# facebookresearch/pytorch3d

Hardware: AMD Instinct MI355X
Metric: rasterized Mpix/s (fwd+bwd) at 512^2 faces_per_pixel=8 (higher is better)
Workload: dtype f32

## Files before the change

include/p3d_amd.h:

```cpp
#ifndef P3D_AMD_H_
#define P3D_AMD_H_

#include <stddef.h>
#include <stdint.h>

#ifdef __cplusplus
extern "C" {
#endif

#define P3D_ABI_VERSION 3

#define P3D_OK 0
#define P3D_ERR_INVALID_ARG (-1)
#define P3D_ERR_K_TOO_LARGE (-2)
#define P3D_ERR_TOO_MANY_BINS (-3)
#define P3D_ERR_WORKSPACE (-4)
#define P3D_ERR_LAUNCH (-5)
#define P3D_ERR_UNSUPPORTED (-6)

#define P3D_MAX_K 150
#define P3D_MAX_BINS_PER_SIDE 21

typedef void* p3d_stream_t;

int p3d_abi_version(void);
const char* p3d_error_string(int code);


size_t p3d_rasterize_meshes_workspace_bytes(int64_t F, int N, int H, int W, int bin_size, int max_faces_per_bin);

size_t p3d_rasterize_meshes_short_workspace_bytes(int64_t F, int N, int H, int W, int bin_size, int max_faces_per_bin,
                                                  int64_t list_entries);
size_t p3d_rasterize_meshes_workspace_need_offset(int64_t F, int N, int H, int W, int bin_size, int max_faces_per_bin);

int p3d_rasterize_meshes(const float* face_verts, const int64_t* mesh_to_face_first_idx,
                         const int64_t* num_faces_per_mesh, const int64_t* clipped_faces_neighbor_idx, int64_t F, int N,
                         int H, int W, float blur_radius, int faces_per_pixel, int bin_size, int max_faces_per_bin,
                         int perspective_correct, int clip_barycentric_coords, int cull_backfaces, int64_t* pix_to_face,
                         float* zbuf, float* bary, float* dists, void* workspace, size_t workspace_bytes,
                         p3d_stream_t stream);

int p3d_rasterize_meshes_naive(const float* face_verts, const int64_t* mesh_to_face_first_idx,
                               const int64_t* num_faces_per_mesh, const int64_t* clipped_faces_neighbor_idx, int64_t F,
                               int N, int H, int W, float blur_radius, int faces_per_pixel, int perspective_correct,
                               int clip_barycentric_coords, int cull_backfaces, int64_t* pix_to_face, float* zbuf,
                               float* bary, float* dists, p3d_stream_t stream);

int p3d_rasterize_meshes_coarse(const float* face_verts, const int64_t* mesh_to_face_first_idx,
                                const int64_t* num_faces_per_mesh, int64_t F, int N, int H, int W, float blur_radius,
                                int bin_size, int max_faces_per_bin, int32_t* bin_faces, void* workspace,
                                size_t workspace_bytes, p3d_stream_t stream);

size_t p3d_rasterize_fine_workspace_bytes(int N, int BH, int BW, int M);

int p3d_rasterize_meshes_fine(const float* face_verts, const int32_t* bin_faces,
                              const int64_t* clipped_faces_neighbor_idx, int64_t F, int N, int BH, int BW, int M, int H,
                              int W, float blur_radius, int bin_size, int faces_per_pixel, int perspective_correct,
                              int clip_barycentric_coords, int cull_backfaces, int64_t* pix_to_face, float* zbuf,
                              float* bary, float* dists, void* workspace, size_t workspace_bytes, p3d_stream_t stream);

int p3d_rasterize_meshes_backward(const float* face_verts, const int64_t* pix_to_face, const float* grad_zbuf,
                                  const float* grad_bary, const float* grad_dists, int64_t F, int N, int H, int W, int K,
                                  int perspective_correct, int clip_barycentric_coords, float* grad_face_verts,
                                  p3d_stream_t stream);

size_t p3d_rasterize_meshes_cover_bytes(int N, int H, int W);

int p3d_rasterize_meshes_cover_check(const int64_t* pix_to_face, const int32_t* cover, int N, int H, int W, int K, int32_t* stale,
                                     p3d_stream_t stream);

size_t p3d_rasterize_meshes_cover_list_bytes(int N, int H, int W);

#define P3D_RASTER_COVER_LIST 1u
#define P3D_RASTER_CUDA_TIE_ORDER 2u


int p3d_rasterize_meshes_ex(const float* face_verts, const int64_t* mesh_to_face_first_idx, const int64_t* num_faces_per_mesh,
                            const int64_t* clipped_faces_neighbor_idx, int64_t F, int N, int H, int W, float blur_radius,
                            int faces_per_pixel, int bin_size, int max_faces_per_bin, int perspective_correct,
                            int clip_barycentric_coords, int cull_backfaces, int64_t* pix_to_face, float* zbuf, float* bary,
                            float* dists, int32_t* cover, unsigned flags, void* workspace, size_t workspace_bytes,
                            p3d_stream_t stream);

int p3d_gather_face_verts_pre(const float* verts, const int64_t* faces, int64_t V, int64_t F, float* face_verts, float* face_pre,
                              p3d_stream_t stream);

size_t p3d_rasterize_meshes_backward_workspace_bytes(int N, int H, int W);

#define P3D_BWD_COVER_HAS_LIST 1u
#define P3D_BWD_MAKE_FACE_PRE 2u

int p3d_rasterize_meshes_backward_ex(const float* face_verts, const int64_t* faces, float* face_pre,
                                     const int64_t* pix_to_face, const float* grad_zbuf, const float* grad_bary,
                                     const float* grad_dists, const int32_t* cover, int64_t F, int64_t V, int N, int H, int W,
                                     int K, int perspective_correct, int clip_barycentric_coords, unsigned flags,
                                     float* grad_out, void* workspace, size_t workspace_bytes, p3d_stream_t stream);


int p3d_gather_face_verts(const float* verts, const int64_t* faces, int64_t V, int64_t F, float* face_verts,
                          p3d_stream_t stream);
int p3d_scatter_face_grads(const float* grad_face_verts, const int64_t* faces, int64_t V, int64_t F, float* grad_verts,
                           p3d_stream_t stream);


int p3d_face_areas_normals_forward(const float* verts, const int64_t* faces, int64_t V, int64_t F, float* areas, float* normals,
                                   p3d_stream_t stream);
int p3d_face_areas_normals_backward(const float* grad_areas, const float* grad_normals, const float* verts, const int64_t* faces,
                                    int64_t V, int64_t F, float* grad_face_verts, p3d_stream_t stream);

size_t p3d_verts_normals_forward_workspace_bytes(int64_t F);
size_t p3d_verts_normals_backward_workspace_bytes(int64_t F);
int p3d_verts_normals_forward(const float* verts, const int64_t* faces, const int32_t* offsets, const int32_t* corners, int64_t V,
                              int64_t F, float* face_raw, float* sums, float* normals, p3d_stream_t stream);
int p3d_verts_normals_backward(const float* grad_normals, const float* verts, const int64_t* faces, const float* sums,
                               const int32_t* offsets, const int32_t* corners, int64_t V, int64_t F, float* face_rows,
                               float* grad_verts, p3d_stream_t stream);

size_t p3d_mesh_edge_loss_forward_workspace_bytes(int64_t E);
size_t p3d_mesh_laplacian_forward_workspace_bytes(int64_t V);
size_t p3d_mesh_normal_consistency_forward_workspace_bytes(int64_t P);
size_t p3d_mesh_normal_consistency_backward_workspace_bytes(int64_t P);
int p3d_mesh_edge_loss_forward(const float* verts, const int32_t* edges, const int32_t* edge_mesh, const int32_t* num_edges, int64_t V,
                               int64_t E, int N, float target_length, void* workspace, size_t workspace_bytes, float* loss,
                               p3d_stream_t stream);
int p3d_mesh_edge_loss_backward(const float* grad_loss, const float* verts, const int32_t* adj_offsets, const int32_t* adj,
                                const int32_t* vert_mesh, const int32_t* num_edges, int64_t V, int64_t E, int N, float target_length,
                                float* grad_verts, p3d_stream_t stream);
int p3d_mesh_laplacian_forward(const float* verts, const int32_t* adj_offsets, const int32_t* adj, const int32_t* vert_mesh,
                               const int32_t* num_verts, int64_t V, int64_t E, int N, float* q, void* workspace, size_t workspace_bytes,
                               float* loss, p3d_stream_t stream);
int p3d_mesh_laplacian_backward(const float* grad_loss, const float* q, const int32_t* adj_offsets, const int32_t* adj, int64_t V, int64_t E,
                                int N, float* grad_verts, p3d_stream_t stream);
int p3d_mesh_normal_consistency_forward(const float* verts, const int32_t* pairs, const int32_t* pair_mesh, const int32_t* num_pairs,
                                        int64_t V, int64_t P, int N, void* workspace, size_t workspace_bytes, float* loss,
                                        p3d_stream_t stream);
int p3d_mesh_normal_consistency_backward(const float* grad_loss, const float* verts, const int32_t* pairs, const int32_t* pair_mesh,
                                         const int32_t* num_pairs, const int32_t* offsets, const int32_t* slots, int64_t V, int64_t P,
                                         int N, void* workspace, size_t workspace_bytes, float* grad_verts, p3d_stream_t stream);


int p3d_transform_gather_face_verts(const float* verts_world, const int64_t* faces, const int64_t* mesh_to_face_first_idx,
                                    const float* matrices, int64_t V, int64_t F, int N, int num_matrices, float* face_verts,
                                    p3d_stream_t stream);
int p3d_transform_verts_forward(const float* verts_world, const int64_t* mesh_to_vert_first_idx, const float* matrices,
                                int64_t V, int N, int num_matrices, float* verts_ndc, p3d_stream_t stream);
int p3d_transform_verts_backward(const float* verts_world, const int64_t* mesh_to_vert_first_idx, const float* matrices,
                                 const float* grad_verts_ndc, int64_t V, int N, int num_matrices, float* grad_verts_world,
                                 p3d_stream_t stream);
size_t p3d_transform_backward_workspace_bytes(int64_t V, int N, int num_matrices);
int p3d_transform_backward_cameras(const float* verts_world, const int64_t* mesh_to_vert_first_idx, const float* matrices,
                                   const float* grad_verts_ndc, int64_t V, int N, int num_matrices, float* grad_verts_world,
                                   float* grad_matrices, void* workspace, size_t workspace_bytes, p3d_stream_t stream);


size_t p3d_rasterize_points_workspace_bytes(int64_t P, int N, int H, int W, int bin_size, int max_points_per_bin);
size_t p3d_rasterize_points_short_workspace_bytes(int64_t P, int N, int H, int W, int bin_size, int max_points_per_bin,
                                                  int64_t list_entries);
size_t p3d_rasterize_points_workspace_need_offset(int64_t P, int N, int H, int W, int bin_size, int max_points_per_bin);

int p3d_rasterize_points_ex(const float* points, const int64_t* cloud_to_packed_first_idx, const int64_t* num_points_per_cloud,
                            const float* radius, int64_t P, int N, int H, int W, int points_per_pixel, int bin_size,
                            int max_points_per_bin, int32_t* idxs, float* zbuf, float* dists, int composite_mode,
                            const float* features, int C, float inv_r2, float* images, unsigned flags, void* workspace,
                            size_t workspace_bytes, p3d_stream_t stream);

int p3d_rasterize_points(const float* points, const int64_t* cloud_to_packed_first_idx,
                         const int64_t* num_points_per_cloud, const float* radius, int64_t P, int N, int H, int W,
                         int points_per_pixel, int bin_size, int max_points_per_bin, int32_t* idxs, float* zbuf,
                         float* dists, void* workspace, size_t workspace_bytes, p3d_stream_t stream);

int p3d_rasterize_points_naive(const float* points, const int64_t* cloud_to_packed_first_idx,
                               const int64_t* num_points_per_cloud, const float* radius, int64_t P, int N, int H, int W,
                               int points_per_pixel, int32_t* idxs, float* zbuf, float* dists, p3d_stream_t stream);
// ... 297 lines not shown
```

pytorch3d_amd/_C.py:

```python
import ctypes
import os

import torch

from . import _lib

EPS = 1e-6
MAX_FLOAT = 3.4e38
MAX_INT = 2147483647
MAX_UINT = 4294967295
MAX_USHORT = 65535
PULSAR_MAX_GRAD_SPHERES = 128

kMaxPointsPerPixel = 150
kMaxItemsPerBin = 22


def _ptr(t):
    return ctypes.c_void_p(t.data_ptr() if t is not None and t.numel() > 0 else None)


def _stream(device):
    return ctypes.c_void_p(torch.cuda.current_stream(device).cuda_stream)

# ... 103 lines not shown
        self.pinned = None
        self.event = None

    def collect(self):
        if self.event is not None and self.event.query():
            self.last = int(self.pinned[0])
            self.entries = self.last if self.entries is None or self.last >= self.entries else self.entries - (self.entries - self.last) // 8
            self.event = None

    def tight(self):
        return self.last is not None and self.capacity is not None and self.last * 5 > self.capacity * 4

    def report_later(self, ws, offset, capacity=None):
        self.calls += 1
        if self.event is not None or (torch.cuda.is_available() and torch.cuda.is_current_stream_capturing()):
            return
        if not (self.calls <= 4 or self.calls % 8 == 0 or self.tight()):
            return
        if self.pinned is None:
            self.pinned = torch.empty((1,), dtype=torch.int64, pin_memory=True)
        self.pinned.copy_(ws[offset:offset + 8].view(torch.int64), non_blocking=True)
        self.event = torch.cuda.Event()
        self.event.record()
        if capacity is not None:
            self.capacity = int(capacity)


def _mesh_workspace(lib, F, N, H, W, bin_size, M, dev, what="meshes", extra=0):
    worst_fn = getattr(lib, f"p3d_rasterize_{what}_workspace_bytes")
    short_fn = getattr(lib, f"p3d_rasterize_{what}_short_workspace_bytes")
    at_fn = getattr(lib, f"p3d_rasterize_{what}_workspace_need_offset")
    worst = worst_fn(F, N, H, W, bin_size, M)
    if SHORT_WORKSPACE == "never" or (SHORT_WORKSPACE != "always" and worst <= SHORT_WORKSPACE_ABOVE):
        WORKSPACE_STATS["last_bytes"], WORKSPACE_STATS["last_entries"] = worst, None
        return _workspace(worst, dev), None, 0, None
    key = (what, dev.index, F, N, H, W, bin_size, M)
    need = _NEEDS.get(key)
    if need is None:
        if len(_NEEDS) >= 64:
            _NEEDS.pop(next(iter(_NEEDS)))
        need = _NEEDS[key] = _Need()
    if not torch.cuda.is_current_stream_capturing():
        need.collect()
    if need.entries is not None:
        entries = need.entries + need.entries // 4 + 4096
    else:
        entries = SHORT_WORKSPACE_FIRST_GUESS if SHORT_WORKSPACE_FIRST_GUESS is not None else 32 * F + (1 << 18)
    nbytes = min(short_fn(F, N, H, W, bin_size, M, int(entries)) + extra, worst)
    WORKSPACE_STATS["short_calls"] += 1
    WORKSPACE_STATS["last_bytes"], WORKSPACE_STATS["last_entries"] = nbytes, int(entries)
    return _workspace(nbytes, dev), need, at_fn(F, N, H, W, bin_size, M), int(entries)


CUDA_TIE_ORDER = os.environ.get("P3D_CUDA_TIE_ORDER", "0") not in ("", "0")


def _check_face_verts(face_verts):
    if not (face_verts.dim() == 3 and face_verts.size(1) == 3 and face_verts.size(2) == 3):
        raise RuntimeError("face_verts must have dimensions (num_faces, 3, 3)")


def _mesh_outputs(N, H, W, K, device):
    p2f = torch.empty((N, H, W, K), dtype=torch.int64, device=device)
    zbuf = torch.empty((N, H, W, K), dtype=torch.float32, device=device)
    bary = torch.empty((N, H, W, K, 3), dtype=torch.float32, device=device)
    dists = torch.empty((N, H, W, K), dtype=torch.float32, device=device)
    return p2f, zbuf, bary, dists


def rasterize_meshes(face_verts, mesh_to_face_first_idx, num_faces_per_mesh, clipped_faces_neighbor_idx, image_size,
                     blur_radius, faces_per_pixel, bin_size, max_faces_per_bin, perspective_correct,
                     clip_barycentric_coords, cull_backfaces):
    out, cover = _rasterize_meshes_covered(face_verts, mesh_to_face_first_idx, num_faces_per_mesh, clipped_faces_neighbor_idx,
                                           image_size, blur_radius, faces_per_pixel, bin_size, max_faces_per_bin, perspective_correct,
                                           clip_barycentric_coords, cull_backfaces, want_cover=True)
    if cover is not None:
        _remember_cover(out[0], cover)
    return out


RECALL_COVERS = os.environ.get("P3D_RECALL_COVERS", "1") not in ("", "0")
COVER_LIST = os.environ.get("P3D_COVER_LIST", "1") not in ("", "0")
FACE_PRE = os.environ.get("P3D_FACE_PRE", "1") not in ("", "0")
CHECK_COVERS = os.environ.get("P3D_CHECK", "0") not in ("", "0")
COVER_RECALLS = [0, 0]
COVER_CHECKS = [0, 0]
_COVER_ATTR = "_p3d_row_cover"


def _remember_cover(p2f, cover):
    setattr(p2f, _COVER_ATTR, (cover, p2f._version))


def forget_cover(pix_to_face):
    if hasattr(pix_to_face, _COVER_ATTR):
        delattr(pix_to_face, _COVER_ATTR)


def cover_is_current(p2f, cover):
    N, H, W, K = p2f.shape
    lib = _lib.load()
    with torch.cuda.device(p2f.device):
        stale = torch.empty((1,), dtype=torch.int32, device=p2f.device)
        rc = lib.p3d_rasterize_meshes_cover_check(_ptr(p2f), _ptr(cover), N, H, W, K, _ptr(stale), _stream(p2f.device))
        _lib.check(rc, "rasterize_meshes_cover_check")
        bad = bool(int(stale.item()))
    COVER_CHECKS[0] += 1
    COVER_CHECKS[1] += int(bad)
    return not bad


def checked_cover(p2f, cover):
    if cover is None or not CHECK_COVERS or torch.cuda.is_current_stream_capturing() or cover_is_current(p2f, cover):
        return cover
    import warnings

    warnings.warn("pytorch3d_amd: pix_to_face holds faces its forward's row cover does not know of (written through .data or by "
                  "another kernel since the forward?); the backward reads every row instead", RuntimeWarning)
    return None


def _recall_cover(p2f):
    e = getattr(p2f, _COVER_ATTR, None) if RECALL_COVERS and p2f.dtype == torch.int64 and p2f.is_contiguous() and p2f.dim() == 4 else None
    ok = e is not None and p2f._version == e[1] and e[0].device == p2f.device and \
        tuple(e[0].shape) == (p2f.shape[0], (p2f.shape[1] + 15) // 16, (p2f.shape[2] + 15) // 16)
    if ok and CHECK_COVERS and not torch.cuda.is_current_stream_capturing() and not cover_is_current(p2f, e[0]):
        import warnings

        warnings.warn("pytorch3d_amd: pix_to_face holds faces its forward's row cover does not know of (written through .data or by "
                      "another kernel since the forward?); the backward reads every row instead", RuntimeWarning)
        forget_cover(p2f)
        ok = False
    if not ok:
        COVER_RECALLS[1] += 1
        return None
    COVER_RECALLS[0] += 1
    return e[0]


def _rasterize_meshes_covered(face_verts, mesh_to_face_first_idx, num_faces_per_mesh, clipped_faces_neighbor_idx, image_size,
                              blur_radius, faces_per_pixel, bin_size, max_faces_per_bin, perspective_correct,
                              clip_barycentric_coords, cull_backfaces, want_cover=True):
    dev = _same_device(("face_verts", face_verts), ("mesh_to_face_first_idx", mesh_to_face_first_idx),
                       ("num_faces_per_mesh", num_faces_per_mesh),
                       ("clipped_faces_neighbor_idx", clipped_faces_neighbor_idx))
    _check_face_verts(face_verts)
    if num_faces_per_mesh.size(0) != mesh_to_face_first_idx.size(0):
        raise RuntimeError("num_faces_per_mesh must have save size first dimension as mesh_to_faces_packed_first_idx")
    if clipped_faces_neighbor_idx.size(0) != face_verts.size(0):
        raise RuntimeError("clipped_faces_neighbor_idx must have save size first dimension as face_verts")
    K = int(faces_per_pixel)
    _check_k(K)
    H, W = _hw(image_size)
    bin_size, M = int(bin_size), int(max_faces_per_bin)
    binned = bin_size > 0 and M > 0
    if binned:
        _num_bins(H, W, bin_size, "RasterizeCoarseCuda")
    fv = _c(face_verts, torch.float32)
    first, count = _c(mesh_to_face_first_idx, torch.int64), _c(num_faces_per_mesh, torch.int64)
    nb = _c(clipped_faces_neighbor_idx, torch.int64)
    N, F = count.size(0), fv.size(0)
    lib = _lib.load()
    with torch.cuda.device(dev):
        out = _mesh_outputs(N, H, W, K, dev)
        if out[0].numel() == 0:
            return out, None
        marks = N * ((H + 7) // 8) * ((W + 7) // 8) * 8 + 1024 if CUDA_TIE_ORDER else 0
        ws, need, need_at, entries = _mesh_workspace(lib, F, N, H, W, bin_size, M, dev, extra=marks) if binned else (_workspace(marks, dev), None, 0, None)
        cover, flags = None, _lib.RASTER_CUDA_TIE_ORDER if CUDA_TIE_ORDER else 0
        if want_cover and not CUDA_TIE_ORDER and COVER_LIST:
            words = N * ((H + 15) // 16) * ((W + 15) // 16)
            buf = torch.empty((lib.p3d_rasterize_meshes_cover_list_bytes(N, H, W) // 4,), dtype=torch.int32, device=dev)
            cover = buf[:words].view(N, (H + 15) // 16, (W + 15) // 16)
            flags |= _lib.RASTER_COVER_LIST
        elif want_cover:
            cover = torch.empty((N, (H + 15) // 16, (W + 15) // 16), dtype=torch.int32, device=dev)
        rc = lib.p3d_rasterize_meshes_ex(
            _ptr(fv), _ptr(first), _ptr(count), _ptr(nb), F, N, H, W, float(blur_radius), K, bin_size if binned else 0,
            M if binned else 0, int(bool(perspective_correct)), int(bool(clip_barycentric_coords)), int(bool(cull_backfaces)),
            _ptr(out[0]), _ptr(out[1]), _ptr(out[2]), _ptr(out[3]), _ptr(cover), flags, _ptr(ws), ws.numel(), _stream(dev))
        _lib.check(rc, "rasterize_meshes")
        if need is not None:
            need.report_later(ws, need_at, entries)
    return out, cover


def _rasterize_meshes_naive(face_verts, mesh_to_face_first_idx, num_faces_per_mesh, clipped_faces_neighbor_idx,
                            image_size, blur_radius, faces_per_pixel, perspective_correct, clip_barycentric_coords,
                            cull_backfaces):
    return rasterize_meshes(face_verts, mesh_to_face_first_idx, num_faces_per_mesh, clipped_faces_neighbor_idx,
                            image_size, blur_radius, faces_per_pixel, 0, 0, perspective_correct,
                            clip_barycentric_coords, cull_backfaces)


def _rasterize_meshes_coarse(face_verts, mesh_to_face_first_idx, num_faces_per_mesh, image_size, blur_radius, bin_size,
                             max_faces_per_bin):
    dev = _same_device(("face_verts", face_verts), ("mesh_to_face_first_idx", mesh_to_face_first_idx),
                       ("num_faces_per_mesh", num_faces_per_mesh))
    _check_face_verts(face_verts)
    H, W = _hw(image_size)
    bin_size, M = int(bin_size), int(max_faces_per_bin)
    BH, BW = _num_bins(H, W, bin_size, "RasterizeCoarseCuda")
    fv = _c(face_verts, torch.float32)
    first, count = _c(mesh_to_face_first_idx, torch.int64), _c(num_faces_per_mesh, torch.int64)
    N, F = count.size(0), fv.size(0)
    lib = _lib.load()
    with torch.cuda.device(dev):
        out = torch.empty((N, BH, BW, M), dtype=torch.int32, device=dev)
        if out.numel() == 0:
            return out
        ws = _workspace(lib.p3d_rasterize_meshes_workspace_bytes(F, N, H, W, bin_size, M), dev)
        rc = lib.p3d_rasterize_meshes_coarse(_ptr(fv), _ptr(first), _ptr(count), F, N, H, W, float(blur_radius),
                                             bin_size, M, _ptr(out), _ptr(ws), ws.numel(), _stream(dev))
        _lib.check(rc, "_rasterize_meshes_coarse")
    return out


def _rasterize_meshes_fine(face_verts, bin_faces, clipped_faces_neighbor_idx, image_size, blur_radius, bin_size,
                           faces_per_pixel, perspective_correct, clip_barycentric_coords, cull_backfaces):
    dev = _same_device(("face_verts", face_verts), ("bin_faces", bin_faces),
                       ("clipped_faces_neighbor_idx", clipped_faces_neighbor_idx))
    _check_face_verts(face_verts)
    if bin_faces.dim() != 4:
        raise RuntimeError("bin_faces must have 4 dimensions")
    if clipped_faces_neighbor_idx.size(0) != face_verts.size(0):
        raise RuntimeError("clipped_faces_neighbor_idx must have the same first dimension as face_verts")
    K = int(faces_per_pixel)
    if K > kMaxPointsPerPixel:
        raise RuntimeError("Must have num_closest <= 150")
    H, W = _hw(image_size)
    fv = _c(face_verts, torch.float32)
    bf = _c(bin_faces, torch.int32)
    nb = _c(clipped_faces_neighbor_idx, torch.int64)
    N, BH, BW, M = bf.shape
    lib = _lib.load()
    with torch.cuda.device(dev):
        out = _mesh_outputs(N, H, W, K, dev)
        if out[0].numel() == 0:
            return out
        ws = _workspace(lib.p3d_rasterize_fine_workspace_bytes(N, BH, BW, M), dev)
        rc = lib.p3d_rasterize_meshes_fine(_ptr(fv), _ptr(bf), _ptr(nb), fv.size(0), N, BH, BW, M, H, W,
                                           float(blur_radius), int(bin_size), K, int(bool(perspective_correct)),
                                           int(bool(clip_barycentric_coords)), int(bool(cull_backfaces)), _ptr(out[0]),
                                           _ptr(out[1]), _ptr(out[2]), _ptr(out[3]), _ptr(ws), ws.numel(), _stream(dev))
        _lib.check(rc, "_rasterize_meshes_fine")
    return out


def cover_ptr(cover, N, H, W):
    if cover is None:
        return None
    if cover.dtype != torch.int32 or tuple(cover.shape) != (N, (H + 15) // 16, (W + 15) // 16) or not cover.is_contiguous():
        raise RuntimeError("row cover does not belong to this pix_to_face")
    return _ptr(cover)


def cover_has_list(cover, N, H, W):
    if cover is None or cover.storage_offset() != 0 or not cover.is_contiguous():
        return False
    need = _lib.load().p3d_rasterize_meshes_cover_list_bytes(N, H, W)
    return need > 0 and cover.untyped_storage().nbytes() == need


def backward_workspace(cover, N, H, W, dev):
    n = _lib.load().p3d_rasterize_meshes_backward_workspace_bytes(N, H, W) if (cover is not None and not cover_has_list(cover, N, H, W)) else 0
    return _workspace(n, dev)


def _mesh_backward(face_verts, faces, V, pix_to_face, grad_zbuf, grad_bary, grad_dists, perspective_correct, clip_barycentric_coords,
                   cover, face_pre=None):
    dev = pix_to_face.device
    zeros = lambda *tail: torch.zeros(tuple(pix_to_face.shape) + tail, dtype=torch.float32, device=dev)
    gz = _c(grad_zbuf, torch.float32) if grad_zbuf is not None else zeros()
    gb = _c(grad_bary, torch.float32) if grad_bary is not None else zeros(3)
    gd = _c(grad_dists, torch.float32) if grad_dists is not None else zeros()
    fv, p2f = _c(face_verts, torch.float32), _c(pix_to_face, torch.int64)
    N, H, W, K = p2f.shape
    F = fv.size(0)
    persp, clip = int(bool(perspective_correct)), int(bool(clip_barycentric_coords))
    has_list = cover_has_list(cover, N, H, W)
    flags = _lib.BWD_COVER_HAS_LIST if has_list else 0
    with torch.cuda.device(dev):
        if faces is None:
            out = torch.empty((F, 3, 3), dtype=torch.float32, device=dev)
            if FACE_PRE and persp and clip and K in (4, 8):
                face_pre = torch.empty((F, 4), dtype=torch.float32, device=dev)
                flags |= _lib.BWD_MAKE_FACE_PRE
        else:
            faces = _c(faces, torch.int64)
            out = (torch.empty if F else torch.zeros)((V, 3), dtype=torch.float32, device=dev)
            if not (has_list or cover is None):
                face_pre = None
        if F == 0:
            return out
        if _ordered():
            lib = _lib.load()
            hits = _sorted_hits(p2f)
            corners = _sorted_corners(faces, V) if faces is not None else None
            ws = _workspace(lib.p3d_rasterize_meshes_backward_ordered_workspace_bytes(F, int(faces is not None), hits.numel()), dev)
            rc = lib.p3d_rasterize_meshes_backward_ordered(
                _ptr(fv), _ptr(faces), _ptr(p2f), _ptr(gz), _ptr(gb), _ptr(gd), _ptr(hits), hits.numel(), _ptr(corners),
                corners.numel() if corners is not None else 0, F, V, N, H, W, K, persp, clip, _ptr(out), _ptr(ws), ws.numel(), _stream(dev))
            _lib.check(rc, "rasterize_meshes_backward")
            return out
        ws = backward_workspace(cover, N, H, W, dev)
        rc = _lib.load().p3d_rasterize_meshes_backward_ex(
            _ptr(fv), _ptr(faces), _ptr(face_pre), _ptr(p2f), _ptr(gz), _ptr(gb), _ptr(gd), cover_ptr(cover, N, H, W), F, V, N, H, W,
            K, persp, clip, flags, _ptr(out), _ptr(ws), ws.numel(), _stream(dev))
        _lib.check(rc, "rasterize_meshes_backward")
    return out


def scatter_face_grads(grad_face_verts, faces, V):
    dev = grad_face_verts.device
    g, faces = _c(grad_face_verts, torch.float32), _c(faces, torch.int64)
    F = faces.shape[0]
    lib = _lib.load()
    with torch.cuda.device(dev):
        out = torch.empty((V, 3), dtype=torch.float32, device=dev)
        if not V:
            return out
        if _ordered():
            corners = _sorted_corners(faces, V)
            ws = _workspace(lib.p3d_scatter_face_grads_ordered_workspace_bytes(F), dev)
            rc = lib.p3d_scatter_face_grads_ordered(_ptr(g), _ptr(faces), _ptr(corners), corners.numel(), V, F, _ptr(out), _ptr(ws),
                                                    ws.numel(), _stream(dev))
        else:
            rc = lib.p3d_scatter_face_grads(_ptr(g), _ptr(faces), V, F, _ptr(out), _stream(dev))
        _lib.check(rc, "scatter_face_grads")
    return out


def rasterize_meshes_backward(face_verts, pix_to_face, grad_zbuf, grad_bary, grad_dists, perspective_correct,
                              clip_barycentric_coords, _cover=None):
    _same_device(("face_verts", face_verts), ("pix_to_face", pix_to_face), ("grad_zbuf", grad_zbuf), ("grad_bary", grad_bary),
                 ("grad_dists", grad_dists))
    if _cover is None:
        _cover = _recall_cover(pix_to_face)
    return _mesh_backward(face_verts, None, 0, pix_to_face, grad_zbuf, grad_bary, grad_dists, perspective_correct,
                          clip_barycentric_coords, _cover)


def _check_points(points):
    if not (points.dim() == 2 and points.size(1) == 3):
        raise RuntimeError("points must have dimensions (num_points, 3)")


def _point_outputs(N, H, W, K, device):
    idx = torch.empty((N, H, W, K), dtype=torch.int32, device=device)
    zbuf = torch.empty((N, H, W, K), dtype=torch.float32, device=device)
    dists = torch.empty((N, H, W, K), dtype=torch.float32, device=device)
    return idx, zbuf, dists


_SPLAT_MODES = {"alpha": 0, "norm": 1}


def _rasterize_points(who, points, cloud_to_packed_first_idx, num_points_per_cloud, image_size, radius, points_per_pixel, bin_size,
                      max_points_per_bin, features=None, inv_r2=0.0, mode="alpha"):
    splat = features is not None
    dev = _same_device(("points", points), ("cloud_to_packed_first_idx", cloud_to_packed_first_idx),
                       ("num_points_per_cloud", num_points_per_cloud), ("radius", radius), *((("features", features),) if splat else ()))
    _check_points(points)
    if radius.dim() != 1 or radius.size(0) != points.size(0):
        raise RuntimeError("radius must be of shape (P,)")
    if splat and (features.dim() != 2 or features.size(0) != points.size(0) or not 1 <= features.size(1) <= 4):
        raise RuntimeError("features must be of shape (P, C) with C in 1..4")
    K = int(points_per_pixel)
    _check_k(K)
    H, W = _hw(image_size)
    bin_size, M = int(bin_size), int(max_points_per_bin)
    binned = bin_size > 0 and M > 0
    if binned:
# ... 769 lines not shown
```

pytorch3d_amd/_lib.py:

```python
import ctypes
import os
import threading

_HERE = os.path.dirname(os.path.abspath(__file__))
LIB_PATH = os.environ.get("P3D_LIB_PATH") or os.path.join(_HERE, "libp3d_amd.so")

c_i64 = ctypes.c_int64
c_int = ctypes.c_int
c_uint = ctypes.c_uint
c_f32 = ctypes.c_float
c_f64 = ctypes.c_double
c_ptr = ctypes.c_void_p
c_size = ctypes.c_size_t

ABI_VERSION = 3

RASTER_COVER_LIST = 1
RASTER_CUDA_TIE_ORDER = 2
BWD_COVER_HAS_LIST = 1
BWD_MAKE_FACE_PRE = 2
KNN_MAX_K = 32
KNN_TILE = 512
KNN_ACCUMULATE_P2 = 1
FRAMES_MAX_K = 64
FRAMES_DISAMBIGUATE = 1
FRAMES_ROWS_PER_GROUP = 64
BOX3D_LDS_CAPACITY = 64
BOX3D_WAVES_PER_GROUP = 4
BOX3D_MAX_GROUPS = 4096
FPS_REGISTER_POINTS = 16384
POINT_MESH_POINT, POINT_MESH_SEGMENT, POINT_MESH_TRIANGLE = 0, 1, 2
POINT_MESH_TILE = 64
POINT_MESH_ACCUMULATE_QUERIES = 1
POINT_MESH_ACCUMULATE_TARGETS = 2

_SIGNATURES = {
    "p3d_abi_version": (c_int, []),
    "p3d_error_string": (ctypes.c_char_p, [c_int]),
    "p3d_rasterize_meshes_workspace_bytes": (c_size, [c_i64, c_int, c_int, c_int, c_int, c_int]),
    "p3d_rasterize_meshes_short_workspace_bytes": (c_size, [c_i64, c_int, c_int, c_int, c_int, c_int, c_i64]),
    "p3d_rasterize_meshes_workspace_need_offset": (c_size, [c_i64, c_int, c_int, c_int, c_int, c_int]),
    "p3d_rasterize_meshes": (c_int, [c_ptr, c_ptr, c_ptr, c_ptr, c_i64, c_int, c_int, c_int, c_f32, c_int, c_int, c_int,
                                     c_int, c_int, c_int, c_ptr, c_ptr, c_ptr, c_ptr, c_ptr, c_size, c_ptr]),
    "p3d_rasterize_meshes_naive": (c_int, [c_ptr, c_ptr, c_ptr, c_ptr, c_i64, c_int, c_int, c_int, c_f32, c_int, c_int,
                                           c_int, c_int, c_ptr, c_ptr, c_ptr, c_ptr, c_ptr]),
    "p3d_rasterize_meshes_coarse": (c_int, [c_ptr, c_ptr, c_ptr, c_i64, c_int, c_int, c_int, c_f32, c_int, c_int, c_ptr,
                                            c_ptr, c_size, c_ptr]),
    "p3d_rasterize_fine_workspace_bytes": (c_size, [c_int, c_int, c_int, c_int]),
    "p3d_rasterize_meshes_fine": (c_int, [c_ptr, c_ptr, c_ptr, c_i64, c_int, c_int, c_int, c_int, c_int, c_int, c_f32,
                                          c_int, c_int, c_int, c_int, c_int, c_ptr, c_ptr, c_ptr, c_ptr, c_ptr, c_size,
                                          c_ptr]),
    "p3d_rasterize_meshes_backward": (c_int, [c_ptr, c_ptr, c_ptr, c_ptr, c_ptr, c_i64, c_int, c_int, c_int, c_int,
                                              c_int, c_int, c_ptr, c_ptr]),
    "p3d_rasterize_meshes_cover_bytes": (c_size, [c_int, c_int, c_int]),
    "p3d_rasterize_meshes_cover_check": (c_int, [c_ptr, c_ptr, c_int, c_int, c_int, c_int, c_ptr, c_ptr]),
    "p3d_rasterize_meshes_cover_list_bytes": (c_size, [c_int, c_int, c_int]),
    "p3d_rasterize_meshes_ex": (c_int, [c_ptr, c_ptr, c_ptr, c_ptr, c_i64, c_int, c_int, c_int, c_f32, c_int, c_int, c_int, c_int,
                                        c_int, c_int, c_ptr, c_ptr, c_ptr, c_ptr, c_ptr, c_uint, c_ptr, c_size, c_ptr]),
    "p3d_rasterize_meshes_backward_workspace_bytes": (c_size, [c_int, c_int, c_int]),
    "p3d_gather_face_verts": (c_int, [c_ptr, c_ptr, c_i64, c_i64, c_ptr, c_ptr]),
    "p3d_gather_face_verts_pre": (c_int, [c_ptr, c_ptr, c_i64, c_i64, c_ptr, c_ptr, c_ptr]),
    "p3d_rasterize_meshes_backward_ex": (c_int, [c_ptr, c_ptr, c_ptr, c_ptr, c_ptr, c_ptr, c_ptr, c_ptr, c_i64, c_i64, c_int, c_int,
                                                 c_int, c_int, c_int, c_int, c_uint, c_ptr, c_ptr, c_size, c_ptr]),
    "p3d_scatter_face_grads": (c_int, [c_ptr, c_ptr, c_i64, c_i64, c_ptr, c_ptr]),
    "p3d_face_areas_normals_forward": (c_int, [c_ptr, c_ptr, c_i64, c_i64, c_ptr, c_ptr, c_ptr]),
    "p3d_face_areas_normals_backward": (c_int, [c_ptr, c_ptr, c_ptr, c_ptr, c_i64, c_i64, c_ptr, c_ptr]),
    "p3d_verts_normals_forward_workspace_bytes": (c_size, [c_i64]),
    "p3d_verts_normals_backward_workspace_bytes": (c_size, [c_i64]),
    "p3d_verts_normals_forward": (c_int, [c_ptr, c_ptr, c_ptr, c_ptr, c_i64, c_i64, c_ptr, c_ptr, c_ptr, c_ptr]),
    "p3d_verts_normals_backward": (c_int, [c_ptr, c_ptr, c_ptr, c_ptr, c_ptr, c_ptr, c_i64, c_i64, c_ptr, c_ptr, c_ptr]),
    "p3d_mesh_edge_loss_forward_workspace_bytes": (c_size, [c_i64]),
    "p3d_mesh_laplacian_forward_workspace_bytes": (c_size, [c_i64]),
    "p3d_mesh_normal_consistency_forward_workspace_bytes": (c_size, [c_i64]),
    "p3d_mesh_normal_consistency_backward_workspace_bytes": (c_size, [c_i64]),
    "p3d_mesh_edge_loss_forward": (c_int, [c_ptr, c_ptr, c_ptr, c_ptr, c_i64, c_i64, c_int, c_f32, c_ptr, c_size, c_ptr, c_ptr]),
    "p3d_mesh_edge_loss_backward": (c_int, [c_ptr, c_ptr, c_ptr, c_ptr, c_ptr, c_ptr, c_i64, c_i64, c_int, c_f32, c_ptr, c_ptr]),
    "p3d_mesh_laplacian_forward": (c_int, [c_ptr, c_ptr, c_ptr, c_ptr, c_ptr, c_i64, c_i64, c_int, c_ptr, c_ptr, c_size, c_ptr, c_ptr]),
    "p3d_mesh_laplacian_backward": (c_int, [c_ptr, c_ptr, c_ptr, c_ptr, c_i64, c_i64, c_int, c_ptr, c_ptr]),
    "p3d_mesh_normal_consistency_forward": (c_int, [c_ptr, c_ptr, c_ptr, c_ptr, c_i64, c_i64, c_int, c_ptr, c_size, c_ptr, c_ptr]),
    "p3d_mesh_normal_consistency_backward": (c_int, [c_ptr, c_ptr, c_ptr, c_ptr, c_ptr, c_ptr, c_ptr, c_i64, c_i64, c_int, c_ptr, c_size,
                                                     c_ptr, c_ptr]),
    "p3d_transform_gather_face_verts": (c_int, [c_ptr, c_ptr, c_ptr, c_ptr, c_i64, c_i64, c_int, c_int, c_ptr, c_ptr]),
    "p3d_transform_verts_forward": (c_int, [c_ptr, c_ptr, c_ptr, c_i64, c_int, c_int, c_ptr, c_ptr]),
    "p3d_transform_verts_backward": (c_int, [c_ptr, c_ptr, c_ptr, c_ptr, c_i64, c_int, c_int, c_ptr, c_ptr]),
    "p3d_transform_backward_workspace_bytes": (c_size, [c_i64, c_int, c_int]),
    "p3d_transform_backward_cameras": (c_int, [c_ptr, c_ptr, c_ptr, c_ptr, c_i64, c_int, c_int, c_ptr, c_ptr, c_ptr, c_size, c_ptr]),
    "p3d_rasterize_points_workspace_bytes": (c_size, [c_i64, c_int, c_int, c_int, c_int, c_int]),
    "p3d_rasterize_points_short_workspace_bytes": (c_size, [c_i64, c_int, c_int, c_int, c_int, c_int, c_i64]),
    "p3d_rasterize_points_workspace_need_offset": (c_size, [c_i64, c_int, c_int, c_int, c_int, c_int]),
    "p3d_rasterize_points_ex": (c_int, [c_ptr, c_ptr, c_ptr, c_ptr, c_i64, c_int, c_int, c_int, c_int, c_int, c_int, c_ptr, c_ptr,
                                        c_ptr, c_int, c_ptr, c_int, c_f32, c_ptr, c_uint, c_ptr, c_size, c_ptr]),
    "p3d_rasterize_points": (c_int, [c_ptr, c_ptr, c_ptr, c_ptr, c_i64, c_int, c_int, c_int, c_int, c_int, c_int, c_ptr,
                                     c_ptr, c_ptr, c_ptr, c_size, c_ptr]),
    "p3d_rasterize_points_naive": (c_int, [c_ptr, c_ptr, c_ptr, c_ptr, c_i64, c_int, c_int, c_int, c_int, c_ptr, c_ptr,
                                           c_ptr, c_ptr]),
    "p3d_rasterize_points_coarse": (c_int, [c_ptr, c_ptr, c_ptr, c_ptr, c_i64, c_int, c_int, c_int, c_int, c_int, c_ptr,
                                            c_ptr, c_size, c_ptr]),
    "p3d_rasterize_points_fine": (c_int, [c_ptr, c_ptr, c_ptr, c_i64, c_int, c_int, c_int, c_int, c_int, c_int, c_int,
                                          c_int, c_ptr, c_ptr, c_ptr, c_ptr, c_size, c_ptr]),
    "p3d_rasterize_points_composite_backward": (c_int, [c_int, c_ptr, c_ptr, c_ptr, c_ptr, c_ptr, c_i64, c_int, c_int, c_int, c_int, c_int,
                                                        ctypes.c_float, c_ptr, c_ptr, c_ptr]),
    "p3d_rasterize_points_backward": (c_int, [c_ptr, c_ptr, c_ptr, c_ptr, c_i64, c_int, c_int, c_int, c_int, c_ptr,
                                              c_ptr]),
    "p3d_composite_forward": (c_int, [c_int, c_ptr, ctypes.POINTER(c_i64), c_ptr, c_ptr, c_int, c_int, c_i64, c_int, c_int, c_int,
                                      ctypes.POINTER(c_i64), ctypes.POINTER(c_i64), c_ptr, c_ptr]),
    "p3d_composite_backward": (c_int, [c_int, c_ptr, c_ptr, ctypes.POINTER(c_i64), c_ptr, c_ptr, c_int, c_int, c_i64, c_int, c_int,
                                       c_int, ctypes.POINTER(c_i64), ctypes.POINTER(c_i64), c_ptr, ctypes.POINTER(c_i64), c_ptr,
                                       c_ptr]),
    "p3d_interp_face_attrs_forward": (c_int, [c_int, c_ptr, c_ptr, c_ptr, c_i64, c_i64, c_i64, c_ptr, c_ptr]),
    "p3d_interp_face_attrs_backward": (c_int, [c_int, c_ptr, c_ptr, c_ptr, c_ptr, c_i64, c_i64, c_i64, c_ptr, c_ptr,
                                               c_ptr]),
    "p3d_interp_face_attrs_backward_nhwk": (c_int, [c_ptr, c_ptr, c_ptr, c_ptr, c_int, c_int, c_int, c_int, c_i64, c_int,
                                                    c_ptr, c_ptr, c_ptr]),
    "p3d_clip_faces_plan_bytes": (c_size, [c_i64]),
    "p3d_clip_faces_plan": (c_int, [c_ptr, c_i64, ctypes.POINTER(c_f32), c_int, c_int, c_int, c_f32, c_ptr, c_size,
                                    c_ptr]),
    "p3d_clip_faces_emit": (c_int, [c_ptr, c_i64, c_ptr, c_int, c_ptr, c_size, c_i64, c_i64, c_i64, c_f32, c_int, c_ptr,
                                    c_ptr, c_ptr, c_ptr, c_ptr, c_ptr, c_ptr, c_ptr]),
    "p3d_clip_faces_backward": (c_int, [c_ptr, c_i64, c_ptr, c_size, c_i64, c_i64, c_f32, c_int, c_ptr, c_ptr, c_ptr,
                                        c_ptr]),
    "p3d_convert_clipped_forward": (c_int, [c_ptr, c_ptr, c_ptr, c_ptr, c_ptr, c_i64, c_ptr, c_ptr, c_ptr]),
    "p3d_convert_clipped_backward": (c_int, [c_ptr, c_ptr, c_ptr, c_ptr, c_ptr, c_i64, c_i64, c_ptr, c_ptr, c_ptr]),
    "p3d_sigmoid_alpha_blend_forward": (c_int, [c_ptr, c_ptr, c_f32, c_i64, c_int, c_ptr, c_ptr]),
    "p3d_sigmoid_alpha_blend_backward": (c_int, [c_ptr, c_ptr, c_ptr, c_ptr, c_f32, c_i64, c_int, c_ptr, c_ptr]),
    "p3d_softmax_rgb_blend_forward": (c_int, [c_ptr, c_ptr, c_ptr, c_ptr, c_f32, c_f32, ctypes.POINTER(c_f32), c_f32,
                                              c_f32, c_ptr, c_ptr, c_i64, c_i64, c_int, c_ptr, c_ptr]),
    "p3d_softmax_rgb_blend_backward": (c_int, [c_ptr, c_ptr, c_ptr, c_ptr, c_ptr, c_f32, c_f32, ctypes.POINTER(c_f32),
                                               c_f32, c_f32, c_ptr, c_ptr, c_i64, c_i64, c_int, c_ptr, c_ptr, c_ptr,
                                               c_ptr]),
    "p3d_phong_shade_forward": (c_int, [c_ptr, c_ptr, c_ptr, c_int, c_ptr, c_ptr, c_int, c_int, c_int, c_int, c_int, c_i64,
                                        c_ptr, c_ptr]),
    "p3d_phong_shade_backward": (c_int, [c_ptr, c_ptr, c_ptr, c_ptr, c_int, c_ptr, c_ptr, c_int, c_int, c_int, c_int,
                                         c_int, c_i64, c_ptr, c_ptr, c_ptr, c_ptr, c_ptr]),
    "p3d_soft_phong_supported_k": (c_int, [c_int]),
    "p3d_soft_phong_forward": (c_int, [c_ptr, c_ptr, c_ptr, c_ptr, c_ptr, c_int, c_ptr, c_ptr, c_int, c_f32, c_f32,
                                       ctypes.POINTER(c_f32), c_f32, c_f32, c_ptr, c_ptr, c_int, c_int, c_int, c_int, c_i64,
                                       c_ptr, c_ptr]),
    "p3d_soft_phong_backward": (c_int, [c_ptr, c_ptr, c_ptr, c_ptr, c_ptr, c_ptr, c_int, c_ptr, c_ptr, c_int, c_f32, c_f32,
                                        ctypes.POINTER(c_f32), c_f32, c_f32, c_ptr, c_ptr, c_int, c_int, c_int, c_int, c_i64,
                                        c_ptr, c_ptr, c_ptr, c_ptr, c_ptr, c_ptr, c_ptr]),
    "p3d_sample_uv_forward": (c_int, [c_ptr, c_ptr, c_ptr, c_ptr, c_int, c_int, c_int, c_int, c_i64, c_int, c_int, c_int,
# ... 135 lines not shown
```

pytorch3d_amd/build.py:

```python
import json
import os
import re
import subprocess
import sys
from concurrent.futures import ThreadPoolExecutor

HERE = os.path.dirname(os.path.abspath(__file__))
CSRC = os.path.join(HERE, "csrc")
LIB = os.environ.get("P3D_LIB_PATH") or os.path.join(HERE, "libp3d_amd.so")
ARCH = "gfx950"

SOURCES = ["binning.hip", "raster_mesh.hip", "raster_mesh_bwd.hip", "gather.hip", "transform.hip", "raster_points.hip", "render_points.hip", "composite.hip", "blend.hip", "clip.hip", "interp.hip", "shade.hip", "soft_phong.hip", "splatter.hip", "texture.hip", "texture_multi.hip", "atlas.hip", "ordered_bwd.hip", "normals.hip", "mesh_losses.hip", "knn.hip", "point_mesh.hip", "sample_points.hip", "fps_ball.hip", "points_to_volumes.hip", "point_frames.hip", "box3d.hip", "profile.cpp"]
HEADERS = ["binning.h", "p3d_common.h", "p3d_geom.h", "topk.h", "topk_insert_asm.h", "wave_table.h", "tile_map.h", "chunk_order.h", "atlas_cell.h", "uvm_sample.h", "shade_sample.h", "ordered_sum.h", "knn_grad.h", "knn_queue.h", "point_mesh_geom.h", "vec3.h", "fixed_sum.h", "csr_gather.h", "box3d_geom.h", os.path.join("..", "..", "include", "p3d_amd.h")]

FLAGS = [
    f"--offload-arch={ARCH}", "-O3", "-std=c++17", "-fPIC", "-fvisibility=hidden", "-ffp-contract=off",
    "-munsafe-fp-atomics", "-Wno-unused-result",
    "-fno-slp-vectorize",
]


AGPR_KERNELS_TESTED = {
    "softmax_blend_bwd_kernel<32>": "tests/test_gpu_blending.py::test_blend_kernels_vs_oracle_all_capacities[17|24|32-dense]",
    "composite_bwd_tile_kernel<0, 32>": "tests/test_gpu_points_composite_interp.py::test_compositors[17|24|32]",
}


def _hipcc():
    for c in (os.environ.get("HIPCC"), "/opt/rocm/bin/hipcc", "hipcc"):
        if c and (os.path.isabs(c) and os.path.exists(c) or not os.path.isabs(c)):
            return c
    return "hipcc"


def _newest(paths):
    return max(os.path.getmtime(p) for p in paths if os.path.exists(p))


def _extra_flags():
    return os.environ.get("P3D_EXTRA_FLAGS", "").split()


def _flag_signature():
    return " ".join(FLAGS + _extra_flags())


def _stamp_path():
    return LIB + ".flags"


def needs_build():
    if not os.path.exists(LIB) or not os.path.exists(LIB + ".resources.json"):
        return True
    try:
        if open(_stamp_path()).read() != _flag_signature():
            return True
    except OSError:
        return True
    deps = [os.path.join(CSRC, s) for s in SOURCES + HEADERS] + [os.path.abspath(__file__)]
    return _newest(deps) > os.path.getmtime(LIB)


def build(force=False, verbose=False):
    if not (force or needs_build()):
        return LIB
    hipcc = _hipcc()
    objdir = os.path.join(HERE, "build", os.path.basename(LIB))
    os.makedirs(objdir, exist_ok=True)

    def compile_one(src):
        obj = os.path.join(objdir, src + ".o")
        extra = _extra_flags()
        cmd = [hipcc] + FLAGS + extra + ["-Rpass-analysis=kernel-resource-usage", "-x", "hip", "-c", os.path.join(CSRC, src), "-o", obj]
        if verbose:
            print(" ".join(cmd))
        res = subprocess.run(cmd, stderr=subprocess.PIPE, text=True)
        if res.returncode != 0:
            sys.stderr.write(res.stderr)
            raise subprocess.CalledProcessError(res.returncode, cmd)
        return obj, kernel_resources(res.stderr)

    with ThreadPoolExecutor(max_workers=min(len(SOURCES), os.cpu_count() or 1)) as ex:
        done = list(ex.map(compile_one, SOURCES))
    objs = [o for o, _ in done]
    resources = {}
    for src, (_, r) in zip(SOURCES, done):
        for k, v in r.items():
            resources[k] = dict(v, source=src)
    spilled = sorted(k for k, v in resources.items() if v["vgpr_spill"] > 0)
    agpr = sorted(k for k, v in resources.items() if v["agprs"] > 0 and not any(demangle(k).startswith("void " + t + "(") or demangle(k).startswith(t + "(")
                                                                                 for t in AGPR_KERNELS_TESTED))
    if (spilled or agpr) and os.environ.get("P3D_ALLOW_SPILLS"):
        print("[build] P3D_ALLOW_SPILLS: kernels with spilled VGPRs:", ", ".join(demangle(k) for k in spilled) or "none",
              "| with untested AGPR use:", ", ".join(demangle(k) for k in agpr) or "none", file=sys.stderr)
    elif agpr:
        raise RuntimeError("kernels that keep registers in AGPRs and are not in build.py: AGPR_KERNELS_TESTED (see there; "
# ... 41 lines not shown
```

pytorch3d_amd/csrc/binning.h:

```cpp
#pragma once

#include "p3d_common.h"

namespace p3d {

constexpr int kBinChunk = 1024;
constexpr int kMaxBinsSide = 32;
constexpr int kMaxBins = kMaxBinsSide * kMaxBinsSide;

enum BinKind { kTriangles = 0, kPoints = 1 };

struct BinGeom {
  int H, W, bin_size, BH, BW, nbins;
};

inline BinGeom make_geom(int H, int W, int bin_size) {
  BinGeom g;
  g.H = H;
  g.W = W;
  g.bin_size = bin_size;
  g.BH = 1 + (H - 1) / bin_size;
  g.BW = 1 + (W - 1) / bin_size;
  g.nbins = g.BH * g.BW;
  return g;
}

inline BinGeom make_internal_geom(int H, int W, int user_bin_size) {
  int b = 16;
  const int m = H > W ? H : W;
  while ((m + b - 1) / b > kMaxBinsSide) b *= 2;
  if (user_bin_size < b) {
    if ((m + user_bin_size - 1) / user_bin_size <= kMaxBinsSide) b = user_bin_size;
  }
  return make_geom(H, W, b);
}

constexpr int kPlanClasses = 64;
constexpr int kPlanHdr = 4;
constexpr int kPlanTicket = kPlanHdr + 2 * kPlanClasses;
constexpr int kPlanHdrInts = kPlanTicket + 4;
struct TilePlan {
  const int* arank;
  const int* bg_list;
  const int* hdr;
  const int* order;
};

struct BinCSR {
  const int64_t* offset;
  const int* total;
  const int* list;
  TilePlan plan;
  int stride = 1;
};

struct BinWorkspace {
  int* chunk_start;
  int* counts;
  int* total;
  int64_t* offset;
  long long* blocksum;
  int* arank;
  int* bg_list;
  int* plan_hdr;
  int* order;
  int* list;
  int stride;
  int64_t max_chunks;
  int64_t capacity;
  int64_t worst;
  size_t need_at;
};

int64_t bin_capacity(int64_t E, int N, const BinGeom& g, int M);
size_t bin_workspace_bytes(int64_t E, int N, const BinGeom& g, int M, int64_t list_entries = -1, bool with_z = false);
bool bin_carve(Arena& arena, int64_t E, int N, const BinGeom& g, int M, BinWorkspace* ws, int64_t list_entries = -1, bool with_z = false);

int bin_build(BinKind kind, const float* elems, const float* aux, const int64_t* first, const int64_t* count, int64_t E,
              int N, const BinGeom& g, int M, float sqrt_blur, const BinWorkspace& ws, hipStream_t stream,
              bool ordered = true);

int exclusive_scan_i32(const int* in, int64_t n, long long* blocksum, int64_t* out, hipStream_t stream);

int bin_expand_padded(const BinWorkspace& ws, int N, const BinGeom& g, int M, int32_t* out, hipStream_t stream);

int bin_compact_padded(const int32_t* padded, int64_t rows, int M, int* ws_list, int* ws_total, int64_t* ws_offset,
                       hipStream_t stream);

}
```

pytorch3d_amd/csrc/binning.hip:

```cpp
#include "binning.h"
#include "p3d_geom.h"

namespace p3d {

namespace {

constexpr int kWavesPerChunk = kBinChunk / kWave;

__global__ __launch_bounds__(1024) void bin_plan_kernel(const int64_t* __restrict__ count, int N,
                                                        int* __restrict__ chunk_start, int* __restrict__ plan_hdr) {
  __shared__ int scan[1024];
  __shared__ int carry_s;
  const int tid = threadIdx.x;
  if (tid < 2 * kPlanClasses) plan_hdr[kPlanHdr + tid] = 0;
  if (tid == 0) plan_hdr[kPlanTicket] = 0;
  if (tid == 0) carry_s = 0;
  __syncthreads();
  for (int base = 0; base < N; base += 1024) {
    const int i = base + tid;
    int v = 0;
    if (i < N) {
      const int64_t c = count[i];
      v = c > 0 ? (int)((c + kBinChunk - 1) / kBinChunk) : 0;
    }
    scan[tid] = v;
    __syncthreads();
    for (int d = 1; d < 1024; d <<= 1) {
      const int add = tid >= d ? scan[tid - d] : 0;
      __syncthreads();
      scan[tid] += add;
      __syncthreads();
    }
    const int carry = carry_s;
    if (i < N) chunk_start[i] = carry + scan[tid] - v;
    __syncthreads();
    if (tid == 1023) carry_s = carry + scan[1023];
    __syncthreads();
  }
  if (tid == 0) chunk_start[N] = carry_s;
}

struct BinRect {
  int x0, x1, y0, y1;
};

struct ChunkCtx {
  int n;
  int64_t e;
  BinRect r;
  BinRect u;
  float z;
};

constexpr int kSelfPlanMax = 64;

__device__ __forceinline__ void plan_in_lds(const int64_t* __restrict__ count, int N, int* cs) {
  const int tid = threadIdx.x;
  if (tid < kWave) {
    int v = 0;
    if (tid < N) {
      const int64_t c = count[tid];
      v = c > 0 ? (int)((c + kBinChunk - 1) / kBinChunk) : 0;
    }
    int x = v;
    for (int d = 1; d < kWave; d <<= 1) {
      const int y = __shfl_up(x, d);
      if (tid >= d) x += y;
    }
    cs[tid + 1] = x;
    if (tid == 0) cs[0] = 0;
  }
  __syncthreads();
}

template <typename Pred>
__device__ __forceinline__ int prefix_count(int n, Pred holds) {
  int lo = 0;
#pragma unroll
  for (int step = 32; step >= 1; step >>= 1) {
    const int t = lo + step;
    const int i = (t < n ? t : n) - 1;
    if (t <= n && holds(i)) lo = t;
  }
  return lo;
}

template <int KIND>
__device__ __forceinline__ bool chunk_prologue(const float* __restrict__ elems, const float* __restrict__ aux,
                                               const int64_t* __restrict__ first, const int64_t* __restrict__ count,
                                               const int* chunk_start, int* cs_l, int N, int H, int W, int bin_size,
                                               int BH, int BW, float sqrt_blur, float* xlo_t, float* xhi_t,
                                               float* ylo_t, float* yhi_t, ChunkCtx* c, int* publish_plan = nullptr,
                                               int* plan_hdr = nullptr) {
  const int tid = threadIdx.x;
  const int chunk = blockIdx.x;
  if (chunk_start == nullptr) {
    plan_in_lds(count, N, cs_l);
    chunk_start = cs_l;
    if (publish_plan != nullptr && chunk == 0) {
      if (tid <= N) publish_plan[tid] = cs_l[tid];
      if (tid < 2 * kPlanClasses) plan_hdr[kPlanHdr + tid] = 0;
      if (tid == 0) plan_hdr[kPlanTicket] = 0;
    }
  }
  if (chunk >= chunk_start[N]) return false;
  int lo = 0, hi = N;
  while (hi - lo > 1) {
    const int mid = (lo + hi) >> 1;
    if (chunk_start[mid] <= chunk)
      lo = mid;
    else
      hi = mid;
  }
  c->n = lo;
  if (tid < BW) {
    xlo_t[tid] = bin_lo(tid, bin_size, W, H);
    xhi_t[tid] = bin_hi(tid, bin_size, W, H);
  } else if (tid >= 64 && tid < 64 + BH) {
    const int b = tid - 64;
    ylo_t[b] = bin_lo(b, bin_size, H, W);
    yhi_t[b] = bin_hi(b, bin_size, H, W);
  }
  __syncthreads();

  const int64_t local = (int64_t)(chunk - chunk_start[lo]) * kBinChunk + tid;
  const int64_t cnt = count[lo];
  BinRect r;
  r.x0 = r.y0 = 1 << 20;
  r.x1 = r.y1 = -1;
  c->e = -1;
  c->z = 0.0f;
  if (local < cnt) {
    const int64_t e = first[lo] + local;
    c->e = e;
    float xmin, xmax, ymin, ymax;
    bool skip;
    if (KIND == kTriangles) {
      const float* q = elems + e * 9;
      const float v0x = q[0], v0y = q[1], v0z = q[2];
      const float v1x = q[3], v1y = q[4], v1z = q[5];
      const float v2x = q[6], v2y = q[7], v2z = q[8];
      xmin = min3(v0x, v1x, v2x) - sqrt_blur;
      xmax = max3(v0x, v1x, v2x) + sqrt_blur;
      ymin = min3(v0y, v1y, v2y) - sqrt_blur;
      ymax = max3(v0y, v1y, v2y) + sqrt_blur;
      skip = (double)min3(v0z, v1z, v2z) < P3D_KEPS;
    } else {
      const float* q = elems + e * 3;
      const float rad = aux[e];
      xmin = q[0] - rad;
      xmax = q[0] + rad;
      ymin = q[1] - rad;
      ymax = q[1] + rad;
      skip = q[2] < 0.0f;
      c->z = q[2];
    }
    if (!skip) {
      const int x0 = prefix_count(BW, [&](int b) { return !(xmin <= xhi_t[b]); });
      int x1 = prefix_count(BW, [&](int b) { return xlo_t[b] < xmax; });
      const int y0 = prefix_count(BH, [&](int b) { return !(ymin <= yhi_t[b]); });
      int y1 = prefix_count(BH, [&](int b) { return ylo_t[b] < ymax; });
      x1 -= 1;
      y1 -= 1;
      if (x0 <= x1 && y0 <= y1) {
        r.x0 = x0;
        r.x1 = x1;
        r.y0 = y0;
        r.y1 = y1;
      }
    }
  }
  c->r = r;
  BinRect u = r;
  for (int d = 32; d >= 1; d >>= 1) {
    u.x0 = min(u.x0, __shfl_xor(u.x0, d));
    u.y0 = min(u.y0, __shfl_xor(u.y0, d));
    u.x1 = max(u.x1, __shfl_xor(u.x1, d));
    u.y1 = max(u.y1, __shfl_xor(u.y1, d));
  }
  c->u = u;
  return true;
}

__device__ __forceinline__ void wave_masks(const ChunkCtx& c, int lane, unsigned long long* rm, unsigned long long* cm) {
  for (int by = c.u.y0; by <= c.u.y1; ++by) {
    const unsigned long long m = __ballot(by >= c.r.y0 && by <= c.r.y1);
    if (lane == 0) rm[by] = m;
  }
  for (int bx = c.u.x0; bx <= c.u.x1; ++bx) {
    const unsigned long long m = __ballot(bx >= c.r.x0 && bx <= c.r.x1);
    if (lane == 0) cm[bx] = m;
  }
  __builtin_amdgcn_fence(__ATOMIC_RELEASE, "wavefront");
}

template <typename F>
__device__ __forceinline__ void for_union_bins(const BinRect& u, int lane, F f) {
  const int ly = lane >> 3, lx = lane & 7;
  for (int ty = u.y0; ty <= u.y1; ty += 8) {
    for (int tx = u.x0; tx <= u.x1; tx += 8) {
      const int by = ty + ly, bx = tx + lx;
      if (by <= u.y1 && bx <= u.x1) f(by, bx);
    }
  }
}

template <int KIND, bool ORDERED>
__global__ __launch_bounds__(kBinChunk) void bin_count_kernel(const float* __restrict__ elems,
                                                              const float* __restrict__ aux,
                                                              const int64_t* __restrict__ first,
                                                              const int64_t* __restrict__ count,
                                                              const int* chunk_start, int N, int H, int W,
                                                              int bin_size, int BH, int BW, float sqrt_blur,
                                                              int* __restrict__ counts, int* publish_plan, int* plan_hdr) {
  __shared__ float xlo_t[32], xhi_t[32], ylo_t[32], yhi_t[32];
  __shared__ int cs_l[kSelfPlanMax + 1];
  __shared__ int blk_cnt[kMaxBins];
  __shared__ unsigned long long rowm[ORDERED ? kWavesPerChunk : 1][kMaxBinsSide], colm[ORDERED ? kWavesPerChunk : 1][kMaxBinsSide];
  const int nbins = BH * BW;
  for (int b = threadIdx.x; b < nbins; b += kBinChunk) blk_cnt[b] = 0;
  ChunkCtx c;
  if (!chunk_prologue<KIND>(elems, aux, first, count, chunk_start, cs_l, N, H, W, bin_size, BH, BW, sqrt_blur, xlo_t,
                            xhi_t, ylo_t, yhi_t, &c, publish_plan, plan_hdr))
    return;
  const int lane = lane_id();
  if (ORDERED) {
    const int w = threadIdx.x / kWave;
    const unsigned long long* rm = rowm[ORDERED ? w : 0];
    const unsigned long long* cm = colm[ORDERED ? w : 0];
    wave_masks(c, lane, rowm[ORDERED ? w : 0], colm[ORDERED ? w : 0]);
    for_union_bins(c.u, lane, [&](int by, int bx) {
      const int members = __popcll(rm[by] & cm[bx]);
      if (members) atomicAdd(&blk_cnt[by * BW + bx], members);
    });
  } else {
    for (int by = c.r.y0; by <= c.r.y1; ++by)
      for (int bx = c.r.x0; bx <= c.r.x1; ++bx) atomicAdd(&blk_cnt[by * BW + bx], 1);
  }
  __syncthreads();
  int* out = counts + (int64_t)blockIdx.x * nbins;
  for (int b = threadIdx.x; b < nbins; b += kBinChunk) out[b] = blk_cnt[b];
}

__global__ __launch_bounds__(256) void bin_scan_rows_kernel(int* __restrict__ counts,
                                                            const int* __restrict__ chunk_start, int N, int nbins, int M,
                                                            int* __restrict__ total) {
  const int lane = lane_id();
  const int64_t row = (int64_t)blockIdx.x * (blockDim.x / kWave) + (threadIdx.x / kWave);
  if (row >= (int64_t)N * nbins) return;
  const int n = (int)(row / nbins);
  const int b = (int)(row % nbins);
  const int c0 = chunk_start[n];
  const int nch = chunk_start[n + 1] - c0;
  int carry = 0;
  constexpr int U = 4;
  for (int base = 0; base < nch; base += U * kWave) {
    int v[U];
#pragma unroll
    for (int u = 0; u < U; ++u) {
      const int i = base + u * kWave + lane;
      v[u] = i < nch ? counts[((int64_t)(c0 + i)) * nbins + b] : 0;
    }
#pragma unroll
    for (int u = 0; u < U; ++u) {
      const int i = base + u * kWave + lane;
      int x = v[u];
      for (int d = 1; d < kWave; d <<= 1) {
        const int y = __shfl_up(x, d);
        if (lane >= d) x += y;
      }
      if (i < nch) counts[((int64_t)(c0 + i)) * nbins + b] = carry + x - v[u];
      carry += __shfl(x, kWave - 1);
    }
  }
  if (lane == 0) total[row] = carry < M ? carry : M;
}

constexpr int kPlanShift = 40;
constexpr long long kPlanMask = (1ll << kPlanShift) - 1;
__device__ __forceinline__ long long plan_pack(int total) { return (long long)total + (total > 0 ? (1ll << kPlanShift) : 0ll); }
__device__ __forceinline__ int plan_class(int v) { return kPlanClasses - 1 - min(v >> 3, kPlanClasses - 1); }

__device__ __forceinline__ void plan_emit(int64_t i, long long ex, int v, int64_t* offset, int* arank, int* bg_list) {
  offset[i] = ex & kPlanMask;
  const int r = (int)(ex >> kPlanShift);
  if (v <= 0) bg_list[i - r] = (int)i;
  arank[i] = r;
}

__device__ __forceinline__ long long block_exclusive_scan_1024(long long v, long long* wsum, long long* block_total) {
  const int tid = threadIdx.x, lane = tid & 63, w = tid >> 6;
  long long x = v;
  for (int d = 1; d < kWave; d <<= 1) {
    const long long y = __shfl_up(x, d);
    if (lane >= d) x += y;
  }
  if (lane == 63) wsum[w] = x;
  __syncthreads();
  long long base = 0, all = 0;
  for (int j = 0; j < 16; ++j) {
    const long long c = wsum[j];
    if (j < w) base += c;
    all += c;
  }
  *block_total = all;
  return base + x - v;
// ... 294 lines not shown
          list[dst_t[b] + pos] = (int)c.e;
      }
    }
  }
}

__global__ void bin_expand_kernel(const int64_t* __restrict__ offset, const int* __restrict__ total,
                                  const int* __restrict__ list, int64_t rows, int M, int32_t* __restrict__ out) {
  const int64_t n = rows * M;
  for (int64_t i = (int64_t)blockIdx.x * blockDim.x + threadIdx.x; i < n; i += (int64_t)gridDim.x * blockDim.x) {
    const int64_t row = i / M;
    const int m = (int)(i - row * M);
    out[i] = m < total[row] ? list[offset[row] + m] : -1;
  }
}

__global__ __launch_bounds__(256) void bin_compact_kernel(const int32_t* __restrict__ padded, int64_t rows, int M,
                                                          int* __restrict__ list, int* __restrict__ total,
                                                          int64_t* __restrict__ offset) {
  const int lane = lane_id();
  const int64_t row = (int64_t)blockIdx.x * (blockDim.x / kWave) + (threadIdx.x / kWave);
  if (row >= rows) return;
  const int32_t* src = padded + row * M;
  int* dst = list + row * M;
  int carry = 0;
  for (int base = 0; base < M; base += kWave) {
    const int i = base + lane;
    const int v = i < M ? src[i] : -1;
    const unsigned long long m = __ballot(v >= 0);
    if (v >= 0) dst[carry + mask_rank(m)] = v;
    carry += __popcll(m);
  }
  if (lane == 0) {
    total[row] = carry;
    offset[row] = row * M;
  }
}

}

int64_t bin_capacity(int64_t E, int N, const BinGeom& g, int M) {
  const int64_t a = E * (int64_t)g.nbins;
  const int64_t b = (int64_t)N * g.nbins * (int64_t)M;
  int64_t c = a < b ? a : b;
  if (c < 1) c = 1;
  return c;
}

bool bin_carve(Arena& arena, int64_t E, int N, const BinGeom& g, int M, BinWorkspace* ws, int64_t list_entries, bool with_z) {
  ws->max_chunks = ceil_div(E, kBinChunk) + N;
  ws->worst = bin_capacity(E, N, g, M);
  ws->chunk_start = arena.take<int>((size_t)N + 1);
  ws->counts = arena.take<int>((size_t)ws->max_chunks * g.nbins);
  ws->total = arena.take<int>((size_t)N * g.nbins);
  ws->need_at = arena.off + (size_t)N * g.nbins * sizeof(int64_t);
  ws->offset = arena.take<int64_t>((size_t)N * g.nbins + 1);
  ws->blocksum = arena.take<long long>((size_t)ceil_div((int64_t)N * g.nbins, 1024) + 1);
  ws->arank = arena.take<int>((size_t)N * g.nbins);
  ws->bg_list = arena.take<int>((size_t)N * g.nbins);
  ws->plan_hdr = arena.take<int>(kPlanHdrInts);
  ws->order = arena.take<int>((size_t)N * g.nbins);
  int64_t want = ws->worst;
  if (list_entries >= 0) {
    want = list_entries < 1 ? 1 : (list_entries < ws->worst ? list_entries : ws->worst);
    if (arena.base != nullptr && arena.cap > arena.off) {
      const int64_t room = (int64_t)((arena.cap - arena.off) / sizeof(int)) / (with_z ? 2 : 1);
      if (room > want) want = room < ws->worst ? room : ws->worst;
    }
  }
  ws->capacity = want;
  ws->stride = with_z ? 2 : 1;
  ws->list = arena.take<int>((size_t)want * (size_t)ws->stride);
  return arena.ok();
}

size_t bin_workspace_bytes(int64_t E, int N, const BinGeom& g, int M, int64_t list_entries, bool with_z) {
  Arena probe(nullptr, 0);
  BinWorkspace ws;
  bin_carve(probe, E, N, g, M, &ws, list_entries, with_z);
  return probe.off;
}

int bin_build(BinKind kind, const float* elems, const float* aux, const int64_t* first, const int64_t* count, int64_t E,
              int N, const BinGeom& g, int M, float sqrt_blur, const BinWorkspace& ws, hipStream_t stream, bool ordered) {
  if (N <= 0) return P3D_OK;
  const int64_t rows = (int64_t)N * g.nbins;
  const bool small = N <= kSelfPlanMax && rows <= 4096 && ws.max_chunks <= 128;
  const bool self_plan = N <= kSelfPlanMax;
  const int* cs = self_plan ? nullptr : ws.chunk_start;
  int* publish = self_plan && !small ? ws.chunk_start : nullptr;
  if (!self_plan) {
    LaunchScope ls("bin_plan", stream);
    bin_plan_kernel<<<1, 1024, 0, stream>>>(count, N, ws.chunk_start, ws.plan_hdr);
  }
  const unsigned chunks = (unsigned)ws.max_chunks;
  {
    LaunchScope ls("bin_count", stream);
    if (kind == kTriangles)
      bin_count_kernel<kTriangles, true><<<chunks, kBinChunk, 0, stream>>>(elems, aux, first, count, cs, N, g.H, g.W,
                                                                          g.bin_size, g.BH, g.BW, sqrt_blur, ws.counts, publish, ws.plan_hdr);
    else if (ordered)
      bin_count_kernel<kPoints, true><<<chunks, kBinChunk, 0, stream>>>(elems, aux, first, count, cs, N, g.H, g.W,
                                                                       g.bin_size, g.BH, g.BW, sqrt_blur, ws.counts, publish, ws.plan_hdr);
    else
      bin_count_kernel<kPoints, false><<<chunks, kBinChunk, 0, stream>>>(elems, aux, first, count, cs, N, g.H, g.W,
                                                                        g.bin_size, g.BH, g.BW, sqrt_blur, ws.counts, publish, ws.plan_hdr);
  }
  if (small) {
    LaunchScope ls("bin_scan_small", stream);
    bin_scan_small_kernel<<<1, 1024, 0, stream>>>(ws.counts, count, N, g.nbins, M, ws.total, ws.offset, ws.arank, ws.bg_list,
                                                  ws.plan_hdr, ws.capacity);
  } else {
    const unsigned nb = (unsigned)ceil_div(rows, 1024);
    const bool thread_rows = ws.max_chunks <= 32 * (int64_t)N;
    {
      LaunchScope ls("bin_scan_rows", stream);
      if (thread_rows)
        bin_scan_rows_sums_kernel<<<nb, 1024, 0, stream>>>(ws.counts, ws.chunk_start, N, g.nbins, M, ws.total, ws.blocksum,
                                                           ws.plan_hdr);
      else if (nb == 1)
        bin_scan_rows_tail_kernel<<<(unsigned)ceil_div(rows, kTailRows), 1024, 0, stream>>>(
            ws.counts, ws.chunk_start, N, g.nbins, M, ws.total, ws.offset, ws.arank, ws.bg_list, ws.plan_hdr, ws.order, ws.capacity);
      else
        bin_scan_rows_kernel<<<(unsigned)ceil_div(rows, 4), 256, 0, stream>>>(ws.counts, ws.chunk_start, N, g.nbins, M,
                                                                             ws.total);
    }
    if (thread_rows || nb > 1) {
      LaunchScope ls("bin_scan_offsets", stream);
      if (!thread_rows && nb > 1) bin_block_sums_kernel<<<nb, 1024, 0, stream>>>(ws.total, rows, ws.blocksum, ws.plan_hdr);
      bin_scan_offsets_kernel<<<nb, 1024, 0, stream>>>(ws.total, rows, ws.blocksum, ws.offset, ws.arank, ws.bg_list, ws.plan_hdr,
                                                       ws.order, ws.capacity);
    }
  }
  {
    LaunchScope ls("bin_fill", stream);
    if (kind == kTriangles)
      bin_fill_kernel<kTriangles, true><<<chunks, kBinChunk, 0, stream>>>(elems, aux, first, count, cs, N, g.H, g.W,
                                                                         g.bin_size, g.BH, g.BW, sqrt_blur, M, ws.counts,
                                                                         ws.offset, ws.list, ws.plan_hdr, ws.stride);
    else if (ordered)
      bin_fill_kernel<kPoints, true><<<chunks, kBinChunk, 0, stream>>>(elems, aux, first, count, cs, N, g.H, g.W,
                                                                      g.bin_size, g.BH, g.BW, sqrt_blur, M, ws.counts,
                                                                      ws.offset, ws.list, ws.plan_hdr, ws.stride);
    else
      bin_fill_kernel<kPoints, false><<<chunks, kBinChunk, 0, stream>>>(elems, aux, first, count, cs, N, g.H, g.W,
                                                                       g.bin_size, g.BH, g.BW, sqrt_blur, M, ws.counts,
                                                                       ws.offset, ws.list, ws.plan_hdr, ws.stride);
  }
  return launch_status();
}

int exclusive_scan_i32(const int* in, int64_t n, long long* blocksum, int64_t* out, hipStream_t stream) {
  if (n <= 0) return P3D_OK;
  const unsigned nb = (unsigned)ceil_div(n, 1024);
  if (nb > 1) bin_block_sums_kernel<<<nb, 1024, 0, stream>>>(in, n, blocksum, nullptr);
  bin_scan_offsets_kernel<<<nb, 1024, 0, stream>>>(in, n, blocksum, out, nullptr, nullptr, nullptr, nullptr, 0);
  return launch_status();
}

int bin_expand_padded(const BinWorkspace& ws, int N, const BinGeom& g, int M, int32_t* out, hipStream_t stream) {
  const int64_t rows = (int64_t)N * g.nbins;
  const int64_t n = rows * M;
  if (n <= 0) return P3D_OK;
  int64_t blocks = ceil_div(n, 256);
  if (blocks > 8192) blocks = 8192;
  LaunchScope ls("bin_expand", stream);
  bin_expand_kernel<<<(unsigned)blocks, 256, 0, stream>>>(ws.offset, ws.total, ws.list, rows, M, out);
  return launch_status();
}

int bin_compact_padded(const int32_t* padded, int64_t rows, int M, int* ws_list, int* ws_total, int64_t* ws_offset,
                       hipStream_t stream) {
  if (rows <= 0) return P3D_OK;
  LaunchScope ls("bin_compact", stream);
  bin_compact_kernel<<<(unsigned)ceil_div(rows, 4), 256, 0, stream>>>(padded, rows, M, ws_list, ws_total, ws_offset);
  return launch_status();
}

}
```

pytorch3d_amd/csrc/gather.hip:

```cpp
#include "p3d_common.h"
#include "p3d_geom.h"
#include "wave_table.h"

namespace p3d {
namespace {

__global__ __launch_bounds__(256) void gather_faces_kernel(const float* __restrict__ verts,
                                                           const int64_t* __restrict__ faces, int64_t V, int64_t n_corners,
                                                           float* __restrict__ face_verts) {
  for (int64_t c = (int64_t)blockIdx.x * 256 + threadIdx.x; c < n_corners; c += (int64_t)gridDim.x * 256) {
    int64_t v = faces[c];
    if (v < 0) v += V;
    const bool ok = v >= 0 && v < V;
    const float* s = verts + (ok ? v : 0) * 3;
    float* d = face_verts + c * 3;
    const float nan = __int_as_float(0x7fc00000);
    d[0] = ok ? s[0] : nan;
    d[1] = ok ? s[1] : nan;
    d[2] = ok ? s[2] : nan;
  }
}

__global__ __launch_bounds__(256) void gather_faces_pre_kernel(const float* __restrict__ verts, const int64_t* __restrict__ faces,
                                                               int64_t V, int64_t F, float* __restrict__ face_verts,
                                                               float4* __restrict__ face_pre) {
  for (int64_t f = (int64_t)blockIdx.x * 256 + threadIdx.x; f < F; f += (int64_t)gridDim.x * 256) {
    float c[9];
    const float nan = __int_as_float(0x7fc00000);
#pragma unroll
    for (int k = 0; k < 3; ++k) {
      int64_t v = faces[f * 3 + k];
      if (v < 0) v += V;
      const bool ok = v >= 0 && v < V;
      const float* s = verts + (ok ? v : 0) * 3;
      c[3 * k + 0] = ok ? s[0] : nan;
      c[3 * k + 1] = ok ? s[1] : nan;
      c[3 * k + 2] = ok ? s[2] : nan;
    }
    float* d = face_verts + f * 9;
#pragma unroll
    for (int k = 0; k < 9; ++k) d[k] = c[k];
    const BwdFacePre r = bwd_face_pre_make(mk3(c[0], c[1], c[2]), mk3(c[3], c[4], c[5]), mk3(c[6], c[7], c[8]));
    face_pre[f] = make_float4(r.inv_area, r.inv_l01, r.inv_l02, r.inv_l12);
  }
}

using VertTable = WaveTable<3, 426>;

__global__ __launch_bounds__(256) void scatter_face_grads_kernel(const float* __restrict__ grad_face_verts,
                                                                 const int64_t* __restrict__ faces, int64_t V,
                                                                 int64_t n_corners, int64_t span,
                                                                 float* __restrict__ grad_verts) {
  __shared__ __align__(16) int s_table[4][VertTable::kLdsInts];
  const int lane = threadIdx.x & 63, w = threadIdx.x >> 6;
  const int64_t begin = ((int64_t)blockIdx.x * 4 + w) * span;
  if (begin >= n_corners) return;
  const int64_t end = begin + span < n_corners ? begin + span : n_corners;
  VertTable tab;
  tab.init(s_table[w], lane);
  for (int64_t base = begin; base < end; base += 64) {
    const int64_t c = base + lane;
    int v = -1;
    float g[3] = {0.f, 0.f, 0.f};
    if (c < end) {
      int64_t vi = faces[c];
      if (vi < 0) vi += V;
      v = (vi >= 0 && vi < V) ? (int)vi : -1;
      const float* s = grad_face_verts + c * 3;
      g[0] = s[0];
      g[1] = s[1];
      g[2] = s[2];
    }
    tab.add(grad_verts, lane, v, g);
  }
  if (tab.used > 0) tab.flush(grad_verts, lane);
}

}
}

using namespace p3d;

P3D_API int p3d_gather_face_verts(const float* verts, const int64_t* faces, int64_t V, int64_t F, float* face_verts,
                                  p3d_stream_t stream) {
  if (V < 0 || F < 0) return P3D_ERR_INVALID_ARG;
  if (F == 0) return P3D_OK;
  if (!verts || !faces || !face_verts) return P3D_ERR_INVALID_ARG;
  hipStream_t s = (hipStream_t)stream;
  const int64_t n = F * 3;
  int64_t blocks = ceil_div(n, 256);
  if (blocks > 256 * 16) blocks = 256 * 16;
  LaunchScope ls("gather_face_verts", s);
  gather_faces_kernel<<<(unsigned)blocks, 256, 0, s>>>(verts, faces, V, n, face_verts);
  return launch_status();
}

P3D_API int p3d_gather_face_verts_pre(const float* verts, const int64_t* faces, int64_t V, int64_t F, float* face_verts,
                                      float* face_pre, p3d_stream_t stream) {
  if (V < 0 || F < 0) return P3D_ERR_INVALID_ARG;
  if (F == 0) return P3D_OK;
  if (!verts || !faces || !face_verts || !face_pre || ((uintptr_t)face_pre & 15u)) return P3D_ERR_INVALID_ARG;
  hipStream_t s = (hipStream_t)stream;
  int64_t blocks = ceil_div(F, 256);
  if (blocks > 256 * 16) blocks = 256 * 16;
  LaunchScope ls("gather_face_verts", s);
  gather_faces_pre_kernel<<<(unsigned)blocks, 256, 0, s>>>(verts, faces, V, F, face_verts, reinterpret_cast<float4*>(face_pre));
  return launch_status();
}

P3D_API int p3d_scatter_face_grads(const float* grad_face_verts, const int64_t* faces, int64_t V, int64_t F,
                                   float* grad_verts, p3d_stream_t stream) {
  if (V < 0 || F < 0) return P3D_ERR_INVALID_ARG;
  if (V == 0) return P3D_OK;
  if (!grad_verts) return P3D_ERR_INVALID_ARG;
  hipStream_t s = (hipStream_t)stream;
  if (hipMemsetAsync(grad_verts, 0, (size_t)V * 3 * sizeof(float), s) != hipSuccess) return P3D_ERR_LAUNCH;
  if (F == 0) return P3D_OK;
  if (!grad_face_verts || !faces) return P3D_ERR_INVALID_ARG;
  const int64_t n = F * 3;
  int64_t waves = ceil_div(n, 1024);
  if (waves > 4 * 4096) waves = 4 * 4096;
  const int64_t blocks = ceil_div(waves, 4);
  const int64_t span = ceil_div(ceil_div(n, blocks * 4), 64) * 64;
  LaunchScope ls("scatter_face_grads", s);
  scatter_face_grads_kernel<<<(unsigned)blocks, 256, 0, s>>>(grad_face_verts, faces, V, n, span, grad_verts);
  return launch_status();
// ... 2 lines not shown
```

pytorch3d_amd/csrc/raster_mesh.hip:

```cpp
#include "binning.h"
#include "tile_map.h"
#include "chunk_order.h"
#include "p3d_geom.h"
#include "topk.h"

#include <stdio.h>
#include <stdlib.h>

#ifndef P3D_STAGE_RANGE_INDEX
#define P3D_STAGE_RANGE_INDEX 1
#endif

#ifdef P3D_PROBE_CHAIN
__device__ unsigned long long g_chain[32];
extern "C" __attribute__((visibility("default"))) void p3d_probe_chain_read(unsigned long long* out) {
  (void)hipDeviceSynchronize();
  (void)hipMemcpyFromSymbol(out, HIP_SYMBOL(g_chain), sizeof(unsigned long long) * 32);
  unsigned long long z[32] = {0};
  (void)hipMemcpyToSymbol(HIP_SYMBOL(g_chain), z, sizeof(z));
}
namespace p3d {
namespace {
constexpr int kChainStamps = 11;
__shared__ unsigned long long s_chain[4][kChainStamps + 1];
// ... 462 lines not shown
        if (GENERAL || adm) hit = face_dist_rec<PC && !GENERAL>(fr, p, a.blur, bp, &h);
      }
      if (hit) {
        bool ins = true;
        if constexpr (GENERAL) {
          const int nb = __float_as_int(r2.z);
          if (nb != -1) {
            const int at = q.find(nb);
            if (at >= 0) {
              float queued;
              if constexpr (Queue::kPayload > 0) {
                queued = q.payload_at(0, at);
              } else {
                queued = recompute_face(a, nb, p, persp, clip).dist;
              }
              if (fabsf(h.dist) < fabsf(queued))
                q.erase(at);
              else
                ins = false;
            }
          }
        }
        if (ins && q.admits(K, h.z, f)) {
          if constexpr (Queue::kPayload > 0) {
            const float pl[kMeshPayload] = {h.dist, h.bary.x, h.bary.y, h.bary.z};
            q.insert(K, h.z, f, pl);
          } else {
            const float none[1] = {0.0f};
            q.insert(K, h.z, f, none);
          }
          if constexpr (TIES && !GENERAL) {
            const bool ev = (kz0 < INFINITY) & (q.kth_z(K) == kz0);
            const int d = kz0 == tie_z ? min(tie_drop, ki0) : ki0;
            tie_drop = ev ? d : tie_drop;
            tie_z = ev ? kz0 : tie_z;
          }
        }
      }
    }
  }
}

__device__ __forceinline__ void cover_mark(const MeshArgs& a, int n, int sy0, bool any, int yo, int xo, int lane) {
  unsigned long long rem = __ballot(any);
  const int wid = (yo >> 4) * a.CX + (xo >> 4);
  while (rem) {
    const int w0 = __builtin_amdgcn_readlane(wid, __builtin_ctzll(rem));
    const unsigned long long same = __ballot(any && wid == w0);
    unsigned bits = 0;
#pragma unroll
    for (int j = 0; j < 8; ++j)
      if ((same >> (8 * j)) & 0xffull) bits |= 1u << ((a.H - 1 - (sy0 + j)) & 15);
    rem &= ~same;
    if (lane == 0) {
      const int word = (n * a.CY) * a.CX + w0;
      if (a.area_list != nullptr && !a.list_by_plan) {
        const int before = atomicOr(a.cover + word, (int)bits);
        if (before == 0 && bits != 0u) a.area_list[atomicAdd(a.area_count, 1)] = word;
      } else {
        atomicOr(a.cover + word, (int)bits);
      }
    }
  }
}

__device__ __forceinline__ float uniform_f(float v) { return __int_as_float(__builtin_amdgcn_readfirstlane(__float_as_int(v))); }

struct StageLds {
  unsigned* pm;
  float pxy;
  unsigned valid_c, valid_r;
  float4 (*rec)[kRecWords];
  float* zc;
  int* order;
  float* qlow;
  ChunkOrderScratch* ord;
  int* wcnt;
};

struct TileRect {
  float x0, x1, y0, y1;
};

template <bool BINNED, bool PC = false>
__device__ __forceinline__ int stage_chunk(const MeshArgs& a, const StageLds& l, const TileRect& tile, int64_t src_base,
                                           int count, int base, int tid, bool cull, bool clip, bool prune, bool* general) {
  const int lane = tid & 63, w = tid >> 6;
  const int i = base + tid;
  bool keep = false;
  f3 v0, v1, v2;
  FaceSetup fs;
  int fid = -1, nb = -1;
  unsigned cm = 0, rm = 0;
  const bool has = i < count;
  fs.xlo = fs.xhi = fs.ylo = fs.yhi = 0.0f;
  fs.reject = true;
  if (has) {
    fid = BINNED ? a.csr.list[src_base + i] : (int)(src_base + i);
    P3D_CHAIN_ARRIVED(2, "v"(fid));
    const float* g = a.face_verts + (int64_t)fid * 9;
    nb = (int)a.neighbor[fid];
    v0 = mk3(g[0], g[1], g[2]);
    v1 = mk3(g[3], g[4], g[5]);
    v2 = mk3(g[6], g[7], g[8]);
    P3D_CHAIN_ARRIVED(3, "v"(v0.x), "v"(v1.y), "v"(v2.z), "v"(nb));
    fs = face_setup(v0, v1, v2, a.sqrt_blur, cull);
  }
  int xb = 0, xa = 0, yb = 0, ya = 0;
  if (__ballot(has) != 0) {
#if P3D_STAGE_RANGE_INDEX
    float pxy = l.pxy;
    asm volatile("" : "+v"(pxy));
    const float x0 = __int_as_float(__builtin_amdgcn_readlane(__float_as_int(pxy), 0));
    const float y0 = __int_as_float(__builtin_amdgcn_readlane(__float_as_int(pxy), 16));
    const float inv_dx = 15.0f * __builtin_amdgcn_rcpf(__int_as_float(__builtin_amdgcn_readlane(__float_as_int(pxy), 15)) - x0);
    const float inv_dy = 15.0f * __builtin_amdgcn_rcpf(__int_as_float(__builtin_amdgcn_readlane(__float_as_int(pxy), 31)) - y0);
    const int rxl = (int)rintf(fminf(fmaxf((fs.xlo - x0) * inv_dx, 0.0f), 15.0f));
    const int rxh = (int)rintf(fmaxf(fminf((fs.xhi - x0) * inv_dx, 15.0f), 0.0f));
    const float cxl = __int_as_float(__builtin_amdgcn_ds_bpermute(rxl << 2, __float_as_int(pxy)));
    const float cxh = __int_as_float(__builtin_amdgcn_ds_bpermute(rxh << 2, __float_as_int(pxy)));
    xb = rxl + (cxl < fs.xlo ? 1 : 0);
    xa = 15 - rxh + (cxh > fs.xhi ? 1 : 0);
    cm = range_mask16(xb, xa) & l.valid_c;
    __builtin_amdgcn_sched_barrier(0);
    const int ryl = (int)rintf(fminf(fmaxf((fs.ylo - y0) * inv_dy, 0.0f), 15.0f));
    const int ryh = (int)rintf(fmaxf(fminf((fs.yhi - y0) * inv_dy, 15.0f), 0.0f));
    const float cyl = __int_as_float(__builtin_amdgcn_ds_bpermute((16 + ryl) << 2, __float_as_int(pxy)));
    const float cyh = __int_as_float(__builtin_amdgcn_ds_bpermute((16 + ryh) << 2, __float_as_int(pxy)));
    yb = ryl + (cyl < fs.ylo ? 1 : 0);
    ya = 15 - ryh + (cyh > fs.yhi ? 1 : 0);
    rm = range_mask16(yb, ya) & l.valid_r;
#else
#pragma unroll
    for (int c = 0; c < 16; ++c) {
      const float xs = __int_as_float(__builtin_amdgcn_readlane(__float_as_int(l.pxy), c));
      const float ys = __int_as_float(__builtin_amdgcn_readlane(__float_as_int(l.pxy), 16 + c));
      xb += xs < fs.xlo ? 1 : 0;
      xa += xs > fs.xhi ? 1 : 0;
      yb += ys < fs.ylo ? 1 : 0;
      ya += ys > fs.yhi ? 1 : 0;
    }
    cm = range_mask16(xb, xa) & l.valid_c;
    rm = range_mask16(yb, ya) & l.valid_r;
#endif
  }
  if (has) {
    keep = !fs.reject && cm != 0 && rm != 0;
    if (keep && prune)
      keep = !rect_cannot_hit(mk2(v0.x, v0.y), mk2(v1.x, v1.y), mk2(v2.x, v2.y), tile.x0, tile.x1, tile.y0, tile.y1, a.sqrt_blur);
  }
  const unsigned long long km = __ballot(keep);
  if (lane == 0) l.wcnt[w] = __popcll(km);
  __syncthreads();
  int pos = mask_rank(km);
  int staged = 0;
#pragma unroll
  for (int j = 0; j < kStage / kWave; ++j) {
    const int c = l.wcnt[j];
    if (j < w) pos += c;
    staged += c;
  }
  bool gen = false;
  if (keep) {
    FaceRec fr;
    face_rec_make(v0, v1, v2, &fr);
    gen = nb != -1 || (PC && (fr.wide || face_rec_degenerate(fr)));
    l.pm[pos] = cm | (rm << 16);
    l.rec[pos][0] = make_float4(v0.x, v0.y, v1.x, v1.y);
    l.rec[pos][1] = make_float4(v2.x, v2.y, v0.z, v1.z);
    l.rec[pos][2] = make_float4(v2.z, __int_as_float(fid), __int_as_float(nb), __int_as_float(fr.wide ? 1 : 0));
    double2 d0, d1;
    d0.x = fr.rd_area;
    d0.y = fr.rd_l01;
    d1.x = fr.rd_l02;
    d1.y = fr.rd_l12;
    *reinterpret_cast<double2*>(&l.rec[pos][3]) = d0;
    *reinterpret_cast<double2*>(&l.rec[pos][4]) = d1;
    l.rec[pos][5] = make_float4(fr.d01.x, fr.d01.y, fr.d12.x, fr.d12.y);
    l.rec[pos][6] = make_float4(fr.d20.x, fr.d20.y, 0.0f, 0.0f);
    const float zmin = min3(v0.z, v1.z, v2.z);
    l.zc[pos] = (clip && nb == -1 && zmin >= 1e-3f && fr.rd_area == fr.rd_area) ? zmin * 0.999998f : -INFINITY;
  }
  *general = __syncthreads_or(gen ? 1 : 0) != 0;
  return staged;
}

struct SubTile {
  float x0, x1, y0, y1;
};

template <bool GENERAL, typename Queue, bool PC = false, bool TIES = false>
__device__ __forceinline__ void wave_chunk(const MeshArgs& a, int K, Queue& q, int staged, bool sorted, const SubTile& st, f2 p,
                                           bool pix_ok, int lane, bool persp, bool clip, bool prune, const unsigned* s_pm,
                                           const float4 (*s_rec)[kRecWords], const float* s_zc, const int* s_order,
                                           const float* s_qlow, int cshift, int rshift, float& tie_z, int& tie_drop, int deal = -1) {
  for (int jb = 0; jb < staged; jb += kWave) {
    const int jfirst = deal >= 0 ? deal * 16 : jb;
    if (jfirst >= staged) break;
    if (sorted && __ballot(pix_ok && !(s_qlow[jfirst] > q.kth_z(K))) == 0) break;
    const int j = deal >= 0 ? (((lane >> 4) * 4 + deal) * 16 + (lane & 15)) : jb + lane;
    bool touch = false;
    int oj = 0;
    unsigned mlo = 0, mhi = 0;
    float zcv = 0.0f;
    if (j < staged) {
      oj = s_order[j];
      const unsigned pm = s_pm[oj];
      const unsigned cmask = (pm >> cshift) & 0xffu, rmask = (pm >> (16 + rshift)) & 0xffu;
      touch = (cmask != 0) & (rmask != 0);
      if (touch && prune) {
        const float4 r0 = s_rec[oj][0], r1 = s_rec[oj][1];
        touch = !rect_cannot_hit(mk2(r0.x, r0.y), mk2(r0.z, r0.w), mk2(r1.x, r1.y), st.x0, st.x1, st.y0, st.y1, a.sqrt_blur);
      }
      block_mask_8x8(cmask, rmask, &mlo, &mhi);
      zcv = s_zc[oj];
    }
    const unsigned long long cand = __ballot(touch);
    eval_candidates<GENERAL, Queue, PC, TIES>(a, K, q, cand, oj, mlo, mhi, zcv, p, pix_ok, persp, clip, s_rec, tie_z, tie_drop);
    if (deal >= 0) break;
  }
}

constexpr int kMergeWords = 2 + kMeshPayload;

template <typename Queue, int KT>
__device__ __forceinline__ void merge_dump(const Queue& q, float* slab, int lane) {
#pragma unroll
  for (int k = 0; k < KT; ++k) {
    slab[(0 * KT + k) * kWave + lane] = q.zf(k);
    slab[(1 * KT + k) * kWave + lane] = __int_as_float(q.ix(k));
#pragma unroll
    for (int pp = 0; pp < kMeshPayload; ++pp) slab[((2 + pp) * KT + k) * kWave + lane] = q.pay(pp, k);
  }
}

template <typename Queue, int KT>
__device__ __forceinline__ void merge_absorb(Queue& q, int K, const float* slab, int lane) {
#pragma unroll 1
  for (int k = 0; k < KT; ++k) {
    const int idx = __float_as_int(slab[(1 * KT + k) * kWave + lane]);
    if (__ballot(idx != kEmptyIdx) == 0) break;
    const float z = slab[(0 * KT + k) * kWave + lane];
    float pl[kMeshPayload];
#pragma unroll
    for (int pp = 0; pp < kMeshPayload; ++pp) pl[pp] = slab[((2 + pp) * KT + k) * kWave + lane];
    if (idx != kEmptyIdx && q.admits(K, z, idx)) q.insert(K, z, idx, pl);
  }
}

template <typename Queue, int KT, bool IN_REGS, bool BINNED, bool EXACT, int WAVES = kFineWaves, bool PC = false,
          bool SPLIT = false, bool TIES = false>
__global__ __launch_bounds__(kStage, WAVES) void mesh_raster_kernel(MeshArgs a) {
  static_assert(!(SPLIT && TIES), "the tie marks of four queues that merge are not tracked: CUDA tie order runs the plain kernels");
  __shared__ float s_merge[SPLIT ? 3 * kMergeWords * KT * kWave : 1];
  __shared__ unsigned s_pm[kStage];
  __shared__ float4 s_rec[kStage][kRecWords];
  __shared__ __align__(16) float s_zc[kStage];
  __shared__ int s_order[kStage];
  __shared__ float s_qlow[kStage];
  __shared__ ChunkOrderScratch s_ord;
  __shared__ int s_wcnt[kStage / kWave];
  __shared__ int s_fill_ticket;

  P3D_CHAIN_ENTRY();
  __builtin_amdgcn_s_setprio(3);
  unsigned blk = SPLIT ? blockIdx.x >> 2 : blockIdx.x;
  const bool plan_walk = BINNED && !SPLIT && a.walk_plan != 0;
  int hdr_a = 0, hdr_b = 0, hdr_order = 0;
  int walk_row = 0;
  if (plan_walk) {
    hdr_a = a.csr.plan.hdr[0];
    hdr_b = a.csr.plan.hdr[1];
    hdr_order = a.csr.plan.hdr[3];
    const unsigned rows = (unsigned)(a.N * a.tm.BH * a.tm.BW);
    walk_row = a.csr.plan.order[blk < rows ? blk : rows - 1u];
  }
  if (a.overflow != nullptr && (*a.overflow != 0) == BINNED) return;
  TileCoord tc;
  bool listed = false;
  if (plan_walk && hdr_order != 0) {
    const unsigned A = (unsigned)hdr_a, B = (unsigned)hdr_b;
    int row;
    if (blk < A) {
      row = walk_row;
    } else if (blk < A + B) {
      if (EXACT && (KT & 3) == 0 && A > 0) return;
      row = a.csr.plan.bg_list[blk - A];
    } else {
      return;
    }
    const int per_image = a.tm.BH * a.tm.BW;
    tc.n = row / per_image;
    const int rem = row - tc.n * per_image;
    tc.by = rem / a.tm.BW;
    tc.bx = rem - tc.by * a.tm.BW;
    tc.ty = tc.tx = 0;
    if (blk < A && a.list_by_plan && threadIdx.x == 0) {
      a.area_list[blk] = (tc.n * a.CY + (a.CY - 1 - tc.by)) * a.CX + (a.CX - 1 - tc.bx);
      if (blk == 0) *a.area_count = (int)A;
    }
    listed = true;
  }
  if (!listed && !tile_of_block(a.tm, blk, &tc)) return;
  const int n = tc.n, by = tc.by, bx = tc.bx, ty = tc.ty, tx = tc.tx;

  const int H = a.H, W = a.W;
  const int y_end = min(H, (by + 1) * a.tm.bin_size);
  const int x_end = min(W, (bx + 1) * a.tm.bin_size);
  const int ty0 = by * a.tm.bin_size + ty * kTile;
  const int tx0 = bx * a.tm.bin_size + tx * kTile;
  if (ty0 >= y_end || tx0 >= x_end) return;

  const int tid = threadIdx.x;
  const int lane = tid & 63;
  const int w = __builtin_amdgcn_readfirstlane(tid >> 6);
  const int sub = SPLIT ? (int)(blockIdx.x & 3u) : w;
  const int sy0 = ty0 + (sub >> 1) * 8;
  const int sx0 = tx0 + (sub & 1) * 8;
  if (SPLIT && (sy0 >= y_end || sx0 >= x_end)) return;
  const int yi = sy0 + (lane >> 3);
  const int xi = sx0 + (lane & 7);
  const bool pix_ok = yi < y_end && xi < x_end;
  const bool wave_ok = sy0 < y_end && sx0 < x_end;

  const bool piggy = BINNED && !SPLIT && EXACT && (KT & 3) == 0 && plan_walk;
  int64_t src_base;
  int count;
  int fill_slot = (int)blk;
  if (BINNED) {
    const int64_t row = ((int64_t)n * a.tm.BH + by) * a.tm.BW + bx;
    count = a.csr.total[row];
    src_base = a.csr.offset[row];
    if (!listed && (piggy || (!SPLIT && a.list_by_plan))) fill_slot = a.csr.plan.arank[row];
  } else {
// ... 7 lines not shown
    const int q_bg = (plan_b + plan_a - 1) / plan_a;
    bg_j0 = (long long)fill_slot * q_bg;
    const long long left = (long long)plan_b - bg_j0;
    bg_n = left < 0 ? 0 : (left < q_bg ? (int)left : q_bg);
    if (bg_n > 0) bg_row0 = a.csr.plan.bg_list[bg_j0];
    if (bg_n > 1) bg_row1 = a.csr.plan.bg_list[bg_j0 + 1];
  }
  if (tid == 0) s_fill_ticket = 0;
  if (BINNED && !SPLIT && a.list_by_plan && !listed && tid == 0) {
    if (count > 0) a.area_list[fill_slot] = (n * a.CY + (a.CY - 1 - by)) * a.CX + (a.CX - 1 - bx);
    if (blockIdx.x == 0) *a.area_count = hdr_a;
  }
  P3D_CHAIN_ARM(BINNED && listed && count > 0 && count <= kStage);
  P3D_CHAIN_STAMP(1);
  if (count <= 0) {
    if (piggy && plan_a > 0) return;
    const int Kbg = EXACT ? KT : a.K;
    if (SPLIT && (Kbg & 3) == 0) {
      fill_tile_background<kStage>(a, n, sy0, sx0, y_end, x_end, tid, 8);
    } else if (SPLIT && w != 0) {
    } else if ((Kbg & 3) == 0) {
      fill_tile_background<kStage>(a, n, ty0, tx0, y_end, x_end, tid);
    } else if constexpr (EXACT && Queue::kPayload > 0) {
      Queue e;
      e.init();
      if (pix_ok) write_pixel<Queue, KT, IN_REGS>(a, e, ((int64_t)n * H + (H - 1 - yi)) * W + (W - 1 - xi));
    } else if (wave_ok) {
      Queue e;
      e.init();
      write_subtile_fill_patch<Queue, KT, IN_REGS>(a, e, false, n, sy0, sx0, y_end, x_end, lane, pix_ok, yi, xi);
    }
    return;
  }

  const int ox = SPLIT ? sx0 : tx0, oy = SPLIT ? sy0 : ty0;
  const float pxy = (lane & 16) ? pix_to_ndc(oy + (lane & 15), H, W) : pix_to_ndc(ox + (lane & 15), W, H);
  auto col_centre = [&](int x) { return __int_as_float(__builtin_amdgcn_readlane(__float_as_int(pxy), x - ox)); };
  auto row_centre = [&](int y) { return __int_as_float(__builtin_amdgcn_readlane(__float_as_int(pxy), 16 + y - oy)); };
  const f2 p = mk2(__int_as_float(__builtin_amdgcn_ds_bpermute((xi - ox) << 2, __float_as_int(pxy))),
                   __int_as_float(__builtin_amdgcn_ds_bpermute((16 + yi - oy) << 2, __float_as_int(pxy))));
  const float tile_x0 = SPLIT ? 0.0f : col_centre(tx0), tile_x1 = SPLIT ? 0.0f : col_centre(min(tx0 + kTile, x_end) - 1);
  const float tile_y0 = SPLIT ? 0.0f : row_centre(ty0), tile_y1 = SPLIT ? 0.0f : row_centre(min(ty0 + kTile, y_end) - 1);
  const float sub_x0 = col_centre(sx0), sub_x1 = col_centre(min(sx0 + 8, x_end) - 1);
  const float sub_y0 = row_centre(sy0), sub_y1 = row_centre(min(sy0 + 8, y_end) - 1);

  Queue q;
  q.init();
  const int K = EXACT ? KT : a.K;
  const bool persp = PC || a.persp != 0, clip = PC || a.clip != 0, cull = a.cull != 0;
  const bool prune = true;
  StageLds lds;
  lds.pm = s_pm;
  {
    const int side = SPLIT ? 8 : kTile;
    const int cols = min(side, x_end - ox), rows = min(side, y_end - oy);
    lds.valid_c = (1u << cols) - 1u;
    lds.valid_r = (1u << rows) - 1u;
    lds.pxy = pxy;
  }
  lds.rec = s_rec;
  lds.zc = s_zc;
  lds.order = s_order;
  lds.qlow = s_qlow;
  lds.ord = &s_ord;
  lds.wcnt = s_wcnt;
  TileRect tile;
  tile.x0 = SPLIT ? sub_x0 : tile_x0;
  tile.x1 = SPLIT ? sub_x1 : tile_x1;
  tile.y0 = SPLIT ? sub_y0 : tile_y0;
  tile.y1 = SPLIT ? sub_y1 : tile_y1;
  SubTile st;
  st.x0 = sub_x0;
  st.x1 = sub_x1;
  st.y0 = sub_y0;
  st.y1 = sub_y1;
  const bool run_waves = wave_ok;

  int base = 0;
  bool general = false;
  float tie_z = -1.0f;
  int tie_drop = kEmptyIdx;
  int staged = 0;
  for (; base < count; base += kStage) {
    staged = stage_chunk<BINNED, PC>(a, lds, tile, src_base, count, base, tid, cull, clip, prune, &general);
    if (general) break;
    P3D_CHAIN_STAMP(4);
    chunk_bucket_order(s_zc, staged, s_order, s_qlow, s_ord, tid);
    P3D_CHAIN_STAMP(5);
    __builtin_amdgcn_s_setprio(0);
    if (run_waves)
      wave_chunk<false, Queue, PC, TIES>(a, K, q, staged, true, st, p, pix_ok, lane, persp, clip, prune, s_pm, s_rec, s_zc, s_order,
                                         s_qlow, SPLIT ? 0 : (sub & 1) * 8, SPLIT ? 0 : (sub >> 1) * 8, tie_z, tie_drop, SPLIT ? w : -1);
    P3D_CHAIN_STAMP(6);
    if (base + kStage < count) __syncthreads();
    P3D_CHAIN_STAMP(7);
  }
  __builtin_amdgcn_s_setprio(0);
  if constexpr (SPLIT && Queue::kPayload > 0) {
    if (w != 0) merge_dump<Queue, KT>(q, s_merge + (w - 1) * kMergeWords * KT * kWave, lane);
    __syncthreads();
    if (w == 0) {
#pragma unroll 1
      for (int src = 0; src < 3; ++src) merge_absorb<Queue, KT>(q, K, s_merge + src * kMergeWords * KT * kWave, lane);
    }
  }
  if (general) {
    for (;;) {
      if (tid < staged) s_order[tid] = tid;
      __syncthreads();
      if (run_waves && (!SPLIT || w == 0))
        wave_chunk<true, Queue, false, TIES>(a, K, q, staged, false, st, p, pix_ok, lane, persp, clip, prune, s_pm, s_rec, s_zc, s_order,
                                             s_qlow, SPLIT ? 0 : (sub & 1) * 8, SPLIT ? 0 : (sub >> 1) * 8, tie_z, tie_drop);
      __syncthreads();
      base += kStage;
      if (base >= count) break;
      bool dummy = false;
      staged = stage_chunk<BINNED, PC>(a, lds, tile, src_base, count, base, tid, cull, clip, prune, &dummy);
    }
  }

  float tie_kz = 0.0f;
  bool tie_cand = false, tie_gen = false;
  if constexpr (TIES) {
    tie_kz = q.kth_z(K);
    tie_gen = tie_z == INFINITY;
    tie_cand = K > 1 && tie_z == tie_kz && tie_kz < INFINITY;
  }
  {
    if constexpr (Queue::kPayload == 0) {
      static_assert(!SPLIT, "queues without payload do not run in split mode");
      if (wave_ok) write_pixel_long<Queue, KT, EXACT>(a, q, ((int64_t)n * H + (H - 1 - yi)) * W + (W - 1 - xi), p, pix_ok, persp, clip);
      if (a.cover != nullptr && wave_ok) cover_mark(a, n, sy0, pix_ok && q.valid(0), H - 1 - yi, W - 1 - xi, lane);
    } else if constexpr (EXACT) {
      if (pix_ok && (!SPLIT || w == 0)) {
        int l2;
        asm volatile("v_mbcnt_lo_u32_b32 %0, -1, 0\n\tv_mbcnt_hi_u32_b32 %0, -1, %0" : "=v"(l2));
        const int yo = sy0 + (l2 >> 3), xo = sx0 + (l2 & 7);
        write_pixel<Queue, KT, IN_REGS>(a, q, ((int64_t)n * H + (H - 1 - yo)) * W + (W - 1 - xo));
      }
      if (a.cover != nullptr && (!SPLIT || w == 0)) {
        int l2;
        asm volatile("v_mbcnt_lo_u32_b32 %0, -1, 0\n\tv_mbcnt_hi_u32_b32 %0, -1, %0" : "=v"(l2));
        const int yo = sy0 + (l2 >> 3), xo = sx0 + (l2 & 7);
        cover_mark(a, n, sy0, yo < y_end && xo < x_end && q.valid(0), H - 1 - yo, W - 1 - xo, l2);
      }
    } else {
      if (wave_ok) write_subtile_fill_patch<Queue, KT, IN_REGS>(a, q, true, n, sy0, sx0, y_end, x_end, lane, pix_ok, yi, xi);
      if (a.cover != nullptr && wave_ok && (!SPLIT || w == 0)) cover_mark(a, n, sy0, pix_ok && q.valid(0), H - 1 - yi, W - 1 - xi, lane);
    }
  }
  if constexpr (TIES) {
    asm volatile("s_waitcnt vmcnt(0)" ::: "memory");
    int l2;
    asm volatile("v_mbcnt_lo_u32_b32 %0, -1, 0\n\tv_mbcnt_hi_u32_b32 %0, -1, %0" : "=v"(l2));
    const int yo = sy0 + (l2 >> 3), xo = sx0 + (l2 & 7);
    const bool inside = yo < y_end && xo < x_end;
    const int64_t tbase = (((int64_t)n * H + (H - 1 - yo)) * W + (W - 1 - xo)) * K;
    bool tie = tie_gen && inside;
    if (tie_cand && inside) {
      int s_max = -1;
      for (int k = 0; k < K; ++k) {
        const long long fi = __hip_atomic_load(a.p2f + tbase + k, __ATOMIC_RELAXED, __HIP_MEMORY_SCOPE_AGENT);
        const float fz = __int_as_float(__hip_atomic_load(reinterpret_cast<const int*>(a.zbuf + tbase + k), __ATOMIC_RELAXED, __HIP_MEMORY_SCOPE_AGENT));
        if (fi >= 0 && fz < tie_kz) s_max = max(s_max, (int)fi);
      }
      tie = s_max > tie_drop;
    }
    if (tie) a.p2f[tbase] = -2;
    const unsigned long long tmask = __ballot(tie);
    if (a.tie_words != nullptr && wave_ok && l2 == 0) a.tie_words[((int64_t)n * a.SY + (sy0 >> 3)) * a.SX + (sx0 >> 3)] = tmask;
  }
  P3D_CHAIN_STAMP(8);
  if constexpr (BINNED && !SPLIT && EXACT && (KT & 3) == 0) {
    if (bg_n > 0) {
      P3D_CHAIN_ARRIVED(9, "s"(bg_row0), "s"(bg_row1));
      int l2;
      asm volatile("v_mbcnt_lo_u32_b32 %0, -1, 0\n\tv_mbcnt_hi_u32_b32 %0, -1, %0" : "=v"(l2));
      const int per_image = a.tm.BH * a.tm.BW;
      for (;;) {
        int t = 0;
        if (l2 == 0) t = atomicAdd(&s_fill_ticket, 1);
        t = __builtin_amdgcn_readfirstlane(t);
        const int j = t >> 2;
        if (j >= bg_n) break;
        const int brow = j == 0 ? bg_row0 : (j == 1 ? bg_row1 : a.csr.plan.bg_list[bg_j0 + j]);
        const int vtid = (t & 3) * kWave + l2;
        const int bn = brow / per_image, brem = brow - bn * per_image;
        const int bby = brem / a.tm.BW, bbx = brem - bby * a.tm.BW;
        const int by_end = min(H, (bby + 1) * a.tm.bin_size), bx_end = min(W, (bbx + 1) * a.tm.bin_size);
        const int bty0 = bby * a.tm.bin_size + ty * kTile, btx0 = bbx * a.tm.bin_size + tx * kTile;
        if (bty0 >= by_end || btx0 >= bx_end) continue;
        if (bty0 + kTile <= by_end && btx0 + kTile <= bx_end)
          fill_tile_full<KT>(a, bn, bty0, btx0, vtid);
        else
          fill_tile_background<kStage>(a, bn, bty0, btx0, by_end, bx_end, vtid);
      }
    }
  }
  P3D_CHAIN_STAMP(10);
  P3D_CHAIN_FLUSH();
}

template <bool BINNED>
__device__ __forceinline__ void replay_pixel(const MeshArgs& a, int n, int yi, int xi, volatile float* qz, volatile int* qi, int lane) {
  const int H = a.H, W = a.W, K = a.K;
  int64_t src;
  int count;
  if (BINNED) {
    const int64_t row = ((int64_t)n * a.tm.BH + yi / a.tm.bin_size) * a.tm.BW + xi / a.tm.bin_size;
    src = a.csr.offset[row];
    count = a.csr.total[row];
  } else {
    src = a.mesh_first[n];
    count = (int)a.mesh_count[n];
  }
  const bool persp = a.persp != 0, clip = a.clip != 0, cull = a.cull != 0;
  auto verts = [&](int f, f3* v0, f3* v1, f3* v2) {
    const float* g = a.face_verts + (int64_t)f * 9;
    *v0 = mk3(g[0], g[1], g[2]);
    *v1 = mk3(g[3], g[4], g[5]);
    *v2 = mk3(g[6], g[7], g[8]);
  };
  struct Batch {
    int f;
    int nb;
    f3 v0, v1, v2;
  };
  auto fetch = [&](int i0) {
    Batch b;
    b.f = -1;
    b.nb = -1;
    b.v0 = b.v1 = b.v2 = mk3(0.0f, 0.0f, 0.0f);
    const int i = i0 + lane;
    if (i < count) {
      b.f = BINNED ? a.csr.list[src + i] : (int)(src + i);
      verts(b.f, &b.v0, &b.v1, &b.v2);
      b.nb = (int)a.neighbor[b.f];
    }
    return b;
  };
  const f2 p = mk2(pix_to_ndc(xi, W, H), pix_to_ndc(yi, H, W));
  const int64_t opix = ((int64_t)n * H + (H - 1 - yi)) * W + (W - 1 - xi);
  int qn = 0, qmax_i = -1;
  float qmax_z = -1000.0f;
  Batch nxt = fetch(0);
  for (int i0 = 0; i0 < count; i0 += kWave) {
    const Batch cur = nxt;
    if (i0 + kWave < count) nxt = fetch(i0 + kWave);
    FaceHit h;
    bool hit = false;
    if (cur.f >= 0) {
      const FaceSetup fs = face_setup(cur.v0, cur.v1, cur.v2, a.sqrt_blur, cull);
      if (!fs.reject && !outside_box(fs, p)) hit = face_hit(cur.v0, cur.v1, cur.v2, p, a.blur, persp, clip, &h);
    }
    unsigned long long hits = __ballot(hit);
    while (hits) {
      const int c = __builtin_ctzll(hits);
      hits &= hits - 1;
      const int cf = __builtin_amdgcn_readlane(cur.f, c);
      const float cz = __int_as_float(__builtin_amdgcn_readlane(__float_as_int(h.z), c));
      const int cnb = __builtin_amdgcn_readlane(cur.nb, c);
      int at = -1;
      if (cnb != -1) {
        for (int j0 = 0; j0 < qn; j0 += kWave) {
          const unsigned long long is = __ballot(j0 + lane < qn && qi[j0 + lane] == cnb);
          if (is) {
            at = j0 + __builtin_ctzll(is);
            break;
          }
        }
      }
      if (at != -1) {
        f3 n0, n1, n2;
        verts(cnb, &n0, &n1, &n2);
        FaceHit hn;
        face_hit(n0, n1, n2, p, a.blur, persp, clip, &hn);
        const float cdist = __int_as_float(__builtin_amdgcn_readlane(__float_as_int(h.dist), c));
        if (fabsf(cdist) < fabsf(hn.dist)) {
          if (lane == 0) {
            qz[at] = cz;
            qi[at] = cf;
          }
          if (cz > qmax_z) {
            qmax_z = cz;
            qmax_i = at;
          }
        }
      } else if (qn < K) {
        if (lane == 0) {
          qz[qn] = cz;
          qi[qn] = cf;
        }
        if (cz > qmax_z) {
          qmax_z = cz;
          qmax_i = qn;
        }
        ++qn;
      } else if (cz < qmax_z) {
        if (lane == 0) {
          qz[qmax_i] = cz;
          qi[qmax_i] = cf;
        }
        qmax_z = cz;
        __builtin_amdgcn_wave_barrier();
        float m = -INFINITY;
        for (int j = lane; j < K; j += kWave) m = fmaxf(m, qz[j]);
        for (int d = 32; d >= 1; d >>= 1) m = fmaxf(m, __shfl_xor(m, d));
        if (m > cz) {
          for (int j0 = 0; j0 < K; j0 += kWave) {
            const unsigned long long is = __ballot(j0 + lane < K && qz[j0 + lane] == m);
            if (is) {
              qmax_i = j0 + __builtin_ctzll(is);
              break;
            }
          }
          qmax_z = m;
        }
      }
      __builtin_amdgcn_wave_barrier();
    }
// ... 9 lines not shown
    const float z = qz[j];
    const int f = qi[j];
    int rank = 0;
    for (int t = 0; t < qn; ++t) {
      const float zt = qz[t];
      const int ft = qi[t];
      rank += (zt < z || (zt == z && ft < f)) ? 1 : 0;
    }
    f3 v0, v1, v2;
    verts(f, &v0, &v1, &v2);
    FaceHit h;
    face_hit(v0, v1, v2, p, a.blur, persp, clip, &h);
    const int64_t o = opix * K + rank;
    a.p2f[o] = f;
    a.zbuf[o] = h.z;
    a.dists[o] = h.dist;
    a.bary[3 * o] = h.bary.x;
    a.bary[3 * o + 1] = h.bary.y;
    a.bary[3 * o + 2] = h.bary.z;
  }
  __builtin_amdgcn_wave_barrier();
}

constexpr int kTieWordsPerWave = 16;
constexpr int kTieWaves = 8;
template <bool BINNED>
__global__ __launch_bounds__(kTieWaves * kWave) void mesh_cuda_order_words_kernel(MeshArgs a, unsigned nwords, unsigned mult) {
  __shared__ float s_qzw[kTieWaves][P3D_MAX_K];
  __shared__ int s_qiw[kTieWaves][P3D_MAX_K];
  if (a.K <= 0) return;
  if (a.overflow != nullptr && (*a.overflow != 0) == BINNED) return;
  const int lane = threadIdx.x & 63, wv = threadIdx.x >> 6;
  volatile float* s_qz = s_qzw[wv];
  volatile int* s_qi = s_qiw[wv];
  int turn = 0;
  const unsigned slot = blockIdx.x * kTieWordsPerWave + lane;
  unsigned wi = 0;
  unsigned long long word = 0;
  if (lane < kTieWordsPerWave && slot < nwords) {
    wi = (unsigned)(((unsigned long long)slot * mult) % nwords);
    word = a.tie_words[wi];
  }
  unsigned long long have = __ballot(word != 0);
  while (have) {
    const int l = __builtin_ctzll(have);
    have &= have - 1;
    const unsigned w = (unsigned)__builtin_amdgcn_readlane((int)wi, l);
    unsigned long long todo = ((unsigned long long)(unsigned)__builtin_amdgcn_readlane((int)(word >> 32), l) << 32) |
                              (unsigned long long)(unsigned)__builtin_amdgcn_readlane((int)word, l);
    const int sx = (int)(w % (unsigned)a.SX);
    const unsigned t = w / (unsigned)a.SX;
    const int sy = (int)(t % (unsigned)a.SY), n = (int)(t / (unsigned)a.SY);
    while (todo) {
      const int L = __builtin_ctzll(todo);
      todo &= todo - 1;
      if (((turn++) & (kTieWaves - 1)) != wv) continue;
      replay_pixel<BINNED>(a, n, sy * 8 + (L >> 3), sx * 8 + (L & 7), s_qz, s_qi, lane);
    }
  }
}

template <bool BINNED>
__global__ __launch_bounds__(kStage) void mesh_cuda_order_kernel(MeshArgs a) {
  __shared__ float s_qz[kStage / kWave][P3D_MAX_K];
  __shared__ int s_qi[kStage / kWave][P3D_MAX_K];
  if (a.overflow != nullptr && (*a.overflow != 0) == BINNED) return;
  TileCoord tc;
  if (!tile_of_block(a.tm, blockIdx.x, &tc)) return;
  const int n = tc.n, H = a.H, W = a.W, K = a.K;
  if (K <= 0) return;
  const int y_end = min(H, (tc.by + 1) * a.tm.bin_size), x_end = min(W, (tc.bx + 1) * a.tm.bin_size);
  const int lane = threadIdx.x & 63, w = threadIdx.x >> 6;
  const int sy0 = tc.by * a.tm.bin_size + tc.ty * kTile + (w >> 1) * 8, sx0 = tc.bx * a.tm.bin_size + tc.tx * kTile + (w & 1) * 8;
  const int yi = sy0 + (lane >> 3), xi = sx0 + (lane & 7);
  const bool pix_ok = yi < y_end && xi < x_end;
  unsigned long long todo = __ballot(pix_ok && a.p2f[(((int64_t)n * H + (H - 1 - yi)) * W + (W - 1 - xi)) * K] == -2);
  while (todo) {
    const int L = __builtin_ctzll(todo);
    todo &= todo - 1;
    replay_pixel<BINNED>(a, n, sy0 + (L >> 3), sx0 + (L & 7), s_qz[w], s_qi[w], lane);
  }
}

template <typename Q, int KT, bool REGS, bool BINNED, bool EXACT, bool TIES>
void launch_fine_variant(const MeshArgs& a, unsigned grid, bool split, size_t dyn_lds, hipStream_t stream) {
  if constexpr (REGS && EXACT && BINNED && !TIES) {
    if (split) {
      constexpr int kSplitWaves = KT >= 8 ? 2 : (KT >= 4 ? 3 : kFineWaves);
      mesh_raster_kernel<Q, KT, REGS, BINNED, EXACT, kSplitWaves, false, true><<<grid * 4, kStage, 0, stream>>>(a);
      return;
    }
  }
  if constexpr (REGS && EXACT) {
    if (a.persp && a.clip) {
      mesh_raster_kernel<typename PcQueue<Q>::type, KT, REGS, BINNED, EXACT, kFineWaves, true, false, TIES><<<grid, kStage, dyn_lds, stream>>>(a);
      return;
    }
  }
  mesh_raster_kernel<Q, KT, REGS, BINNED, EXACT, kFineWaves, false, false, TIES><<<grid, kStage, dyn_lds, stream>>>(a);
}

template <int KT, bool BINNED, int WAVES, bool TIES>
void launch_long_variant(const MeshArgs& a, unsigned grid, hipStream_t stream) {
  if (a.persp && a.clip)
    mesh_raster_kernel<TopKPairs<KT, true, 0>, KT, true, BINNED, false, WAVES, true, false, TIES><<<grid, kStage, 0, stream>>>(a);
  else
    mesh_raster_kernel<TopKPairs<KT, false, 0>, KT, true, BINNED, false, WAVES, false, false, TIES><<<grid, kStage, 0, stream>>>(a);
}

#define P3D_COMMA ,
template <bool BINNED, bool TIES>
int launch_mesh_raster_t(const MeshArgs& a0, hipStream_t stream) {
  MeshArgs a = a0;
  unsigned grid = tile_grid(a.tm);
  const char* name = BINNED ? "mesh_fine" : "mesh_naive";
  LaunchScope ls(name, stream);
  const int K = a.K;
  const bool split = BINNED && !TIES && grid <= (unsigned)kSplitMaxTiles;
  a.walk_plan = BINNED && !split && a.csr.plan.hdr != nullptr && a.csr.plan.order != nullptr && a.tm.Ty == 1 && a.tm.Tx == 1;
  a.list_by_plan = a.walk_plan && a.area_list != nullptr && a.overflow == nullptr && a.tm.bin_size == kTile && a.H % kTile == 0 && a.W % kTile == 0 &&
                   a.csr.plan.arank != nullptr;
  const size_t dyn_lds = 0;
#define P3D_LAUNCH_FINE(KT_, REGS_, EXACT_, Q_) launch_fine_variant<Q_, KT_, REGS_, BINNED, EXACT_, TIES>(a, grid, split, dyn_lds, stream)
#define P3D_LAUNCH_FINE_W(KT_, WAVES_, Q_) mesh_raster_kernel<Q_, KT_, true, BINNED, false, WAVES_, false, false, TIES><<<grid, kStage, 0, stream>>>(a)
#define P3D_LAUNCH_LONG(KT_, WAVES_) launch_long_variant<KT_, BINNED, WAVES_, TIES>(a, grid, stream)
  if (K == 1)
    P3D_LAUNCH_FINE(1, true, true, TopKReg<1 P3D_COMMA kMeshPayload>);
  else if (K == 2)
    P3D_LAUNCH_FINE(2, true, true, TopKReg<2 P3D_COMMA kMeshPayload>);
  else if (K == 3)
    P3D_LAUNCH_FINE_W(4, kFineWaves, TopKPairs<4>);
  else if (K == 4)
    P3D_LAUNCH_FINE(4, true, true, TopKPairs<4>);
  else if (K < 8)
    P3D_LAUNCH_FINE_W(8, 3, TopKPairs<8>);
  else if (K == 8)
    P3D_LAUNCH_FINE(8, true, true, TopKPairs<8>);
  else if (K <= 16)
    P3D_LAUNCH_LONG(16, 4);
  else if (K <= 24)
    P3D_LAUNCH_LONG(24, 3);
  else if (K <= 32)
    P3D_LAUNCH_LONG(32, 3);
  else if (K <= 40)
    P3D_LAUNCH_LONG(40, 2);
  else if (K <= 48)
    P3D_LAUNCH_LONG(48, 2);
  else
    P3D_LAUNCH_FINE(P3D_MAX_K, false, false, TopKMem<P3D_MAX_K P3D_COMMA kMeshPayload>);
#undef P3D_LAUNCH_FINE
#undef P3D_LAUNCH_FINE_W
#undef P3D_LAUNCH_LONG
  return launch_status();
}

template <bool BINNED>
int launch_mesh_raster(const MeshArgs& a, hipStream_t stream) {
  return a.ties ? launch_mesh_raster_t<BINNED, true>(a, stream) : launch_mesh_raster_t<BINNED, false>(a, stream);
}

void set_tiles(MeshArgs* a, int bin_size, int BH, int BW) { a->tm = make_tile_map(a->N, a->H, a->W, bin_size, BH, BW, true); }

int check_common(int N, int H, int W, int K) {
  if (N < 0 || H < 0 || W < 0 || K < 0) return P3D_ERR_INVALID_ARG;
  if (K > P3D_MAX_K) return P3D_ERR_K_TOO_LARGE;
  return P3D_OK;
}

}

}

using namespace p3d;

static size_t tie_marks_bytes(int N, int H, int W) {
  return align_up((size_t)N * (size_t)((H + 7) / 8) * (size_t)((W + 7) / 8) * sizeof(unsigned long long), 256);
}

P3D_API size_t p3d_rasterize_meshes_workspace_bytes(int64_t F, int N, int H, int W, int bin_size,
                                                    int max_faces_per_bin) {
  if (bin_size <= 0 || max_faces_per_bin <= 0 || N <= 0 || H <= 0 || W <= 0) return 0;
  const size_t user = bin_workspace_bytes(F, N, make_geom(H, W, bin_size), max_faces_per_bin);
  const size_t internal = bin_workspace_bytes(F, N, make_internal_geom(H, W, bin_size), max_faces_per_bin);
  return (user > internal ? user : internal) + 256 + tie_marks_bytes(N, H, W) + 256;
}

P3D_API size_t p3d_rasterize_meshes_short_workspace_bytes(int64_t F, int N, int H, int W, int bin_size, int max_faces_per_bin,
                                                          int64_t list_entries) {
  if (bin_size <= 0 || max_faces_per_bin <= 0 || N <= 0 || H <= 0 || W <= 0 || list_entries < 0) return 0;
  return bin_workspace_bytes(F, N, make_internal_geom(H, W, bin_size), max_faces_per_bin, list_entries) + 256;
}

P3D_API size_t p3d_rasterize_meshes_workspace_need_offset(int64_t F, int N, int H, int W, int bin_size,
                                                          int max_faces_per_bin) {
  if (bin_size <= 0 || max_faces_per_bin <= 0 || N <= 0 || H <= 0 || W <= 0) return 0;
  const BinGeom g = make_internal_geom(H, W, bin_size);
  Arena probe(nullptr, 0);
  BinWorkspace ws;
  bin_carve(probe, F, N, g, max_faces_per_bin, &ws, 1);
  return ws.need_at;
}

P3D_API size_t p3d_rasterize_fine_workspace_bytes(int N, int BH, int BW, int M) {
  const size_t rows = (size_t)N * BH * BW;
  return align_up(rows * (size_t)M * sizeof(int), 256) + align_up(rows * sizeof(int), 256) +
         align_up((rows + 1) * sizeof(int64_t), 256) + 256;
}

P3D_API size_t p3d_rasterize_meshes_cover_bytes(int N, int H, int W) {
  if (N <= 0 || H <= 0 || W <= 0) return 0;
  return (size_t)N * (size_t)((H + 15) / 16) * (size_t)((W + 15) / 16) * sizeof(int32_t);
}

P3D_API size_t p3d_rasterize_meshes_cover_list_bytes(int N, int H, int W) {
  const size_t words = p3d_rasterize_meshes_cover_bytes(N, H, W) / sizeof(int32_t);
  return words == 0 ? 0 : (2 * words + 16) * sizeof(int32_t);
}

static int cover_begin(MeshArgs* a, int32_t* cover, bool with_list, bool zero, hipStream_t s) {
  a->cover = cover;
  a->CY = (a->H + 15) / 16;
  a->CX = (a->W + 15) / 16;
  a->area_count = nullptr;
  a->area_list = nullptr;
  if (cover == nullptr) return P3D_OK;
  const size_t bytes = p3d_rasterize_meshes_cover_bytes(a->N, a->H, a->W);
  if (with_list && bytes > 0) {
    a->area_count = cover + bytes / sizeof(int32_t);
    a->area_list = a->area_count + 16;
  }
  if (!zero || bytes == 0) return P3D_OK;
  return hipMemsetAsync(cover, 0, bytes + (with_list ? 16 * sizeof(int32_t) : 0), s) == hipSuccess ? P3D_OK : P3D_ERR_LAUNCH;
}

static MeshArgs mesh_args(const float* face_verts, const int64_t* mesh_first, const int64_t* mesh_count, const int64_t* neighbor,
                          int N, int H, int W, float blur_radius, int K, int persp, int clip, int cull, int64_t* p2f, float* zbuf,
                          float* bary, float* dists) {
  MeshArgs a{};
  a.face_verts = face_verts;
  a.neighbor = neighbor;
  a.mesh_first = mesh_first;
  a.mesh_count = mesh_count;
  a.N = N;
  a.H = H;
  a.W = W;
  a.K = K;
  a.blur = blur_radius;
  a.sqrt_blur = sqrtf(blur_radius);
  a.persp = persp;
  a.clip = clip;
  a.cull = cull;
  a.p2f = p2f;
  a.zbuf = zbuf;
  a.bary = bary;
  a.dists = dists;
  return a;
}

static int mesh_naive_impl(MeshArgs a, int64_t F, int32_t* cover, bool with_list, hipStream_t s) {
  const int st = cover_begin(&a, cover, with_list, a.overflow == nullptr, s);
  if (st != P3D_OK) return st;
  if ((int64_t)a.N * a.H * a.W * a.K == 0) return P3D_OK;
  if ((!a.face_verts || !a.neighbor) && F > 0) return P3D_ERR_INVALID_ARG;
  if (!a.mesh_first || !a.mesh_count || !a.p2f || !a.zbuf || !a.bary || !a.dists) return P3D_ERR_INVALID_ARG;
  set_tiles(&a, a.H > a.W ? a.H : a.W, 1, 1);
  return launch_mesh_raster<false>(a, s);
}

P3D_API int p3d_rasterize_meshes_naive(const float* face_verts, const int64_t* mesh_first, const int64_t* mesh_count,
                                       const int64_t* neighbor, int64_t F, int N, int H, int W, float blur_radius, int K,
                                       int persp, int clip, int cull, int64_t* p2f, float* zbuf, float* bary,
                                       float* dists, p3d_stream_t stream) {
  const int rc = check_common(N, H, W, K);
  if (rc != P3D_OK) return rc;
  return mesh_naive_impl(mesh_args(face_verts, mesh_first, mesh_count, neighbor, N, H, W, blur_radius, K, persp, clip, cull, p2f, zbuf,
                                   bary, dists),
                         F, nullptr, false, (hipStream_t)stream);
}

static int mesh_fine_from_csr(MeshArgs a, const BinCSR& csr, const BinGeom& g, int32_t* cover, bool with_list, hipStream_t s) {
  a.csr = csr;
  const int st = cover_begin(&a, cover, with_list, true, s);
  if (st != P3D_OK) return st;
  set_tiles(&a, g.bin_size, g.BH, g.BW);
  return launch_mesh_raster<true>(a, s);
}

static int cuda_order_replay(MeshArgs a, const BinCSR* csr, const BinGeom* g, hipStream_t s) {
  static const bool skip = getenv("P3D_TIE_SKIP_REPLAY") != nullptr;
  if (skip) return P3D_OK;
  LaunchScope ls("mesh_cuda_order", s);
  const uint64_t nwords = (uint64_t)a.N * (uint64_t)a.SY * (uint64_t)a.SX;
  const bool words = a.tie_words != nullptr && nwords > 0 && nwords < 0xffffffffull;
  const unsigned wgrid = (unsigned)ceil_div((int64_t)nwords, kTieWordsPerWave);
  const unsigned mult = words ? scatter_multiplier(nwords) : 1u;
  if (!words) a.tie_words = nullptr;
  if (csr != nullptr) {
    a.csr = *csr;
    set_tiles(&a, g->bin_size, g->BH, g->BW);
    if (words)
      mesh_cuda_order_words_kernel<true><<<wgrid, kTieWaves * kWave, 0, s>>>(a, (unsigned)nwords, mult);
    else
      mesh_cuda_order_kernel<true><<<tile_grid(a.tm), kStage, 0, s>>>(a);
  } else {
    set_tiles(&a, a.H > a.W ? a.H : a.W, 1, 1);
    if (words)
      mesh_cuda_order_words_kernel<false><<<wgrid, kTieWaves * kWave, 0, s>>>(a, (unsigned)nwords, mult);
    else
      mesh_cuda_order_kernel<false><<<tile_grid(a.tm), kStage, 0, s>>>(a);
  }
  return launch_status();
}

P3D_API int p3d_rasterize_meshes_ex(const float* face_verts, const int64_t* mesh_first, const int64_t* mesh_count,
                                    const int64_t* neighbor, int64_t F, int N, int H, int W, float blur_radius, int K, int bin_size,
                                    int max_faces_per_bin, int persp, int clip, int cull, int64_t* p2f, float* zbuf, float* bary,
                                    float* dists, int32_t* cover, unsigned flags, void* workspace, size_t workspace_bytes,
                                    p3d_stream_t stream) {
  const bool cuda_order = (flags & P3D_RASTER_CUDA_TIE_ORDER) != 0, with_list = (flags & P3D_RASTER_COVER_LIST) != 0;
  if ((flags & ~(P3D_RASTER_COVER_LIST | P3D_RASTER_CUDA_TIE_ORDER)) != 0 || (cuda_order && with_list) || (with_list && cover == nullptr))
    return P3D_ERR_INVALID_ARG;
  const int rc = check_common(N, H, W, K);
  if (rc != P3D_OK) return rc;
  hipStream_t s = (hipStream_t)stream;
  const bool any_output = (int64_t)N * H * W * K != 0;
  MeshArgs a = mesh_args(face_verts, mesh_first, mesh_count, neighbor, N, H, W, blur_radius, K, persp, clip, cull, p2f, zbuf, bary, dists);
  a.ties = cuda_order ? 1 : 0;
  const size_t full_workspace_bytes = workspace_bytes;
  const bool words_ok = bin_size <= 0 || max_faces_per_bin <= 0 || make_internal_geom(H > 0 ? H : 1, W > 0 ? W : 1, bin_size).bin_size % 8 == 0;
  if (cuda_order && words_ok && any_output && workspace != nullptr && N > 0 && H > 0 && W > 0) {
    const size_t mb = tie_marks_bytes(N, H, W);
    if (workspace_bytes >= mb + 256) {
      const size_t at = (workspace_bytes - mb) & ~(size_t)255;
      if (((uintptr_t)workspace & 7u) == 0) {
        a.tie_words = reinterpret_cast<unsigned long long*>(static_cast<char*>(workspace) + at);
        a.SY = (H + 7) / 8;
        a.SX = (W + 7) / 8;
        workspace_bytes = at;
        if (hipMemsetAsync(a.tie_words, 0, mb, s) != hipSuccess) return P3D_ERR_LAUNCH;
      }
    }
  }
  if (bin_size <= 0 || max_faces_per_bin <= 0) {
    const int st = mesh_naive_impl(a, F, cover, with_list, s);
    if (st != P3D_OK || !cuda_order || !any_output) return st;
    return cuda_order_replay(a, nullptr, nullptr, s);
  }
  if (cover != nullptr && !any_output) return cover_begin(&a, cover, with_list, true, s);
  if (!any_output) return P3D_OK;
  if ((!face_verts || !neighbor) && F > 0) return P3D_ERR_INVALID_ARG;
  if (!mesh_first || !mesh_count || !p2f || !zbuf || !bary || !dists) return P3D_ERR_INVALID_ARG;
  const BinGeom gu = make_geom(H, W, bin_size);
  if (gu.BH > P3D_MAX_BINS_PER_SIDE || gu.BW > P3D_MAX_BINS_PER_SIDE) return P3D_ERR_TOO_MANY_BINS;
  const BinGeom g = make_internal_geom(H, W, bin_size);
  Arena arena(workspace, workspace_bytes);
  BinWorkspace ws;
  if (!workspace) return P3D_ERR_WORKSPACE;
  if (!bin_carve(arena, F, N, g, max_faces_per_bin, &ws, 1)) {
    if (a.tie_words == nullptr) return P3D_ERR_WORKSPACE;
    a.tie_words = nullptr;
    a.SY = a.SX = 0;
    workspace_bytes = full_workspace_bytes;
    arena = Arena(workspace, workspace_bytes);
    if (!bin_carve(arena, F, N, g, max_faces_per_bin, &ws, 1)) return P3D_ERR_WORKSPACE;
  }
  const bool is_short = ws.capacity < ws.worst;
  a.overflow = is_short ? ws.plan_hdr + 2 : nullptr;
  int st = bin_build(kTriangles, face_verts, nullptr, mesh_first, mesh_count, F, N, g, max_faces_per_bin,
                     sqrtf(blur_radius), ws, s);
  if (st != P3D_OK) return st;
  BinCSR csr{ws.offset, ws.total, ws.list, TilePlan{ws.arank, ws.bg_list, ws.plan_hdr, ws.order}};
  st = mesh_fine_from_csr(a, csr, g, cover, with_list, s);
  if (st == P3D_OK && is_short) st = mesh_naive_impl(a, F, cover, with_list, s);
  if (st != P3D_OK || !cuda_order) return st;
  st = cuda_order_replay(a, &csr, &g, s);
  if (st != P3D_OK || !is_short) return st;
  return cuda_order_replay(a, nullptr, nullptr, s);
}

P3D_API int p3d_rasterize_meshes(const float* face_verts, const int64_t* mesh_first, const int64_t* mesh_count,
                                 const int64_t* neighbor, int64_t F, int N, int H, int W, float blur_radius, int K,
                                 int bin_size, int max_faces_per_bin, int persp, int clip, int cull, int64_t* p2f,
                                 float* zbuf, float* bary, float* dists, void* workspace, size_t workspace_bytes,
                                 p3d_stream_t stream) {
  return p3d_rasterize_meshes_ex(face_verts, mesh_first, mesh_count, neighbor, F, N, H, W, blur_radius, K, bin_size, max_faces_per_bin,
                                 persp, clip, cull, p2f, zbuf, bary, dists, nullptr, 0, workspace, workspace_bytes, stream);
}

P3D_API int p3d_rasterize_meshes_coarse(const float* face_verts, const int64_t* mesh_first, const int64_t* mesh_count,
                                        int64_t F, int N, int H, int W, float blur_radius, int bin_size,
                                        int max_faces_per_bin, int32_t* bin_faces, void* workspace,
                                        size_t workspace_bytes, p3d_stream_t stream) {
  if (N < 0 || H <= 0 || W <= 0 || bin_size <= 0 || max_faces_per_bin < 0) return P3D_ERR_INVALID_ARG;
  const BinGeom g = make_geom(H, W, bin_size);
  if (g.BH > P3D_MAX_BINS_PER_SIDE || g.BW > P3D_MAX_BINS_PER_SIDE) return P3D_ERR_TOO_MANY_BINS;
  if ((int64_t)N * g.nbins * max_faces_per_bin == 0) return P3D_OK;
  if (!mesh_first || !mesh_count || !bin_faces || (!face_verts && F > 0)) return P3D_ERR_INVALID_ARG;
  Arena arena(workspace, workspace_bytes);
  BinWorkspace ws;
  if (!workspace || !bin_carve(arena, F, N, g, max_faces_per_bin, &ws)) return P3D_ERR_WORKSPACE;
  hipStream_t s = (hipStream_t)stream;
  int st = bin_build(kTriangles, face_verts, nullptr, mesh_first, mesh_count, F, N, g, max_faces_per_bin,
                     sqrtf(blur_radius), ws, s);
  if (st != P3D_OK) return st;
  return bin_expand_padded(ws, N, g, max_faces_per_bin, bin_faces, s);
}

P3D_API int p3d_rasterize_meshes_fine(const float* face_verts, const int32_t* bin_faces, const int64_t* neighbor,
                                      int64_t F, int N, int BH, int BW, int M, int H, int W, float blur_radius,
                                      int bin_size, int K, int persp, int clip, int cull, int64_t* p2f, float* zbuf,
                                      float* bary, float* dists, void* workspace, size_t workspace_bytes,
                                      p3d_stream_t stream) {
  const int rc = check_common(N, H, W, K);
  if (rc != P3D_OK) return rc;
  if ((int64_t)N * H * W * K == 0) return P3D_OK;
  if (bin_size <= 0 || BH <= 0 || BW <= 0 || M < 0) return P3D_ERR_INVALID_ARG;
  if (((!face_verts || !neighbor) && F > 0) || !p2f || !zbuf || !bary || !dists) return P3D_ERR_INVALID_ARG;
  if (BH > P3D_MAX_BINS_PER_SIDE || BW > P3D_MAX_BINS_PER_SIDE) return P3D_ERR_TOO_MANY_BINS;
  if ((int64_t)BH * bin_size < H || (int64_t)BW * bin_size < W) return P3D_ERR_INVALID_ARG;
  if (workspace_bytes < p3d_rasterize_fine_workspace_bytes(N, BH, BW, M) || !workspace) return P3D_ERR_WORKSPACE;
  if (M > 0 && !bin_faces) return P3D_ERR_INVALID_ARG;
  const int64_t rows = (int64_t)N * BH * BW;
  Arena arena(workspace, workspace_bytes);
  int* list = arena.take<int>((size_t)rows * M);
  int* total = arena.take<int>((size_t)rows);
  int64_t* offset = arena.take<int64_t>((size_t)rows + 1);
  hipStream_t s = (hipStream_t)stream;
  int st = bin_compact_padded(bin_faces, rows, M, list, total, offset, s);
  if (st != P3D_OK) return st;
  BinGeom g;
  g.H = H;
  g.W = W;
  g.bin_size = bin_size;
  g.BH = BH;
  g.BW = BW;
  g.nbins = BH * BW;
  BinCSR csr{offset, total, list, TilePlan{nullptr, nullptr, nullptr, nullptr}};
  return mesh_fine_from_csr(mesh_args(face_verts, nullptr, nullptr, neighbor, N, H, W, blur_radius, K, persp, clip, cull, p2f, zbuf, bary,
                                      dists),
                            csr, g, nullptr, false, s);
}
```

pytorch3d_amd/csrc/raster_mesh_bwd.hip:

```cpp
#include "p3d_common.h"
#include "p3d_geom.h"
#include "wave_table.h"

#include <stdlib.h>

#include <type_traits>

namespace p3d {

namespace {

constexpr int kRegion = 32;
constexpr int kBwdSlots = 182;
using FaceTable = WaveTable<9, kBwdSlots, kRows>;
using FaceTableV = WaveTable<9, kBwdSlots, kCorners>;

struct BwdArgs {
  const float* face_verts;
  const int64_t* p2f;
  const float* grad_zbuf;
  const float* grad_bary;
  const float* grad_dists;
  float* grad_fv;
  const int64_t* faces;
// ... 466 lines not shown
  BwdArgs a;
  a.face_pre = reinterpret_cast<const float4*>(face_pre);
  a.V = V;
  a.face_verts = face_verts;
  a.p2f = p2f;
  a.grad_zbuf = grad_zbuf;
  a.grad_bary = grad_bary;
  a.grad_dists = grad_dists;
  a.grad_fv = grad_out;
  a.faces = faces;
  a.N = N;
  a.H = H;
  a.W = W;
  a.K = K;
  a.RY = (int)ceil_div(H, kRegion);
  a.RX = (int)ceil_div(W, kRegion);
  a.persp = persp;
  a.clip = clip;
  a.cover = cover;
  a.CY = (H + 15) / 16;
  a.CX = (W + 15) / 16;
  a.area_list = nullptr;
  a.area_count = nullptr;
  const bool rows_kernel = K == 4 || K == 8 || K == 16 || K == 32;
  const int64_t items = rows_kernel ? (int64_t)N * a.CY * a.CX : (int64_t)N * a.RY * a.RX;
  if (items > 0x7fffffffll) return P3D_ERR_INVALID_ARG;
  a.nblocks = (unsigned)items;
  a.scatter = scatter_multiplier((uint64_t)items);
  if (rows_kernel && cover != nullptr && cover_has_list) {
    const int* count = reinterpret_cast<const int*>(cover) + items;
    a.area_list = count + 16;
    a.area_count = count;
  } else if (rows_kernel && cover != nullptr && workspace != nullptr &&
      workspace_bytes >= p3d_rasterize_meshes_backward_workspace_bytes(N, H, W)) {
    int* count = static_cast<int*>(workspace);
    int* list = count + 16;
    if (hipMemsetAsync(count, 0, sizeof(int), s) != hipSuccess) return P3D_ERR_LAUNCH;
    LaunchScope ls("mesh_backward_areas", s);
    area_list_kernel<<<(unsigned)ceil_div(items, 256), 256, 0, s>>>(cover, (int)items, list, count);
    a.area_list = list;
    a.area_count = count;
  }
  LaunchScope ls("mesh_backward", s);
  const unsigned grid = rows_kernel ? (unsigned)ceil_div(items, 4) : (unsigned)items;
  const bool pc = persp && clip;
#define P3D_LAUNCH_MESH_BWD(TV)                                                  \
  switch (K) {                                                                   \
    case 1: mesh_backward_kernel<1, TV><<<grid, 256, 0, s>>>(a); break;          \
    case 2: mesh_backward_kernel<2, TV><<<grid, 256, 0, s>>>(a); break;          \
    case 4:                                                                      \
      if (pc && a.face_pre) mesh_backward_rows_kernel<4, TV, true, true><<<grid, 256, 0, s>>>(a); \
      else if (pc) mesh_backward_rows_kernel<4, TV, true><<<grid, 256, 0, s>>>(a); \
      else mesh_backward_rows_kernel<4, TV><<<grid, 256, 0, s>>>(a);             \
      break;                                                                     \
    case 8:                                                                      \
      if (pc && a.face_pre) mesh_backward_rows_kernel<8, TV, true, true><<<grid, 256, 0, s>>>(a); \
      else if (pc) mesh_backward_rows_kernel<8, TV, true><<<grid, 256, 0, s>>>(a); \
      else mesh_backward_rows_kernel<8, TV><<<grid, 256, 0, s>>>(a);             \
      break;                                                                     \
    case 16: mesh_backward_rows_kernel<16, TV><<<grid, 256, 0, s>>>(a); break;   \
    case 32: mesh_backward_rows_kernel<32, TV><<<grid, 256, 0, s>>>(a); break;   \
    default: mesh_backward_kernel<0, TV><<<grid, 256, 0, s>>>(a); break;         \
  }
  if (faces) {
    P3D_LAUNCH_MESH_BWD(true)
  } else {
    P3D_LAUNCH_MESH_BWD(false)
  }
#undef P3D_LAUNCH_MESH_BWD
  return launch_status();
}
}

P3D_API size_t p3d_rasterize_meshes_backward_workspace_bytes(int N, int H, int W) {
  if (N <= 0 || H <= 0 || W <= 0) return 0;
  return ((size_t)N * (size_t)((H + 15) / 16) * (size_t)((W + 15) / 16) + 16) * sizeof(int);
}

P3D_API int p3d_rasterize_meshes_backward_ex(const float* face_verts, const int64_t* faces, float* face_pre, const int64_t* p2f,
                                              const float* grad_zbuf, const float* grad_bary, const float* grad_dists, const int32_t* cover,
                                              int64_t F, int64_t V, int N, int H, int W, int K, int persp, int clip, unsigned flags,
                                              float* grad_out, void* workspace, size_t workspace_bytes, p3d_stream_t stream) {
  if (F < 0 || V < 0 || N < 0 || H < 0 || W < 0 || K < 0) return P3D_ERR_INVALID_ARG;
  if ((flags & ~(P3D_BWD_COVER_HAS_LIST | P3D_BWD_MAKE_FACE_PRE)) != 0 || ((uintptr_t)face_pre & 15u)) return P3D_ERR_INVALID_ARG;
  const int64_t out_floats = faces ? V * 3 : F * 9;
  if (out_floats == 0) return P3D_OK;
  if (!grad_out) return P3D_ERR_INVALID_ARG;
  hipStream_t s = (hipStream_t)stream;
  if (hipMemsetAsync(grad_out, 0, (size_t)out_floats * sizeof(float), s) != hipSuccess) return P3D_ERR_LAUNCH;
  if (F == 0 || (int64_t)N * H * W * K == 0) return P3D_OK;
  if (!face_verts || !p2f || !grad_zbuf || !grad_bary || !grad_dists) return P3D_ERR_INVALID_ARG;
  if (flags & P3D_BWD_MAKE_FACE_PRE) {
    if (face_pre != nullptr && persp && clip && (K == 4 || K == 8)) {
      int64_t blocks = ceil_div(F, 256);
      if (blocks > 256 * 16) blocks = 256 * 16;
      LaunchScope ls("face_pre", s);
      face_pre_kernel<<<(unsigned)blocks, 256, 0, s>>>(face_verts, F, reinterpret_cast<float4*>(face_pre));
      const int st = launch_status();
      if (st != P3D_OK) return st;
    } else {
      face_pre = nullptr;
    }
  }
  const bool list = cover != nullptr && (flags & P3D_BWD_COVER_HAS_LIST) != 0;
  return launch_mesh_backward(face_verts, faces, faces ? V : -1, p2f, grad_zbuf, grad_bary, grad_dists, N, H, W, K, persp, clip,
                              grad_out, cover, list ? nullptr : workspace, list ? 0 : workspace_bytes, s, list, face_pre);
}

P3D_API int p3d_rasterize_meshes_backward(const float* face_verts, const int64_t* p2f, const float* grad_zbuf,
                                          const float* grad_bary, const float* grad_dists, int64_t F, int N, int H,
                                          int W, int K, int persp, int clip, float* grad_face_verts,
                                          p3d_stream_t stream) {
  return p3d_rasterize_meshes_backward_ex(face_verts, nullptr, nullptr, p2f, grad_zbuf, grad_bary, grad_dists, nullptr, F, 0, N, H, W, K,
                                          persp, clip, 0, grad_face_verts, nullptr, 0, stream);
}

P3D_API int p3d_rasterize_meshes_cover_check(const int64_t* p2f, const int32_t* cover, int N, int H, int W, int K, int32_t* stale,
                                             p3d_stream_t stream) {
  if (N < 0 || H < 0 || W < 0 || K < 0 || !stale) return P3D_ERR_INVALID_ARG;
  hipStream_t s = (hipStream_t)stream;
  if (hipMemsetAsync(stale, 0, sizeof(int32_t), s) != hipSuccess) return P3D_ERR_LAUNCH;
  const int CY = (H + 15) / 16, CX = (W + 15) / 16;
  const int64_t items = (int64_t)N * H * CX;
  if (items == 0 || K == 0) return P3D_OK;
  if (!p2f || !cover) return P3D_ERR_INVALID_ARG;
  const int64_t blocks = ceil_div(items, 256);
  if (blocks > 0x7fffffffll) return P3D_ERR_INVALID_ARG;
  LaunchScope ls("mesh_cover_check", s);
  cover_check_kernel<<<(unsigned)blocks, 256, 0, s>>>(p2f, reinterpret_cast<const int*>(cover), N, H, W, K, CY, CX, reinterpret_cast<int*>(stale));
  return launch_status();
}
```

pytorch3d_amd/rasterize_meshes.py:

```python
from typing import List, Optional, Tuple, Union

import numpy as np
import torch

from . import _C

kMaxFacesPerBin = 22


def parse_image_size(image_size):
    if not isinstance(image_size, (tuple, list)):
        return (int(image_size), int(image_size))
    if len(image_size) != 2:
        raise ValueError("Image size can only be a tuple/list of (H, W)")
    if not all(i > 0 for i in image_size):
        raise ValueError("Image sizes must be greater than 0; got %d, %d" % tuple(image_size))
    if not all(isinstance(i, int) for i in image_size):
        raise ValueError("Image sizes must be integers; got %r, %r" % tuple(image_size))
    return tuple(image_size)


def default_bin_size(max_image_size: int) -> int:
    if max_image_size <= 64:
        return 8
    return int(2 ** max(np.ceil(np.log2(max_image_size)) - 4, 4))


def _bins(im_size, bin_size, max_faces_per_bin, num_faces):
    max_image_size = max(*im_size)
    if bin_size is None:
        bin_size = default_bin_size(max_image_size)
    if bin_size != 0:
        faces_per_bin = 1 + (max_image_size - 1) // bin_size
        if faces_per_bin >= kMaxFacesPerBin:
            raise ValueError("bin_size too small, number of faces per bin must be less than %d; got %d" %
                             (kMaxFacesPerBin, faces_per_bin))
    if max_faces_per_bin is None:
        max_faces_per_bin = int(max(10000, num_faces / 5))
    return bin_size, max_faces_per_bin


def rasterize_meshes(
    meshes,
    image_size: Union[int, List[int], Tuple[int, int]] = 256,
    blur_radius: float = 0.0,
    faces_per_pixel: int = 8,
    bin_size: Optional[int] = None,
    max_faces_per_bin: Optional[int] = None,
    perspective_correct: bool = False,
    clip_barycentric_coords: bool = False,
    cull_backfaces: bool = False,
    z_clip_value: Optional[float] = None,
    cull_to_frustum: bool = False,
):
    verts_packed = meshes.verts_packed()
    faces_packed = meshes.faces_packed()
    fused_verts = (z_clip_value is None and not cull_to_frustum and _gatherable(verts_packed, faces_packed))
    face_verts = None if fused_verts else gather_face_verts(verts_packed, faces_packed)
    mesh_to_face_first_idx = meshes.mesh_to_faces_packed_first_idx()
    num_faces_per_mesh = meshes.num_faces_per_mesh()
    im_size = parse_image_size(image_size)

    clipped_faces = None
    clipped_faces_neighbor_idx = None
    if z_clip_value is not None or cull_to_frustum:
        from .clip import ClipFrustum, clip_faces

        frustum = ClipFrustum(left=-1, right=1, top=-1, bottom=1, perspective_correct=perspective_correct,
                              z_clip_value=z_clip_value, cull=cull_to_frustum)
        clipped_faces = clip_faces(face_verts, mesh_to_face_first_idx, num_faces_per_mesh, frustum=frustum)
        face_verts = clipped_faces.face_verts
        mesh_to_face_first_idx = clipped_faces.mesh_to_face_first_idx
        num_faces_per_mesh = clipped_faces.num_faces_per_mesh
        clipped_faces_neighbor_idx = clipped_faces.clipped_faces_neighbor_idx
    if clipped_faces_neighbor_idx is None:
        clipped_faces_neighbor_idx = torch.full(
            size=(faces_packed.shape[0] if fused_verts else face_verts.shape[0],), fill_value=-1,
            device=verts_packed.device, dtype=torch.int64)

    bin_size, max_faces_per_bin = _bins(im_size, bin_size, max_faces_per_bin, meshes._F)

    if fused_verts:
        return _RasterizeMeshVerts.apply(
            verts_packed, faces_packed, mesh_to_face_first_idx, num_faces_per_mesh, clipped_faces_neighbor_idx, im_size,
            blur_radius, faces_per_pixel, bin_size, max_faces_per_bin, perspective_correct, clip_barycentric_coords,
            cull_backfaces)
    pix_to_face, zbuf, barycentric_coords, dists = _RasterizeFaceVerts.apply(
        face_verts, mesh_to_face_first_idx, num_faces_per_mesh, clipped_faces_neighbor_idx, im_size, blur_radius,
        faces_per_pixel, bin_size, max_faces_per_bin, perspective_correct, clip_barycentric_coords, cull_backfaces)
    if clipped_faces is not None:
        from .clip import convert_clipped_rasterization_to_original_faces

        pix_to_face, barycentric_coords = convert_clipped_rasterization_to_original_faces(
            pix_to_face, barycentric_coords, clipped_faces)
    return pix_to_face, zbuf, barycentric_coords, dists


def _gatherable(verts_packed, faces_packed):
    return (verts_packed.is_cuda and verts_packed.dtype == torch.float32 and faces_packed.dtype == torch.int64
            and faces_packed.device == verts_packed.device and verts_packed.dim() == 2 and faces_packed.dim() == 2
            and verts_packed.shape[1] == 3 and faces_packed.shape[1] == 3)


def gather_face_verts(verts_packed, faces_packed):
    if _gatherable(verts_packed, faces_packed):
        return _GatherFaceVerts.apply(verts_packed, faces_packed)
    return verts_packed[faces_packed]


class _GatherFaceVerts(torch.autograd.Function):
    @staticmethod
    def forward(ctx, verts, faces):
        import ctypes

        from . import _lib

        lib = _lib.load()
        verts_c, faces_c = verts.contiguous(), faces.contiguous()
        V, F = verts_c.shape[0], faces_c.shape[0]
        with torch.cuda.device(verts.device):
            out = torch.empty((F, 3, 3), dtype=torch.float32, device=verts.device)
            if F:
                rc = lib.p3d_gather_face_verts(_C._ptr(verts_c), _C._ptr(faces_c), V, F, _C._ptr(out),
                                               _C._stream(verts.device))
                _lib.check(rc, "gather_face_verts")
        ctx.save_for_backward(faces_c)
        ctx.V = V
        return out

    @staticmethod
    def backward(ctx, grad_face_verts):
        (faces,) = ctx.saved_tensors
        return _C.scatter_face_grads(grad_face_verts, faces, ctx.V), None


class _RasterizeFaceVerts(torch.autograd.Function):

    @staticmethod
    def forward(ctx, face_verts, mesh_to_face_first_idx, num_faces_per_mesh, clipped_faces_neighbor_idx,
                image_size=(256, 256), blur_radius=0.01, faces_per_pixel=0, bin_size=0, max_faces_per_bin=0,
                perspective_correct=False, clip_barycentric_coords=False, cull_backfaces=False):
        (pix_to_face, zbuf, barycentric_coords, dists), cover = _C._rasterize_meshes_covered(
            face_verts, mesh_to_face_first_idx, num_faces_per_mesh, clipped_faces_neighbor_idx, image_size,
            blur_radius, faces_per_pixel, bin_size, max_faces_per_bin, perspective_correct, clip_barycentric_coords,
            cull_backfaces)
        ctx.save_for_backward(face_verts, pix_to_face, cover)
        ctx.mark_non_differentiable(pix_to_face)
        ctx.set_materialize_grads(False)
        ctx.perspective_correct = perspective_correct
        ctx.clip_barycentric_coords = clip_barycentric_coords
        return pix_to_face, zbuf, barycentric_coords, dists

    @staticmethod
    def backward(ctx, grad_pix_to_face, grad_zbuf, grad_barycentric_coords, grad_dists):
        face_verts, pix_to_face, cover = ctx.saved_tensors
        cover = _C.checked_cover(pix_to_face, cover)
        if grad_zbuf is None and grad_barycentric_coords is None and grad_dists is None:
            return (None,) * 12
        grad_face_verts = _C._mesh_backward(face_verts, None, 0, pix_to_face, grad_zbuf, grad_barycentric_coords, grad_dists,
                                            ctx.perspective_correct, ctx.clip_barycentric_coords, cover)
        return (grad_face_verts,) + (None,) * 11


class _RasterizeMeshVerts(torch.autograd.Function):

    @staticmethod
    def forward(ctx, verts, faces, mesh_to_face_first_idx, num_faces_per_mesh, clipped_faces_neighbor_idx, image_size,
                blur_radius, faces_per_pixel, bin_size, max_faces_per_bin, perspective_correct, clip_barycentric_coords,
                cull_backfaces):
        from . import _lib

        lib = _lib.load()
        verts_c, faces_c = verts.contiguous(), faces.contiguous()
        V, F = verts_c.shape[0], faces_c.shape[0]
        with torch.cuda.device(verts.device):
            face_verts = torch.empty((F, 3, 3), dtype=torch.float32, device=verts.device)
            face_pre = torch.empty((F, 4), dtype=torch.float32, device=verts.device) if (_C.FACE_PRE and ctx.needs_input_grad[0]) else None
            if F and face_pre is not None:
                rc = lib.p3d_gather_face_verts_pre(_C._ptr(verts_c), _C._ptr(faces_c), V, F, _C._ptr(face_verts), _C._ptr(face_pre),
                                                   _C._stream(verts.device))
                _lib.check(rc, "gather_face_verts_pre")
            elif F:
                rc = lib.p3d_gather_face_verts(_C._ptr(verts_c), _C._ptr(faces_c), V, F, _C._ptr(face_verts),
                                               _C._stream(verts.device))
                _lib.check(rc, "gather_face_verts")
        (pix_to_face, zbuf, barycentric_coords, dists), cover = _C._rasterize_meshes_covered(
            face_verts, mesh_to_face_first_idx, num_faces_per_mesh, clipped_faces_neighbor_idx, image_size, blur_radius,
            faces_per_pixel, bin_size, max_faces_per_bin, perspective_correct, clip_barycentric_coords, cull_backfaces)
        ctx.save_for_backward(face_verts, faces_c, pix_to_face, cover, face_pre)
        ctx.mark_non_differentiable(pix_to_face)
        ctx.set_materialize_grads(False)
        ctx.V = V
        ctx.flags = (int(bool(perspective_correct)), int(bool(clip_barycentric_coords)))
        return pix_to_face, zbuf, barycentric_coords, dists

    @staticmethod
    def backward(ctx, grad_pix_to_face, grad_zbuf, grad_barycentric_coords, grad_dists):
        face_verts, faces, pix_to_face, cover, face_pre = ctx.saved_tensors
        cover = _C.checked_cover(pix_to_face, cover)
        if grad_zbuf is None and grad_barycentric_coords is None and grad_dists is None:
            return (None,) * 13
        grad_verts = _C._mesh_backward(face_verts, faces, ctx.V, pix_to_face, grad_zbuf, grad_barycentric_coords, grad_dists,
                                       *ctx.flags, cover, face_pre)
        return (grad_verts,) + (None,) * 12


def _pack_matrices(world_to_view, view_to_ndc, n_meshes, device):
    mats = []
    for m in (world_to_view, view_to_ndc):
        m = torch.as_tensor(m, dtype=torch.float32, device=device)
        if m.dim() == 2:
            m = m[None]
        if m.dim() != 3 or m.shape[1:] != (4, 4) or m.shape[0] not in (1, n_meshes):
            raise ValueError("camera matrices must have shape (4, 4), (1, 4, 4) or (N, 4, 4); got %s" % repr(tuple(m.shape)))
        mats.append(m)
    num = max(mats[0].shape[0], mats[1].shape[0])
    return torch.stack([m.expand(num, 4, 4) for m in mats], 1).contiguous()


def transform_points_reference(verts_packed, mesh_idx, world_to_view, view_to_ndc):
    one = torch.ones_like(verts_packed[:, :1])
    a = world_to_view[mesh_idx] if world_to_view.shape[0] > 1 else world_to_view.expand(verts_packed.shape[0], 4, 4)
    b = view_to_ndc[mesh_idx] if view_to_ndc.shape[0] > 1 else view_to_ndc.expand(verts_packed.shape[0], 4, 4)
    vh = torch.bmm(torch.cat([verts_packed, one], 1)[:, None], a)[:, 0]
    view = vh[:, :3] / vh[:, 3:]
    nh = torch.bmm(torch.cat([view, one], 1)[:, None], b)[:, 0]
    ndc = nh[:, :3] / nh[:, 3:]
    return torch.cat([ndc[:, :2], view[:, 2:3]], 1)


def rasterize_meshes_world(meshes_world, world_to_view, view_to_ndc, image_size=256, blur_radius: float = 0.0,
                           faces_per_pixel: int = 8, bin_size: Optional[int] = None, max_faces_per_bin: Optional[int] = None,
                           perspective_correct: bool = False, clip_barycentric_coords: bool = False,
                           cull_backfaces: bool = False):
    verts = meshes_world.verts_packed()
    faces = meshes_world.faces_packed()
    n = len(meshes_world)
    w2v = torch.as_tensor(world_to_view)
    v2n = torch.as_tensor(view_to_ndc)
    if not _gatherable(verts, faces):
        a = w2v.to(verts.device, torch.float32)
        b = v2n.to(verts.device, torch.float32)
        a = a[None] if a.dim() == 2 else a
        b = b[None] if b.dim() == 2 else b
        ndc = transform_points_reference(verts, meshes_world.verts_packed_to_mesh_idx(), a, b)
        return rasterize_meshes(_PackedVertsView(meshes_world, ndc), image_size, blur_radius, faces_per_pixel, bin_size,
                                max_faces_per_bin, perspective_correct, clip_barycentric_coords, cull_backfaces)
    mats = _pack_matrices(w2v, v2n, n, verts.device)
    im_size = parse_image_size(image_size)
    bin_size, max_faces_per_bin = _bins(im_size, bin_size, max_faces_per_bin, meshes_world._F)
    nbr = torch.full((faces.shape[0],), -1, dtype=torch.int64, device=verts.device)
    return _RasterizeMeshWorld.apply(verts, faces, meshes_world.mesh_to_faces_packed_first_idx(),
                                     meshes_world.num_faces_per_mesh(), meshes_world.mesh_to_verts_packed_first_idx(), mats, nbr,
                                     (im_size, blur_radius, faces_per_pixel, bin_size, max_faces_per_bin,
                                      bool(perspective_correct), bool(clip_barycentric_coords), bool(cull_backfaces)))


class _TransformVerts(torch.autograd.Function):

    @staticmethod
    def forward(ctx, verts, vert_first, mats):
        from . import _lib

        lib = _lib.load()
        v = verts.contiguous()
        dev = v.device
        with torch.cuda.device(dev):
            out = torch.empty_like(v)
            if v.shape[0]:
                rc = lib.p3d_transform_verts_forward(_C._ptr(v), _C._ptr(vert_first), _C._ptr(mats), v.shape[0], vert_first.shape[0],
                                                     mats.shape[0], _C._ptr(out), _C._stream(dev))
                _lib.check(rc, "transform_verts_forward")
        ctx.save_for_backward(v, vert_first, mats)
        return out

    @staticmethod
    def backward(ctx, g):
        v, vert_first, mats = ctx.saved_tensors
        g_world, g_mats = _transform_backward(v, vert_first, mats, g.contiguous(), ctx.needs_input_grad[0], ctx.needs_input_grad[2])
        return g_world, None, g_mats


def camera_grad_tree_depth(count):
    rows = -(-int(count) // 64) + 1
    return 12 + -(-rows // 64)

# ... 92 lines not shown
```

Measured before the change: 8224.

## Fuse face-vertex gather and gradient zeroing into the binning count kernel

The face-vertex gather (and face_pre computation) moves into the bin_count kernel's chunk prologue, which reads verts/faces directly and writes face_verts as a side effect. That kernel also zeroes the vertex-gradient buffer in a grid-stride loop, so the backward can skip its memset. A null neighbor index replaces the torch.full tensor allocation. Together these remove separate launches and allocations from the forward/backward pipeline. The cost is extra work and register pressure in the binning kernel, plus a cross-call dependency on a pre-zeroed buffer held in ctx.

```diff
diff --git a/include/p3d_amd.h b/include/p3d_amd.h
--- a/include/p3d_amd.h
+++ b/include/p3d_amd.h
@@ -82,6 +82,14 @@
                             float* dists, int32_t* cover, unsigned flags, void* workspace, size_t workspace_bytes,
                             p3d_stream_t stream);
 
+int p3d_rasterize_meshes_verts_ex(const float* verts, const int64_t* faces, int64_t V, float* face_verts, float* face_pre,
+                                  float* zero_verts, const int64_t* mesh_to_face_first_idx, const int64_t* num_faces_per_mesh,
+                                  const int64_t* clipped_faces_neighbor_idx, int64_t F, int N, int H, int W, float blur_radius,
+                                  int faces_per_pixel, int bin_size, int max_faces_per_bin, int perspective_correct,
+                                  int clip_barycentric_coords, int cull_backfaces, int64_t* pix_to_face, float* zbuf, float* bary,
+                                  float* dists, int32_t* cover, unsigned flags, void* workspace, size_t workspace_bytes,
+                                  p3d_stream_t stream);
+
 int p3d_gather_face_verts_pre(const float* verts, const int64_t* faces, int64_t V, int64_t F, float* face_verts, float* face_pre,
                               p3d_stream_t stream);
 
@@ -89,6 +97,7 @@
 
 #define P3D_BWD_COVER_HAS_LIST 1u
 #define P3D_BWD_MAKE_FACE_PRE 2u
+#define P3D_BWD_GRAD_OUT_ZEROED 8u
 
 int p3d_rasterize_meshes_backward_ex(const float* face_verts, const int64_t* faces, float* face_pre,
                                      const int64_t* pix_to_face, const float* grad_zbuf, const float* grad_bary,
diff --git a/pytorch3d_amd/_C.py b/pytorch3d_amd/_C.py
--- a/pytorch3d_amd/_C.py
+++ b/pytorch3d_amd/_C.py
@@ -209,6 +209,9 @@
 RECALL_COVERS = os.environ.get("P3D_RECALL_COVERS", "1") not in ("", "0")
 COVER_LIST = os.environ.get("P3D_COVER_LIST", "1") not in ("", "0")
 FACE_PRE = os.environ.get("P3D_FACE_PRE", "1") not in ("", "0")
+NULL_NEIGHBOR = os.environ.get("P3D_NULL_NEIGHBOR", "1") not in ("", "0")
+FUSED_GATHER = os.environ.get("P3D_FUSED_GATHER", "1") not in ("", "0")
+PRECLEARED_GRAD = os.environ.get("P3D_PRECLEARED_GRAD", "1") not in ("", "0")
 CHECK_COVERS = os.environ.get("P3D_CHECK", "0") not in ("", "0")
 COVER_RECALLS = [0, 0]
 COVER_CHECKS = [0, 0]
@@ -267,14 +270,14 @@
 
 def _rasterize_meshes_covered(face_verts, mesh_to_face_first_idx, num_faces_per_mesh, clipped_faces_neighbor_idx, image_size,
                               blur_radius, faces_per_pixel, bin_size, max_faces_per_bin, perspective_correct,
-                              clip_barycentric_coords, cull_backfaces, want_cover=True):
+                              clip_barycentric_coords, cull_backfaces, want_cover=True, packed=None):
     dev = _same_device(("face_verts", face_verts), ("mesh_to_face_first_idx", mesh_to_face_first_idx),
                        ("num_faces_per_mesh", num_faces_per_mesh),
-                       ("clipped_faces_neighbor_idx", clipped_faces_neighbor_idx))
+                       *([("clipped_faces_neighbor_idx", clipped_faces_neighbor_idx)] if clipped_faces_neighbor_idx is not None else []))
     _check_face_verts(face_verts)
     if num_faces_per_mesh.size(0) != mesh_to_face_first_idx.size(0):
         raise RuntimeError("num_faces_per_mesh must have save size first dimension as mesh_to_faces_packed_first_idx")
-    if clipped_faces_neighbor_idx.size(0) != face_verts.size(0):
+    if clipped_faces_neighbor_idx is not None and clipped_faces_neighbor_idx.size(0) != face_verts.size(0):
         raise RuntimeError("clipped_faces_neighbor_idx must have save size first dimension as face_verts")
     K = int(faces_per_pixel)
     _check_k(K)
@@ -285,12 +288,14 @@
         _num_bins(H, W, bin_size, "RasterizeCoarseCuda")
     fv = _c(face_verts, torch.float32)
     first, count = _c(mesh_to_face_first_idx, torch.int64), _c(num_faces_per_mesh, torch.int64)
-    nb = _c(clipped_faces_neighbor_idx, torch.int64)
+    nb = _c(clipped_faces_neighbor_idx, torch.int64) if clipped_faces_neighbor_idx is not None else None
     N, F = count.size(0), fv.size(0)
     lib = _lib.load()
     with torch.cuda.device(dev):
         out = _mesh_outputs(N, H, W, K, dev)
         if out[0].numel() == 0:
+            if packed is not None:
+                raise RuntimeError("packed vertices with an empty output: gather the faces with p3d_gather_face_verts instead")
             return out, None
         marks = N * ((H + 7) // 8) * ((W + 7) // 8) * 8 + 1024 if CUDA_TIE_ORDER else 0
         ws, need, need_at, entries = _mesh_workspace(lib, F, N, H, W, bin_size, M, dev, extra=marks) if binned else (_workspace(marks, dev), None, 0, None)
@@ -302,10 +307,17 @@
             flags |= _lib.RASTER_COVER_LIST
         elif want_cover:
             cover = torch.empty((N, (H + 15) // 16, (W + 15) // 16), dtype=torch.int32, device=dev)
-        rc = lib.p3d_rasterize_meshes_ex(
-            _ptr(fv), _ptr(first), _ptr(count), _ptr(nb), F, N, H, W, float(blur_radius), K, bin_size if binned else 0,
-            M if binned else 0, int(bool(perspective_correct)), int(bool(clip_barycentric_coords)), int(bool(cull_backfaces)),
-            _ptr(out[0]), _ptr(out[1]), _ptr(out[2]), _ptr(out[3]), _ptr(cover), flags, _ptr(ws), ws.numel(), _stream(dev))
+        tail = (_ptr(first), _ptr(count), _ptr(nb), F, N, H, W, float(blur_radius), K, bin_size if binned else 0,
+                M if binned else 0, int(bool(perspective_correct)), int(bool(clip_barycentric_coords)), int(bool(cull_backfaces)),
+                _ptr(out[0]), _ptr(out[1]), _ptr(out[2]), _ptr(out[3]), _ptr(cover), flags, _ptr(ws), ws.numel(), _stream(dev))
+        if packed is not None:
+            verts, faces, face_pre, zero_verts = packed
+            if fv is not face_verts:
+                raise RuntimeError("packed vertices: face_verts must be the contiguous float32 buffer the call fills")
+            rc = lib.p3d_rasterize_meshes_verts_ex(_ptr(verts), _ptr(faces), verts.size(0), _ptr(fv), _ptr(face_pre), _ptr(zero_verts),
+                                                   *tail)
+        else:
+            rc = lib.p3d_rasterize_meshes_ex(_ptr(fv), *tail)
         _lib.check(rc, "rasterize_meshes")
         if need is not None:
             need.report_later(ws, need_at, entries)
@@ -395,7 +407,7 @@
 
 
 def _mesh_backward(face_verts, faces, V, pix_to_face, grad_zbuf, grad_bary, grad_dists, perspective_correct, clip_barycentric_coords,
-                   cover, face_pre=None):
+                   cover, face_pre=None, zeroed_out=None):
     dev = pix_to_face.device
     zeros = lambda *tail: torch.zeros(tuple(pix_to_face.shape) + tail, dtype=torch.float32, device=dev)
     gz = _c(grad_zbuf, torch.float32) if grad_zbuf is not None else zeros()
@@ -415,7 +427,12 @@
                 flags |= _lib.BWD_MAKE_FACE_PRE
         else:
             faces = _c(faces, torch.int64)
-            out = (torch.empty if F else torch.zeros)((V, 3), dtype=torch.float32, device=dev)
+            if zeroed_out is not None and F and not _ordered() and tuple(zeroed_out.shape) == (V, 3) and zeroed_out.dtype == torch.float32 \
+                    and zeroed_out.device == dev and zeroed_out.is_contiguous():
+                out = zeroed_out
+                flags |= _lib.BWD_GRAD_OUT_ZEROED
+            else:
+                out = (torch.empty if F else torch.zeros)((V, 3), dtype=torch.float32, device=dev)
             if not (has_list or cover is None):
                 face_pre = None
         if F == 0:
diff --git a/pytorch3d_amd/_lib.py b/pytorch3d_amd/_lib.py
--- a/pytorch3d_amd/_lib.py
+++ b/pytorch3d_amd/_lib.py
@@ -19,6 +19,7 @@
 RASTER_CUDA_TIE_ORDER = 2
 BWD_COVER_HAS_LIST = 1
 BWD_MAKE_FACE_PRE = 2
+BWD_GRAD_OUT_ZEROED = 8
 KNN_MAX_K = 32
 KNN_TILE = 512
 KNN_ACCUMULATE_P2 = 1
@@ -57,6 +58,9 @@
     "p3d_rasterize_meshes_cover_list_bytes": (c_size, [c_int, c_int, c_int]),
     "p3d_rasterize_meshes_ex": (c_int, [c_ptr, c_ptr, c_ptr, c_ptr, c_i64, c_int, c_int, c_int, c_f32, c_int, c_int, c_int, c_int,
                                         c_int, c_int, c_ptr, c_ptr, c_ptr, c_ptr, c_ptr, c_uint, c_ptr, c_size, c_ptr]),
+    "p3d_rasterize_meshes_verts_ex": (c_int, [c_ptr, c_ptr, c_i64, c_ptr, c_ptr, c_ptr, c_ptr, c_ptr, c_ptr, c_i64, c_int, c_int, c_int,
+                                              c_f32, c_int, c_int, c_int, c_int, c_int, c_int, c_ptr, c_ptr, c_ptr, c_ptr, c_ptr, c_uint,
+                                              c_ptr, c_size, c_ptr]),
     "p3d_rasterize_meshes_backward_workspace_bytes": (c_size, [c_int, c_int, c_int]),
     "p3d_gather_face_verts": (c_int, [c_ptr, c_ptr, c_i64, c_i64, c_ptr, c_ptr]),
     "p3d_gather_face_verts_pre": (c_int, [c_ptr, c_ptr, c_i64, c_i64, c_ptr, c_ptr, c_ptr]),
diff --git a/pytorch3d_amd/build.py b/pytorch3d_amd/build.py
--- a/pytorch3d_amd/build.py
+++ b/pytorch3d_amd/build.py
@@ -11,7 +11,7 @@
 ARCH = "gfx950"
 
 SOURCES = ["binning.hip", "raster_mesh.hip", "raster_mesh_bwd.hip", "gather.hip", "transform.hip", "raster_points.hip", "render_points.hip", "composite.hip", "blend.hip", "clip.hip", "interp.hip", "shade.hip", "soft_phong.hip", "splatter.hip", "texture.hip", "texture_multi.hip", "atlas.hip", "ordered_bwd.hip", "normals.hip", "mesh_losses.hip", "knn.hip", "point_mesh.hip", "sample_points.hip", "fps_ball.hip", "points_to_volumes.hip", "point_frames.hip", "box3d.hip", "profile.cpp"]
-HEADERS = ["binning.h", "p3d_common.h", "p3d_geom.h", "topk.h", "topk_insert_asm.h", "wave_table.h", "tile_map.h", "chunk_order.h", "atlas_cell.h", "uvm_sample.h", "shade_sample.h", "ordered_sum.h", "knn_grad.h", "knn_queue.h", "point_mesh_geom.h", "vec3.h", "fixed_sum.h", "csr_gather.h", "box3d_geom.h", os.path.join("..", "..", "include", "p3d_amd.h")]
+HEADERS = ["binning.h", "p3d_common.h", "p3d_geom.h", "topk.h", "topk_insert_asm.h", "wave_table.h", "tile_map.h", "chunk_order.h", "atlas_cell.h", "uvm_sample.h", "shade_sample.h", "ordered_sum.h", "knn_grad.h", "knn_queue.h", "point_mesh_geom.h", "vec3.h", "fixed_sum.h", "csr_gather.h", "box3d_geom.h", "face_gather.h", os.path.join("..", "..", "include", "p3d_amd.h")]
 
 FLAGS = [
     f"--offload-arch={ARCH}", "-O3", "-std=c++17", "-fPIC", "-fvisibility=hidden", "-ffp-contract=off",
diff --git a/pytorch3d_amd/csrc/binning.h b/pytorch3d_amd/csrc/binning.h
--- a/pytorch3d_amd/csrc/binning.h
+++ b/pytorch3d_amd/csrc/binning.h
@@ -76,9 +76,20 @@
 size_t bin_workspace_bytes(int64_t E, int N, const BinGeom& g, int M, int64_t list_entries = -1, bool with_z = false);
 bool bin_carve(Arena& arena, int64_t E, int N, const BinGeom& g, int M, BinWorkspace* ws, int64_t list_entries = -1, bool with_z = false);
 
+struct BinFused {
+  const float* verts = nullptr;
+  const int64_t* faces = nullptr;
+  int64_t V = 0, E = 0;
+  float* face_verts = nullptr;
+  float4* face_pre = nullptr;
+  int* zero0 = nullptr;
+  int* zero1 = nullptr;
+  int64_t n0 = 0, n1 = 0;
+};
+
 int bin_build(BinKind kind, const float* elems, const float* aux, const int64_t* first, const int64_t* count, int64_t E,
               int N, const BinGeom& g, int M, float sqrt_blur, const BinWorkspace& ws, hipStream_t stream,
-              bool ordered = true);
+              bool ordered = true, const BinFused* fused = nullptr);
 
 int exclusive_scan_i32(const int* in, int64_t n, long long* blocksum, int64_t* out, hipStream_t stream);
 
diff --git a/pytorch3d_amd/csrc/binning.hip b/pytorch3d_amd/csrc/binning.hip
--- a/pytorch3d_amd/csrc/binning.hip
+++ b/pytorch3d_amd/csrc/binning.hip
@@ -1,5 +1,6 @@
 #include "binning.h"
 #include "p3d_geom.h"
+#include "face_gather.h"
 
 namespace p3d {
 
@@ -85,13 +86,13 @@
   return lo;
 }
 
-template <int KIND>
+template <int KIND, bool GATHER = false>
 __device__ __forceinline__ bool chunk_prologue(const float* __restrict__ elems, const float* __restrict__ aux,
                                                const int64_t* __restrict__ first, const int64_t* __restrict__ count,
                                                const int* chunk_start, int* cs_l, int N, int H, int W, int bin_size,
                                                int BH, int BW, float sqrt_blur, float* xlo_t, float* xhi_t,
                                                float* ylo_t, float* yhi_t, ChunkCtx* c, int* publish_plan = nullptr,
-                                               int* plan_hdr = nullptr) {
+                                               int* plan_hdr = nullptr, const BinFused* fz = nullptr) {
   const int tid = threadIdx.x;
   const int chunk = blockIdx.x;
   if (chunk_start == nullptr) {
@@ -136,7 +137,20 @@
     float xmin, xmax, ymin, ymax;
     bool skip;
     if (KIND == kTriangles) {
-      const float* q = elems + e * 9;
+      float q[9];
+      if (GATHER) {
+        if (e >= 0 && e < fz->E) {
+          gather_face_corners(fz->verts, fz->faces, fz->V, e, q);
+          store_face(q, e, fz->face_verts, fz->face_pre);
+        } else {
+#pragma unroll
+          for (int k = 0; k < 9; ++k) q[k] = __int_as_float(0x7fc00000);
+        }
+      } else {
+        const float* g = elems + e * 9;
+#pragma unroll
+        for (int k = 0; k < 9; ++k) q[k] = g[k];
+      }
       const float v0x = q[0], v0y = q[1], v0z = q[2];
       const float v1x = q[3], v1y = q[4], v1z = q[5];
       const float v2x = q[6], v2y = q[7], v2z = q[8];
@@ -205,23 +219,29 @@
   }
 }
 
-template <int KIND, bool ORDERED>
+template <int KIND, bool ORDERED, bool GATHER = false>
 __global__ __launch_bounds__(kBinChunk) void bin_count_kernel(const float* __restrict__ elems,
                                                               const float* __restrict__ aux,
                                                               const int64_t* __restrict__ first,
                                                               const int64_t* __restrict__ count,
                                                               const int* chunk_start, int N, int H, int W,
                                                               int bin_size, int BH, int BW, float sqrt_blur,
-                                                              int* __restrict__ counts, int* publish_plan, int* plan_hdr) {
+                                                              int* __restrict__ counts, int* publish_plan, int* plan_hdr,
+                                                              const BinFused fz) {
   __shared__ float xlo_t[32], xhi_t[32], ylo_t[32], yhi_t[32];
   __shared__ int cs_l[kSelfPlanMax + 1];
   __shared__ int blk_cnt[kMaxBins];
   __shared__ unsigned long long rowm[ORDERED ? kWavesPerChunk : 1][kMaxBinsSide], colm[ORDERED ? kWavesPerChunk : 1][kMaxBinsSide];
   const int nbins = BH * BW;
+  {
+    const int64_t t = (int64_t)blockIdx.x * kBinChunk + threadIdx.x, step = (int64_t)gridDim.x * kBinChunk;
+    for (int64_t i = t; i < fz.n0; i += step) fz.zero0[i] = 0;
+    for (int64_t i = t; i < fz.n1; i += step) fz.zero1[i] = 0;
+  }
   for (int b = threadIdx.x; b < nbins; b += kBinChunk) blk_cnt[b] = 0;
   ChunkCtx c;
-  if (!chunk_prologue<KIND>(elems, aux, first, count, chunk_start, cs_l, N, H, W, bin_size, BH, BW, sqrt_blur, xlo_t,
-                            xhi_t, ylo_t, yhi_t, &c, publish_plan, plan_hdr))
+  if (!chunk_prologue<KIND, GATHER>(elems, aux, first, count, chunk_start, cs_l, N, H, W, bin_size, BH, BW, sqrt_blur, xlo_t,
+                                    xhi_t, ylo_t, yhi_t, &c, publish_plan, plan_hdr, &fz))
     return;
   const int lane = lane_id();
   if (ORDERED) {
@@ -682,8 +702,10 @@
 }
 
 int bin_build(BinKind kind, const float* elems, const float* aux, const int64_t* first, const int64_t* count, int64_t E,
-              int N, const BinGeom& g, int M, float sqrt_blur, const BinWorkspace& ws, hipStream_t stream, bool ordered) {
+              int N, const BinGeom& g, int M, float sqrt_blur, const BinWorkspace& ws, hipStream_t stream, bool ordered,
+              const BinFused* fused) {
   if (N <= 0) return P3D_OK;
+  const BinFused fz = (fused != nullptr && kind == kTriangles) ? *fused : BinFused();
   const int64_t rows = (int64_t)N * g.nbins;
   const bool small = N <= kSelfPlanMax && rows <= 4096 && ws.max_chunks <= 128;
   const bool self_plan = N <= kSelfPlanMax;
@@ -696,15 +718,18 @@
   const unsigned chunks = (unsigned)ws.max_chunks;
   {
     LaunchScope ls("bin_count", stream);
-    if (kind == kTriangles)
+    if (kind == kTriangles && fz.verts != nullptr)
+      bin_count_kernel<kTriangles, true, true><<<chunks, kBinChunk, 0, stream>>>(elems, aux, first, count, cs, N, g.H, g.W, g.bin_size,
+                                                                                g.BH, g.BW, sqrt_blur, ws.counts, publish, ws.plan_hdr, fz);
+    else if (kind == kTriangles)
       bin_count_kernel<kTriangles, true><<<chunks, kBinChunk, 0, stream>>>(elems, aux, first, count, cs, N, g.H, g.W,
-                                                                          g.bin_size, g.BH, g.BW, sqrt_blur, ws.counts, publish, ws.plan_hdr);
+                                                                          g.bin_size, g.BH, g.BW, sqrt_blur, ws.counts, publish, ws.plan_hdr, fz);
     else if (ordered)
       bin_count_kernel<kPoints, true><<<chunks, kBinChunk, 0, stream>>>(elems, aux, first, count, cs, N, g.H, g.W,
-                                                                       g.bin_size, g.BH, g.BW, sqrt_blur, ws.counts, publish, ws.plan_hdr);
+                                                                       g.bin_size, g.BH, g.BW, sqrt_blur, ws.counts, publish, ws.plan_hdr, fz);
     else
       bin_count_kernel<kPoints, false><<<chunks, kBinChunk, 0, stream>>>(elems, aux, first, count, cs, N, g.H, g.W,
-                                                                        g.bin_size, g.BH, g.BW, sqrt_blur, ws.counts, publish, ws.plan_hdr);
+                                                                        g.bin_size, g.BH, g.BW, sqrt_blur, ws.counts, publish, ws.plan_hdr, fz);
   }
   if (small) {
     LaunchScope ls("bin_scan_small", stream);
diff --git a/pytorch3d_amd/csrc/face_gather.h b/pytorch3d_amd/csrc/face_gather.h
--- /dev/null
+++ b/pytorch3d_amd/csrc/face_gather.h
@@ -0,0 +1,32 @@
+#pragma once
+
+#include "p3d_geom.h"
+
+namespace p3d {
+
+__device__ __forceinline__ void gather_face_corners(const float* __restrict__ verts, const int64_t* __restrict__ faces, int64_t V,
+                                                    int64_t f, float c[9]) {
+  const float nan = __int_as_float(0x7fc00000);
+#pragma unroll
+  for (int k = 0; k < 3; ++k) {
+    int64_t v = faces[f * 3 + k];
+    if (v < 0) v += V;
+    const bool ok = v >= 0 && v < V;
+    const float* s = verts + (ok ? v : 0) * 3;
+    c[3 * k + 0] = ok ? s[0] : nan;
+    c[3 * k + 1] = ok ? s[1] : nan;
+    c[3 * k + 2] = ok ? s[2] : nan;
+  }
+}
+
+__device__ __forceinline__ void store_face(const float c[9], int64_t f, float* __restrict__ face_verts, float4* __restrict__ face_pre) {
+  float* d = face_verts + f * 9;
+#pragma unroll
+  for (int k = 0; k < 9; ++k) d[k] = c[k];
+  if (face_pre != nullptr) {
+    const BwdFacePre r = bwd_face_pre_make(mk3(c[0], c[1], c[2]), mk3(c[3], c[4], c[5]), mk3(c[6], c[7], c[8]));
+    face_pre[f] = make_float4(r.inv_area, r.inv_l01, r.inv_l02, r.inv_l12);
+  }
+}
+
+}
diff --git a/pytorch3d_amd/csrc/gather.hip b/pytorch3d_amd/csrc/gather.hip
--- a/pytorch3d_amd/csrc/gather.hip
+++ b/pytorch3d_amd/csrc/gather.hip
@@ -1,5 +1,6 @@
 #include "p3d_common.h"
 #include "p3d_geom.h"
+#include "face_gather.h"
 #include "wave_table.h"
 
 namespace p3d {
@@ -26,22 +27,8 @@
                                                                float4* __restrict__ face_pre) {
   for (int64_t f = (int64_t)blockIdx.x * 256 + threadIdx.x; f < F; f += (int64_t)gridDim.x * 256) {
     float c[9];
-    const float nan = __int_as_float(0x7fc00000);
-#pragma unroll
-    for (int k = 0; k < 3; ++k) {
-      int64_t v = faces[f * 3 + k];
-      if (v < 0) v += V;
-      const bool ok = v >= 0 && v < V;
-      const float* s = verts + (ok ? v : 0) * 3;
-      c[3 * k + 0] = ok ? s[0] : nan;
-      c[3 * k + 1] = ok ? s[1] : nan;
-      c[3 * k + 2] = ok ? s[2] : nan;
-    }
-    float* d = face_verts + f * 9;
-#pragma unroll
-    for (int k = 0; k < 9; ++k) d[k] = c[k];
-    const BwdFacePre r = bwd_face_pre_make(mk3(c[0], c[1], c[2]), mk3(c[3], c[4], c[5]), mk3(c[6], c[7], c[8]));
-    face_pre[f] = make_float4(r.inv_area, r.inv_l01, r.inv_l02, r.inv_l12);
+    gather_face_corners(verts, faces, V, f, c);
+    store_face(c, f, face_verts, face_pre);
   }
 }
 
diff --git a/pytorch3d_amd/csrc/raster_mesh.hip b/pytorch3d_amd/csrc/raster_mesh.hip
--- a/pytorch3d_amd/csrc/raster_mesh.hip
+++ b/pytorch3d_amd/csrc/raster_mesh.hip
@@ -568,7 +568,7 @@
   float x0, x1, y0, y1;
 };
 
-template <bool BINNED, bool PC = false>
+template <bool BINNED, bool PC = false, bool NB = true>
 __device__ __forceinline__ int stage_chunk(const MeshArgs& a, const StageLds& l, const TileRect& tile, int64_t src_base,
                                            int count, int base, int tid, bool cull, bool clip, bool prune, bool* general) {
   const int lane = tid & 63, w = tid >> 6;
@@ -585,7 +585,7 @@
     fid = BINNED ? a.csr.list[src_base + i] : (int)(src_base + i);
     P3D_CHAIN_ARRIVED(2, "v"(fid));
     const float* g = a.face_verts + (int64_t)fid * 9;
-    nb = (int)a.neighbor[fid];
+    if (NB) nb = (int)a.neighbor[fid];
     v0 = mk3(g[0], g[1], g[2]);
     v1 = mk3(g[3], g[4], g[5]);
     v2 = mk3(g[6], g[7], g[8]);
@@ -735,7 +735,7 @@
 }
 
 template <typename Queue, int KT, bool IN_REGS, bool BINNED, bool EXACT, int WAVES = kFineWaves, bool PC = false,
-          bool SPLIT = false, bool TIES = false>
+          bool SPLIT = false, bool TIES = false, bool NB = true>
 __global__ __launch_bounds__(kStage, WAVES) void mesh_raster_kernel(MeshArgs a) {
   static_assert(!(SPLIT && TIES), "the tie marks of four queues that merge are not tracked: CUDA tie order runs the plain kernels");
   __shared__ float s_merge[SPLIT ? 3 * kMergeWords * KT * kWave : 1];
@@ -909,7 +909,7 @@
   int tie_drop = kEmptyIdx;
   int staged = 0;
   for (; base < count; base += kStage) {
-    staged = stage_chunk<BINNED, PC>(a, lds, tile, src_base, count, base, tid, cull, clip, prune, &general);
+    staged = stage_chunk<BINNED, PC, NB>(a, lds, tile, src_base, count, base, tid, cull, clip, prune, &general);
     if (general) break;
     P3D_CHAIN_STAMP(4);
     chunk_bucket_order(s_zc, staged, s_order, s_qlow, s_ord, tid);
@@ -942,7 +942,7 @@
       base += kStage;
       if (base >= count) break;
       bool dummy = false;
-      staged = stage_chunk<BINNED, PC>(a, lds, tile, src_base, count, base, tid, cull, clip, prune, &dummy);
+      staged = stage_chunk<BINNED, PC, NB>(a, lds, tile, src_base, count, base, tid, cull, clip, prune, &dummy);
     }
   }
 
@@ -1062,7 +1062,7 @@
     if (i < count) {
       b.f = BINNED ? a.csr.list[src + i] : (int)(src + i);
       verts(b.f, &b.v0, &b.v1, &b.v2);
-      b.nb = (int)a.neighbor[b.f];
+      if (a.neighbor != nullptr) b.nb = (int)a.neighbor[b.f];
     }
     return b;
   };
@@ -1238,34 +1238,34 @@
   }
 }
 
-template <typename Q, int KT, bool REGS, bool BINNED, bool EXACT, bool TIES>
+template <typename Q, int KT, bool REGS, bool BINNED, bool EXACT, bool TIES, bool NB>
 void launch_fine_variant(const MeshArgs& a, unsigned grid, bool split, size_t dyn_lds, hipStream_t stream) {
   if constexpr (REGS && EXACT && BINNED && !TIES) {
     if (split) {
       constexpr int kSplitWaves = KT >= 8 ? 2 : (KT >= 4 ? 3 : kFineWaves);
-      mesh_raster_kernel<Q, KT, REGS, BINNED, EXACT, kSplitWaves, false, true><<<grid * 4, kStage, 0, stream>>>(a);
+      mesh_raster_kernel<Q, KT, REGS, BINNED, EXACT, kSplitWaves, false, true, false, NB><<<grid * 4, kStage, 0, stream>>>(a);
       return;
     }
   }
   if constexpr (REGS && EXACT) {
     if (a.persp && a.clip) {
-      mesh_raster_kernel<typename PcQueue<Q>::type, KT, REGS, BINNED, EXACT, kFineWaves, true, false, TIES><<<grid, kStage, dyn_lds, stream>>>(a);
+      mesh_raster_kernel<typename PcQueue<Q>::type, KT, REGS, BINNED, EXACT, kFineWaves, true, false, TIES, NB><<<grid, kStage, dyn_lds, stream>>>(a);
       return;
     }
   }
-  mesh_raster_kernel<Q, KT, REGS, BINNED, EXACT, kFineWaves, false, false, TIES><<<grid, kStage, dyn_lds, stream>>>(a);
-}
-
-template <int KT, bool BINNED, int WAVES, bool TIES>
+  mesh_raster_kernel<Q, KT, REGS, BINNED, EXACT, kFineWaves, false, false, TIES, NB><<<grid, kStage, dyn_lds, stream>>>(a);
+}
+
+template <int KT, bool BINNED, int WAVES, bool TIES, bool NB>
 void launch_long_variant(const MeshArgs& a, unsigned grid, hipStream_t stream) {
   if (a.persp && a.clip)
-    mesh_raster_kernel<TopKPairs<KT, true, 0>, KT, true, BINNED, false, WAVES, true, false, TIES><<<grid, kStage, 0, stream>>>(a);
+    mesh_raster_kernel<TopKPairs<KT, true, 0>, KT, true, BINNED, false, WAVES, true, false, TIES, NB><<<grid, kStage, 0, stream>>>(a);
   else
-    mesh_raster_kernel<TopKPairs<KT, false, 0>, KT, true, BINNED, false, WAVES, false, false, TIES><<<grid, kStage, 0, stream>>>(a);
+    mesh_raster_kernel<TopKPairs<KT, false, 0>, KT, true, BINNED, false, WAVES, false, false, TIES, NB><<<grid, kStage, 0, stream>>>(a);
 }
 
 #define P3D_COMMA ,
-template <bool BINNED, bool TIES>
+template <bool BINNED, bool TIES, bool NB>
 int launch_mesh_raster_t(const MeshArgs& a0, hipStream_t stream) {
   MeshArgs a = a0;
   unsigned grid = tile_grid(a.tm);
@@ -1277,9 +1277,9 @@
   a.list_by_plan = a.walk_plan && a.area_list != nullptr && a.overflow == nullptr && a.tm.bin_size == kTile && a.H % kTile == 0 && a.W % kTile == 0 &&
                    a.csr.plan.arank != nullptr;
   const size_t dyn_lds = 0;
-#define P3D_LAUNCH_FINE(KT_, REGS_, EXACT_, Q_) launch_fine_variant<Q_, KT_, REGS_, BINNED, EXACT_, TIES>(a, grid, split, dyn_lds, stream)
-#define P3D_LAUNCH_FINE_W(KT_, WAVES_, Q_) mesh_raster_kernel<Q_, KT_, true, BINNED, false, WAVES_, false, false, TIES><<<grid, kStage, 0, stream>>>(a)
-#define P3D_LAUNCH_LONG(KT_, WAVES_) launch_long_variant<KT_, BINNED, WAVES_, TIES>(a, grid, stream)
+#define P3D_LAUNCH_FINE(KT_, REGS_, EXACT_, Q_) launch_fine_variant<Q_, KT_, REGS_, BINNED, EXACT_, TIES, NB>(a, grid, split, dyn_lds, stream)
+#define P3D_LAUNCH_FINE_W(KT_, WAVES_, Q_) mesh_raster_kernel<Q_, KT_, true, BINNED, false, WAVES_, false, false, TIES, NB><<<grid, kStage, 0, stream>>>(a)
+#define P3D_LAUNCH_LONG(KT_, WAVES_) launch_long_variant<KT_, BINNED, WAVES_, TIES, NB>(a, grid, stream)
   if (K == 1)
     P3D_LAUNCH_FINE(1, true, true, TopKReg<1 P3D_COMMA kMeshPayload>);
   else if (K == 2)
@@ -1312,7 +1312,8 @@
 
 template <bool BINNED>
 int launch_mesh_raster(const MeshArgs& a, hipStream_t stream) {
-  return a.ties ? launch_mesh_raster_t<BINNED, true>(a, stream) : launch_mesh_raster_t<BINNED, false>(a, stream);
+  if (a.neighbor == nullptr) return a.ties ? launch_mesh_raster_t<BINNED, true, false>(a, stream) : launch_mesh_raster_t<BINNED, false, false>(a, stream);
+  return a.ties ? launch_mesh_raster_t<BINNED, true, true>(a, stream) : launch_mesh_raster_t<BINNED, false, true>(a, stream);
 }
 
 void set_tiles(MeshArgs* a, int bin_size, int BH, int BW) { a->tm = make_tile_map(a->N, a->H, a->W, bin_size, BH, BW, true); }
@@ -1417,7 +1418,7 @@
   const int st = cover_begin(&a, cover, with_list, a.overflow == nullptr, s);
   if (st != P3D_OK) return st;
   if ((int64_t)a.N * a.H * a.W * a.K == 0) return P3D_OK;
-  if ((!a.face_verts || !a.neighbor) && F > 0) return P3D_ERR_INVALID_ARG;
+  if (!a.face_verts && F > 0) return P3D_ERR_INVALID_ARG;
   if (!a.mesh_first || !a.mesh_count || !a.p2f || !a.zbuf || !a.bary || !a.dists) return P3D_ERR_INVALID_ARG;
   set_tiles(&a, a.H > a.W ? a.H : a.W, 1, 1);
   return launch_mesh_raster<false>(a, s);
@@ -1434,9 +1435,10 @@
                          F, nullptr, false, (hipStream_t)stream);
 }
 
-static int mesh_fine_from_csr(MeshArgs a, const BinCSR& csr, const BinGeom& g, int32_t* cover, bool with_list, hipStream_t s) {
+static int mesh_fine_from_csr(MeshArgs a, const BinCSR& csr, const BinGeom& g, int32_t* cover, bool with_list, hipStream_t s,
+                              bool zero = true) {
   a.csr = csr;
-  const int st = cover_begin(&a, cover, with_list, true, s);
+  const int st = cover_begin(&a, cover, with_list, zero, s);
   if (st != P3D_OK) return st;
   set_tiles(&a, g.bin_size, g.BH, g.BW);
   return launch_mesh_raster<true>(a, s);
@@ -1468,11 +1470,36 @@
   return launch_status();
 }
 
-P3D_API int p3d_rasterize_meshes_ex(const float* face_verts, const int64_t* mesh_first, const int64_t* mesh_count,
-                                    const int64_t* neighbor, int64_t F, int N, int H, int W, float blur_radius, int K, int bin_size,
-                                    int max_faces_per_bin, int persp, int clip, int cull, int64_t* p2f, float* zbuf, float* bary,
-                                    float* dists, int32_t* cover, unsigned flags, void* workspace, size_t workspace_bytes,
-                                    p3d_stream_t stream) {
+#ifndef P3D_BIN_CLEARS_COVER
+#define P3D_BIN_CLEARS_COVER 1
+#endif
+
+struct VertsIn {
+  const float* verts;
+  const int64_t* faces;
+  int64_t V;
+  float* face_verts;
+  float* face_pre;
+  float* zero_verts;
+};
+
+static int verts_in_standalone(const VertsIn& vi, int64_t F, hipStream_t s) {
+  if (F > 0) {
+    const int st = vi.face_pre != nullptr ? p3d_gather_face_verts_pre(vi.verts, vi.faces, vi.V, F, vi.face_verts, vi.face_pre, s)
+                                          : p3d_gather_face_verts(vi.verts, vi.faces, vi.V, F, vi.face_verts, s);
+    if (st != P3D_OK) return st;
+  }
+  if (vi.zero_verts != nullptr && vi.V > 0 &&
+      hipMemsetAsync(vi.zero_verts, 0, (size_t)vi.V * 3 * sizeof(float), s) != hipSuccess)
+    return P3D_ERR_LAUNCH;
+  return P3D_OK;
+}
+
+static int rasterize_meshes_impl(const float* face_verts, const int64_t* mesh_first, const int64_t* mesh_count,
+                                 const int64_t* neighbor, int64_t F, int N, int H, int W, float blur_radius, int K, int bin_size,
+                                 int max_faces_per_bin, int persp, int clip, int cull, int64_t* p2f, float* zbuf, float* bary,
+                                 float* dists, int32_t* cover, unsigned flags, void* workspace, size_t workspace_bytes,
+                                 p3d_stream_t stream, const VertsIn* vi) {
   const bool cuda_order = (flags & P3D_RASTER_CUDA_TIE_ORDER) != 0, with_list = (flags & P3D_RASTER_COVER_LIST) != 0;
   if ((flags & ~(P3D_RASTER_COVER_LIST | P3D_RASTER_CUDA_TIE_ORDER)) != 0 || (cuda_order && with_list) || (with_list && cover == nullptr))
     return P3D_ERR_INVALID_ARG;
@@ -1480,6 +1507,11 @@
   if (rc != P3D_OK) return rc;
   hipStream_t s = (hipStream_t)stream;
   const bool any_output = (int64_t)N * H * W * K != 0;
+  const bool fuse_verts = vi != nullptr && bin_size > 0 && max_faces_per_bin > 0 && any_output && F > 0;
+  if (vi != nullptr && !fuse_verts) {
+    const int st = verts_in_standalone(*vi, F, s);
+    if (st != P3D_OK) return st;
+  }
   MeshArgs a = mesh_args(face_verts, mesh_first, mesh_count, neighbor, N, H, W, blur_radius, K, persp, clip, cull, p2f, zbuf, bary, dists);
   a.ties = cuda_order ? 1 : 0;
   const size_t full_workspace_bytes = workspace_bytes;
@@ -1504,7 +1536,7 @@
   }
   if (cover != nullptr && !any_output) return cover_begin(&a, cover, with_list, true, s);
   if (!any_output) return P3D_OK;
-  if ((!face_verts || !neighbor) && F > 0) return P3D_ERR_INVALID_ARG;
+  if (!face_verts && F > 0) return P3D_ERR_INVALID_ARG;
   if (!mesh_first || !mesh_count || !p2f || !zbuf || !bary || !dists) return P3D_ERR_INVALID_ARG;
   const BinGeom gu = make_geom(H, W, bin_size);
   if (gu.BH > P3D_MAX_BINS_PER_SIDE || gu.BW > P3D_MAX_BINS_PER_SIDE) return P3D_ERR_TOO_MANY_BINS;
@@ -1522,16 +1554,65 @@
   }
   const bool is_short = ws.capacity < ws.worst;
   a.overflow = is_short ? ws.plan_hdr + 2 : nullptr;
+  BinFused fz;
+  const size_t cover_words = cover != nullptr ? p3d_rasterize_meshes_cover_bytes(N, H, W) / sizeof(int32_t) : 0;
+  const bool bin_clears_cover = P3D_BIN_CLEARS_COVER && cover_words > 0;
+  if (bin_clears_cover) {
+    fz.zero0 = cover;
+    fz.n0 = (int64_t)cover_words + (with_list ? 16 : 0);
+  }
+  if (fuse_verts) {
+    fz.verts = vi->verts;
+    fz.faces = vi->faces;
+    fz.V = vi->V;
+    fz.E = F;
+    fz.face_verts = vi->face_verts;
+    fz.face_pre = reinterpret_cast<float4*>(vi->face_pre);
+    if (vi->zero_verts != nullptr) {
+      fz.zero1 = reinterpret_cast<int*>(vi->zero_verts);
+      fz.n1 = vi->V * 3;
+    }
+  }
   int st = bin_build(kTriangles, face_verts, nullptr, mesh_first, mesh_count, F, N, g, max_faces_per_bin,
-                     sqrtf(blur_radius), ws, s);
+                     sqrtf(blur_radius), ws, s, true, &fz);
   if (st != P3D_OK) return st;
   BinCSR csr{ws.offset, ws.total, ws.list, TilePlan{ws.arank, ws.bg_list, ws.plan_hdr, ws.order}};
-  st = mesh_fine_from_csr(a, csr, g, cover, with_list, s);
+  st = mesh_fine_from_csr(a, csr, g, cover, with_list, s, !bin_clears_cover);
   if (st == P3D_OK && is_short) st = mesh_naive_impl(a, F, cover, with_list, s);
   if (st != P3D_OK || !cuda_order) return st;
   st = cuda_order_replay(a, &csr, &g, s);
   if (st != P3D_OK || !is_short) return st;
   return cuda_order_replay(a, nullptr, nullptr, s);
+}
+
+P3D_API int p3d_rasterize_meshes_ex(const float* face_verts, const int64_t* mesh_first, const int64_t* mesh_count,
+                                    const int64_t* neighbor, int64_t F, int N, int H, int W, float blur_radius, int K, int bin_size,
+                                    int max_faces_per_bin, int persp, int clip, int cull, int64_t* p2f, float* zbuf, float* bary,
+                                    float* dists, int32_t* cover, unsigned flags, void* workspace, size_t workspace_bytes,
+                                    p3d_stream_t stream) {
+  return rasterize_meshes_impl(face_verts, mesh_first, mesh_count, neighbor, F, N, H, W, blur_radius, K, bin_size, max_faces_per_bin,
+                               persp, clip, cull, p2f, zbuf, bary, dists, cover, flags, workspace, workspace_bytes, stream, nullptr);
+}
+
+P3D_API int p3d_rasterize_meshes_verts_ex(const float* verts, const int64_t* faces, int64_t V, float* face_verts, float* face_pre,
+                                          float* zero_verts, const int64_t* mesh_first, const int64_t* mesh_count,
+                                          const int64_t* neighbor, int64_t F, int N, int H, int W, float blur_radius, int K,
+                                          int bin_size, int max_faces_per_bin, int persp, int clip, int cull, int64_t* p2f,
+                                          float* zbuf, float* bary, float* dists, int32_t* cover, unsigned flags, void* workspace,
+                                          size_t workspace_bytes, p3d_stream_t stream) {
+  if ((flags & ~(P3D_RASTER_COVER_LIST | P3D_RASTER_CUDA_TIE_ORDER)) != 0 ||
+      ((flags & P3D_RASTER_CUDA_TIE_ORDER) != 0 && (flags & P3D_RASTER_COVER_LIST) != 0) ||
+      ((flags & P3D_RASTER_COVER_LIST) != 0 && cover == nullptr))
+    return P3D_ERR_INVALID_ARG;
+  if (V < 0 || F < 0) return P3D_ERR_INVALID_ARG;
+  if (face_pre != nullptr && (face_verts == nullptr || ((uintptr_t)face_pre & 15u) != 0)) return P3D_ERR_INVALID_ARG;
+  if (F > 0 && (!verts || !faces || !face_verts)) return P3D_ERR_INVALID_ARG;
+  const int rc = check_common(N, H, W, K);
+  if (rc != P3D_OK) return rc;
+  if ((int64_t)N * H * W * K != 0 && (!mesh_first || !mesh_count || !p2f || !zbuf || !bary || !dists)) return P3D_ERR_INVALID_ARG;
+  const VertsIn vi{verts, faces, V, face_verts, face_pre, zero_verts};
+  return rasterize_meshes_impl(face_verts, mesh_first, mesh_count, neighbor, F, N, H, W, blur_radius, K, bin_size, max_faces_per_bin,
+                               persp, clip, cull, p2f, zbuf, bary, dists, cover, flags, workspace, workspace_bytes, stream, &vi);
 }
 
 P3D_API int p3d_rasterize_meshes(const float* face_verts, const int64_t* mesh_first, const int64_t* mesh_count,
diff --git a/pytorch3d_amd/csrc/raster_mesh_bwd.hip b/pytorch3d_amd/csrc/raster_mesh_bwd.hip
--- a/pytorch3d_amd/csrc/raster_mesh_bwd.hip
+++ b/pytorch3d_amd/csrc/raster_mesh_bwd.hip
@@ -572,12 +572,14 @@
                                               int64_t F, int64_t V, int N, int H, int W, int K, int persp, int clip, unsigned flags,
                                               float* grad_out, void* workspace, size_t workspace_bytes, p3d_stream_t stream) {
   if (F < 0 || V < 0 || N < 0 || H < 0 || W < 0 || K < 0) return P3D_ERR_INVALID_ARG;
-  if ((flags & ~(P3D_BWD_COVER_HAS_LIST | P3D_BWD_MAKE_FACE_PRE)) != 0 || ((uintptr_t)face_pre & 15u)) return P3D_ERR_INVALID_ARG;
+  if ((flags & ~(P3D_BWD_COVER_HAS_LIST | P3D_BWD_MAKE_FACE_PRE | P3D_BWD_GRAD_OUT_ZEROED)) != 0 || ((uintptr_t)face_pre & 15u))
+    return P3D_ERR_INVALID_ARG;
   const int64_t out_floats = faces ? V * 3 : F * 9;
   if (out_floats == 0) return P3D_OK;
   if (!grad_out) return P3D_ERR_INVALID_ARG;
   hipStream_t s = (hipStream_t)stream;
-  if (hipMemsetAsync(grad_out, 0, (size_t)out_floats * sizeof(float), s) != hipSuccess) return P3D_ERR_LAUNCH;
+  if ((flags & P3D_BWD_GRAD_OUT_ZEROED) == 0 && hipMemsetAsync(grad_out, 0, (size_t)out_floats * sizeof(float), s) != hipSuccess)
+    return P3D_ERR_LAUNCH;
   if (F == 0 || (int64_t)N * H * W * K == 0) return P3D_OK;
   if (!face_verts || !p2f || !grad_zbuf || !grad_bary || !grad_dists) return P3D_ERR_INVALID_ARG;
   if (flags & P3D_BWD_MAKE_FACE_PRE) {
diff --git a/pytorch3d_amd/rasterize_meshes.py b/pytorch3d_amd/rasterize_meshes.py
--- a/pytorch3d_amd/rasterize_meshes.py
+++ b/pytorch3d_amd/rasterize_meshes.py
@@ -73,7 +73,7 @@
         mesh_to_face_first_idx = clipped_faces.mesh_to_face_first_idx
         num_faces_per_mesh = clipped_faces.num_faces_per_mesh
         clipped_faces_neighbor_idx = clipped_faces.clipped_faces_neighbor_idx
-    if clipped_faces_neighbor_idx is None:
+    if clipped_faces_neighbor_idx is None and not _C.NULL_NEIGHBOR:
         clipped_faces_neighbor_idx = torch.full(
             size=(faces_packed.shape[0] if fused_verts else face_verts.shape[0],), fill_value=-1,
             device=verts_packed.device, dtype=torch.int64)
@@ -176,7 +176,14 @@
         with torch.cuda.device(verts.device):
             face_verts = torch.empty((F, 3, 3), dtype=torch.float32, device=verts.device)
             face_pre = torch.empty((F, 4), dtype=torch.float32, device=verts.device) if (_C.FACE_PRE and ctx.needs_input_grad[0]) else None
-            if F and face_pre is not None:
+            K, (H, W) = int(faces_per_pixel), image_size
+            fused = (_C.FUSED_GATHER and F > 0 and mesh_to_face_first_idx.shape[0] * H * W * K > 0 and verts_c.dtype == torch.float32
+                     and faces_c.dtype == torch.int64)
+            zeroed = None
+            if fused:
+                if _C.PRECLEARED_GRAD and ctx.needs_input_grad[0] and not _C._ordered():
+                    zeroed = torch.empty((V, 3), dtype=torch.float32, device=verts.device)
+            elif F and face_pre is not None:
                 rc = lib.p3d_gather_face_verts_pre(_C._ptr(verts_c), _C._ptr(faces_c), V, F, _C._ptr(face_verts), _C._ptr(face_pre),
                                                    _C._stream(verts.device))
                 _lib.check(rc, "gather_face_verts_pre")
@@ -186,11 +193,13 @@
                 _lib.check(rc, "gather_face_verts")
         (pix_to_face, zbuf, barycentric_coords, dists), cover = _C._rasterize_meshes_covered(
             face_verts, mesh_to_face_first_idx, num_faces_per_mesh, clipped_faces_neighbor_idx, image_size, blur_radius,
-            faces_per_pixel, bin_size, max_faces_per_bin, perspective_correct, clip_barycentric_coords, cull_backfaces)
+            faces_per_pixel, bin_size, max_faces_per_bin, perspective_correct, clip_barycentric_coords, cull_backfaces,
+            packed=(verts_c, faces_c, face_pre, zeroed) if fused else None)
         ctx.save_for_backward(face_verts, faces_c, pix_to_face, cover, face_pre)
         ctx.mark_non_differentiable(pix_to_face)
         ctx.set_materialize_grads(False)
         ctx.V = V
+        ctx.zeroed_grad_verts = zeroed
         ctx.flags = (int(bool(perspective_correct)), int(bool(clip_barycentric_coords)))
         return pix_to_face, zbuf, barycentric_coords, dists
 
@@ -200,8 +209,9 @@
         cover = _C.checked_cover(pix_to_face, cover)
         if grad_zbuf is None and grad_barycentric_coords is None and grad_dists is None:
             return (None,) * 13
+        zeroed, ctx.zeroed_grad_verts = getattr(ctx, "zeroed_grad_verts", None), None
         grad_verts = _C._mesh_backward(face_verts, faces, ctx.V, pix_to_face, grad_zbuf, grad_barycentric_coords, grad_dists,
-                                       *ctx.flags, cover, face_pre)
+                                       *ctx.flags, cover, face_pre, zeroed_out=zeroed)
         return (grad_verts,) + (None,) * 12
 
 
```

Measured after the change: 8360, median of 6. 1.02x the previous value.
